# holstegelab/otter

Hardware: AMD Instinct MI355X
Metric: regions/sec (otter assemble) on synthetic TR BED+BAM, 1/2/4/8 MI355X (higher is better)
Workload: dtype i16

## Files before the change

otter_amd/csrc/otg_common.hpp:

```cpp
#pragma once
#include <hip/hip_runtime.h>
#include <cstdint>
#include <cstdio>
#include <cstring>
#include <mutex>
#include <string>
#include <vector>
#include "../../include/otter_gpu.h"

#define OTG_NULL_OFF (-(1 << 30))

struct DevBuf {
  void* p = nullptr;
  size_t cap = 0;
};

struct otg_ctx {
  int device = 0;
  hipStream_t stream = nullptr;
  hipDeviceProp_t prop;
  std::string err;
  int exp_variant = 1;
  long long exp_probe_mismatches = 0;
  int n_cu = 256;
  uint32_t max_seq_len = 65536;
  std::vector<DevBuf> pool;
  struct Pipeline* pipe = nullptr;
  hipEvent_t ev0 = nullptr, ev1 = nullptr;
  hipStream_t tier_stream[5] = {nullptr, nullptr, nullptr, nullptr, nullptr};
  hipEvent_t ev_fork = nullptr, ev_join[5] = {nullptr, nullptr, nullptr, nullptr, nullptr};
  int edit_pass_kind = 0;
  uint32_t* edit_hist = nullptr;
  hipEvent_t edit_hist_ev[2] = {nullptr, nullptr};
  uint32_t edit_hist_mask[2] = {0u, 0u};
  double last_score_ms = 0.0, last_prov_ms = 0.0;
  uint32_t last_align_tiers[2] = {0u, 0u};
  double last_kmer_count_ms = 0.0, last_kmer_epi_ms = 0.0;
  hipEvent_t ev2 = nullptr;
  double last_motif_count_ms = 0.0, last_motif_reduce_ms = 0.0;
  uint32_t last_motif_n = 0, last_motif_stride = 0;
  double last_repeat_runs_ms = 0.0, last_repeat_select_ms = 0.0;
  uint32_t last_repeat_n = 0;
  uint64_t last_repeat_total = 0;
  bool last_repeat_valid = false;
  const uint8_t* last_motif_arena = nullptr;
  const uint64_t* last_motif_off = nullptr;
  const uint32_t* last_motif_len = nullptr;
  double last_unitalign_ms = 0.0;
  uint32_t last_unitalign_n = 0;
  double last_unitparse_forward_ms = 0.0, last_unitparse_trace_ms = 0.0;
  uint32_t last_unitparse_n = 0;
  uint64_t last_unitparse_total = 0;
  bool last_unitparse_valid = false;
  double last_kernel_ms = 0.0;
  double last_gt_align_ms = 0.0, last_gt_cluster_ms = 0.0;
  bool gt_edit_ran = false;
  size_t gt_edit_cnt_off = 0;
  int heur_strategy = OTG_HEURISTIC_NONE, heur_min_wf_len = 10, heur_max_dist = 50, heur_steps = 1;
  int last_chain = -1;
  struct AffineLast {
    uint32_t n_tasks = 0;
    bool hbm_tiers = false;
    bool bounded = false;
    bool sublist = false;
    int reg_mask = 0;
    const void* scores_at = nullptr;
  } affine_last;
  struct Cohort* cohort = nullptr;
};

extern thread_local std::string g_otg_err;

int otg_fail(otg_ctx* ctx, int code, const char* fmt, ...);

#define HIP_TRY(ctx, call)                                                                      \
  do {                                                                                          \
    hipError_t e__ = (call);                                                                    \
    if (e__ != hipSuccess)                                                                      \
      return otg_fail(ctx, OTG_ERR_HIP, "%s failed: %s (%s:%d)", #call, hipGetErrorString(e__), \
                      __FILE__, __LINE__);                                                      \
  } while (0)

void* otg_slot(otg_ctx* ctx, int slot, size_t bytes);

constexpr uint32_t OTG_CLUSTER_NMAX = 256;
enum {
  SLOT_ARENA = 0, SLOT_TASKS, SLOT_SCORES, SLOT_CELLS, SLOT_COUNTERS , SLOT_WF_WS, SLOT_CIG_OFF, SLOT_CIG_LEN,
  SLOT_CIG_ARENA, SLOT_BT_POOL, SLOT_ROWTAB, SLOT_REVOPS, SLOT_TASKSTATE, SLOT_TODO, SLOT_AUX0, SLOT_AUX1,
  SLOT_AUX2, SLOT_AUX3, SLOT_AUX4, SLOT_AUX5, SLOT_AUX6, SLOT_AUX7, SLOT_AUX8, SLOT_AUX9,
  SLOT_P0, SLOT_P1, SLOT_P2, SLOT_P3, SLOT_P4, SLOT_P5, SLOT_P6, SLOT_P7, SLOT_P8, SLOT_P9,
  SLOT_P10, SLOT_P11, SLOT_P12, SLOT_P13, SLOT_P14, SLOT_P15, SLOT_P16, SLOT_P17, SLOT_P18, SLOT_P19,
  SLOT_P20, SLOT_P21, SLOT_P22, SLOT_P23, SLOT_P24, SLOT_P25, SLOT_P26, SLOT_P27, SLOT_P28, SLOT_P29,
  SLOT_KMER_SEQ, SLOT_KMER_META, SLOT_KMER_HIST, SLOT_KMER_OUT,
  SLOT_KMER_BLK,
  SLOT_GTE_CLS, SLOT_GTE_TASKS, SLOT_GTE_SCORES, SLOT_GTE_DEN, SLOT_GTE_TODO,
  SLOT_MOTIF_SEQ, SLOT_MOTIF_META, SLOT_MOTIF_OFF, SLOT_MOTIF_M, SLOT_MOTIF_PLANES, SLOT_MOTIF_OUT,
  SLOT_REPEAT_SEQ, SLOT_REPEAT_META, SLOT_REPEAT_OFF, SLOT_REPEAT_CNT, SLOT_REPEAT_PLANES, SLOT_REPEAT_RUNS, SLOT_REPEAT_STACK, SLOT_REPEAT_SCRATCH,
  SLOT_REPEAT_RES, SLOT_REPEAT_SEGS,
  SLOT_UNITALIGN_SEQ, SLOT_UNITALIGN_META, SLOT_UNITALIGN_UNITS, SLOT_UNITALIGN_BINS, SLOT_UNITALIGN_ORDER,
  SLOT_UNITALIGN_OUT,
  SLOT_UNITPARSE_SEQ, SLOT_UNITPARSE_META, SLOT_UNITPARSE_UNITS, SLOT_UNITPARSE_PLAN, SLOT_UNITPARSE_TRACE,
  SLOT_UNITPARSE_RES, SLOT_UNITPARSE_SEGS,
  SLOT_COUNT
};

inline void otg_region_name(std::string& o, const char* chr, uint32_t chr_len, int32_t start, int32_t end)
{
  o.append(chr, chr_len);
  o += ':'; o += std::to_string((uint32_t)start); o += '-'; o += std::to_string((uint32_t)end);
}

void otg_pipeline_free(otg_ctx* ctx);
int64_t otg_pipeline_run_regions(otg_ctx* ctx);
void otg_cohort_free(otg_ctx* ctx);
void otg_bam_set_samples(otg_bam* b, const char* const* names, uint32_t n, int32_t offset_l, int32_t offset_r);

std::mutex& otg_device_mutex(int device);

#if defined(__HIPCC__)
__device__ __forceinline__ uint32_t otg_wave_atomic_add(uint32_t* ctr, uint32_t val)
{
  uint32_t r;
  uint64_t saved;
  asm volatile(
      "s_mov_b64 %1, exec\n\t"
      "s_mov_b64 exec, 1\n\t"
      "global_atomic_add %0, %2, %3, off sc0\n\t"
      "s_waitcnt vmcnt(0)\n\t"
      "s_mov_b64 exec, %1"
      : "=&v"(r), "=&s"(saved)
      : "v"(ctr), "v"(val)
      : "memory");
  return (uint32_t)__builtin_amdgcn_readfirstlane((int)r);
}

__device__ __forceinline__ int otg_imax(int a, int b) { return a > b ? a : b; }
__device__ __forceinline__ int otg_wave_max_i32(int v)
{
  constexpr int NEG = -2147483647 - 1;
  v = otg_imax(v, __builtin_amdgcn_update_dpp(NEG, v, 0x111, 0xf, 0xf, false));
  v = otg_imax(v, __builtin_amdgcn_update_dpp(NEG, v, 0x112, 0xf, 0xf, false));
  v = otg_imax(v, __builtin_amdgcn_update_dpp(NEG, v, 0x114, 0xf, 0xf, false));
  v = otg_imax(v, __builtin_amdgcn_update_dpp(NEG, v, 0x118, 0xf, 0xf, false));
  v = otg_imax(v, __builtin_amdgcn_update_dpp(NEG, v, 0x142, 0xa, 0xf, false));
  v = otg_imax(v, __builtin_amdgcn_update_dpp(NEG, v, 0x143, 0xc, 0xf, false));
  return __builtin_amdgcn_readlane(v, 63);
}

__device__ __forceinline__ void otg_myers_band(int K, int d, int pbf, int pef, int* KL, int* KU)
{
  const int u1 = (K + d + pbf + 1) / 2, u2 = K + pbf;
  *KU = u1 < u2 ? u1 : u2;
  int l = (K - d + pef + 1) / 2;
  if (l > K) l = K;
  if (K - d + pef < 0) l = K - d + pef;
  *KL = l;
}
__device__ __forceinline__ unsigned long long otg_edit_wfa_cells(int s, int m, int n, int pbf, int tbf)
{
  if (s < 0) return 0ull;
  if (pbf > m) pbf = m;
  if (tbf > n) tbf = n;
  const long long kh = s < n - tbf ? s : n - tbf, kl = s < m - pbf ? s : m - pbf;
  const long long sum_hi = (kh + 1) * tbf + kh * (kh + 1) / 2 + ((long long)s - kh) * n;
  const long long sum_lo = (kl + 1) * pbf + kl * (kl + 1) / 2 + ((long long)s - kl) * m;
  return (unsigned long long)(sum_hi + sum_lo + (long long)s + 1);
}

__device__ __forceinline__ int otg_myers_threshold(int R, int d, int pbf, int pef)
{
  int lo = 0, hi = R;
  while (lo < hi) {
    const int mid = (lo + hi + 1) >> 1;
    int kl, ku;
    otg_myers_band(mid, d, pbf, pef, &kl, &ku);
    if (kl + ku <= R) lo = mid; else hi = mid - 1;
  }
  return lo;
}

__device__ __forceinline__ uint64_t otg_load8(const uint8_t* p) { uint64_t v; __builtin_memcpy(&v, p, 8); return v; }

__device__ __forceinline__ int otg_dpp_shr1(int x) { return __builtin_amdgcn_update_dpp(x, x, 0x138, 0xf, 0xf, false); }
__device__ __forceinline__ int otg_dpp_shl1(int x) { return __builtin_amdgcn_update_dpp(x, x, 0x130, 0xf, 0xf, false); }

__device__ __forceinline__ bool otg_ends_free_done(int h, int v, int pl, int tl, int pef, int tef)
{
  return (h >= tl && pl - v <= pef) || (v >= pl && tl - h <= tef);
}

__device__ __forceinline__ int otg_match16(const uint8_t* P, const uint8_t* T, int v, int h, int rem)
{
  const uint64_t xl = otg_load8(P + v) ^ otg_load8(T + h), xh = otg_load8(P + v + 8) ^ otg_load8(T + h + 8);
  const int m = xl ? (__builtin_ctzll(xl) >> 3) : (xh ? 8 + (__builtin_ctzll(xh) >> 3) : 16);
  return m < rem ? m : rem;
}

__device__ __forceinline__ int otg_match64(const uint8_t* P, const uint8_t* T, int v, int h, int rem)
{
  uint64_t x[8];
#pragma unroll
  for (int i = 0; i < 8; ++i) x[i] = (8 * i < rem) ? (otg_load8(P + v + 8 * i) ^ otg_load8(T + h + 8 * i)) : ~0ull;
  int m = 64;
#pragma unroll
  for (int i = 7; i >= 0; --i) if (x[i]) m = 8 * i + (__builtin_ctzll(x[i]) >> 3);
  return m < rem ? m : rem;
}

__device__ __forceinline__ int otg_wave_match(const uint8_t* P, const uint8_t* T, int v, int h, int rem, int lane)
{
  int total = 0;
  while (total < rem) {
    const int off = total + lane * 8;
    const bool in = off < rem;
    uint64_t x = ~0ull;
    if (in) x = otg_load8(P + v + off) ^ otg_load8(T + h + off);
    const int m = x ? (int)(__builtin_ctzll(x) >> 3) : 8;
    const unsigned long long stop = __ballot(m < 8);
    if (stop) {
      const int first = (int)__builtin_ctzll(stop);
      total += first * 8 + __builtin_amdgcn_readlane(m, first);
      break;
    }
    total += 512;
  }
  return total < rem ? total : rem;
}
#endif


int otg_launch_edit(otg_ctx* ctx, const uint8_t* d_arena, const otg_align_task* d_tasks, uint32_t n_tasks,
                    int32_t* d_scores, uint64_t* d_cells, float* kernel_ms, uint64_t* launches);

int otg_launch_edit_align(otg_ctx* ctx, const uint8_t* d_arena, const otg_align_task* d_tasks, const otg_align_task* h_tasks, uint32_t n_tasks,
                          int32_t* scores_out, uint32_t* len_out, uint8_t* d_cig_base, const uint64_t* cig_slot, double* score_ms, double* prov_ms,
                          uint32_t* finished = nullptr);
int otg_launch_edit_align_adaptive(otg_ctx* ctx, const uint8_t* d_arena, const otg_align_task* d_tasks, const otg_align_task* h_tasks, uint32_t n_tasks,
                                   int32_t* scores_out, uint64_t* cells_out, uint32_t* len_out, uint8_t* d_cig_base, const uint64_t* cig_slot,
                                   double* score_ms, double* prov_ms, uint32_t finished[2]);

constexpr int OTG_MYERS_TIERS = 8;
constexpr int OTG_REG_TIERS = 5;
namespace otg_myers { struct PlaneBlock; }
int otg_launch_myers(otg_ctx* ctx, int tier, const uint8_t* d_arena, const otg_align_task* d_tasks, const uint32_t* d_todo,
                     const uint32_t* d_n_todo, uint32_t n_tasks, int32_t* d_scores, uint64_t* d_cells,
                     uint32_t* ticket, uint32_t* n_overflow, uint32_t* overflow_list,
                     const uint32_t* d_pblk = nullptr, const otg_myers::PlaneBlock* d_masks = nullptr);
int otg_launch_edit_todo(otg_ctx* ctx, const uint8_t* d_arena, const otg_align_task* d_tasks, const uint32_t* d_todo,
                         const uint32_t* d_n_todo, uint32_t n_task_slots, int32_t* d_scores, uint64_t* d_cells,
                         float* kernel_ms, uint64_t* launches,
                         const uint32_t* d_pblk = nullptr, const otg_myers::PlaneBlock* d_masks = nullptr);
int otg_launch_read_masks(otg_ctx* ctx, const uint8_t* d_arena, const otg_read* d_reads, const uint32_t* d_read_region, uint32_t n_reads,
                          const uint32_t* d_first_blk, otg_myers::PlaneBlock* d_masks, uint32_t* d_read_blk);
int otg_launch_affine_todo(otg_ctx* ctx, const uint8_t* d_arena, const otg_align_task* d_tasks, const uint32_t* d_todo,
                           const uint32_t* d_n_todo, uint32_t n_task_slots, int x, int o, int e, int32_t* d_scores,
                           const uint64_t* d_cig_off, uint32_t* d_cig_len, uint8_t* d_cig_arena, uint64_t* d_cells,
                           float* kernel_ms = nullptr, uint64_t* launches = nullptr);

int otg_launch_affine(otg_ctx* ctx, const uint8_t* d_arena, const otg_align_task* d_tasks, uint32_t n_tasks,
                      int x, int o, int e, int32_t* d_scores, const uint64_t* d_cig_off, uint32_t* d_cig_len,
                      uint8_t* d_cig_arena, uint64_t* d_cells);

int otg_launch_edit_adaptive_todo(otg_ctx* ctx, const uint8_t* d_arena, const otg_align_task* d_tasks, const uint32_t* d_todo,
                                  const uint32_t* d_n_todo, uint32_t n_task_slots, int32_t* d_scores, uint64_t* d_cells,
                                  float* kernel_ms, uint64_t* launches);
int otg_launch_affine_adaptive_todo(otg_ctx* ctx, const uint8_t* d_arena, const otg_align_task* d_tasks, const uint32_t* d_todo,
                                    const uint32_t* d_n_todo, uint32_t n_task_slots, int x, int o, int e, int32_t* d_scores,
                                    const uint64_t* d_cig_off, uint32_t* d_cig_len, uint8_t* d_cig_arena, uint64_t* d_cells,
                                    float* kernel_ms, uint64_t* launches);

int otg_launch_cluster(otg_ctx* ctx, const otg_params* P, const double* d_dist, const uint64_t* d_dist_off,
                       const uint32_t* d_read_len, const uint64_t* d_len_off, const uint32_t* d_n_valid,
                       uint32_t n_regions, uint32_t n_max, const uint32_t* h_wide, uint32_t n_wide, int32_t* d_labels, int32_t* d_ic,
                       int32_t* d_fc, double* d_bounds, int32_t* d_err, const otg_cluster_trace* d_trace = nullptr, int exp_variant = -1);
int otg_launch_exp(otg_ctx* ctx, double* d_x, uint64_t n, int variant);

int otg_launch_poa(otg_ctx* ctx, const uint8_t* d_seq_arena, const uint8_t* d_cig_arena,
                   const otg_poa_member* d_members, uint32_t n_members, const otg_poa_graph* d_graphs,
                   const otg_poa_graph* h_graphs, uint32_t n_graphs, uint32_t* d_out_len,
                   std::vector<uint64_t>& node_off);

int otg_genotype_resident(otg_ctx* ctx, const otg_params* params, const uint8_t* d_arena, const uint64_t* d_off, const uint32_t* d_len,
                          const uint32_t* d_first, const uint32_t* d_n, const uint32_t* h_n_alleles, uint32_t n_regions, const uint64_t* d_poff,
                          uint64_t n_pairs, uint64_t na, int32_t* d_gt, double* d_hsd, int32_t* d_ngt, double* d_height = nullptr,
                          int metric = OTG_GT_METRIC_LENGTH, uint32_t max_len = 0);

int otg_genotype_metric_fits(otg_ctx* ctx, const char* who, int metric, uint64_t n_pairs);
int otg_device_max_u32(otg_ctx* ctx, const uint32_t* d_v, uint64_t n, uint32_t* out);
int otg_launch_genotype_edit_matrix(otg_ctx* ctx, const uint8_t* d_arena, const uint64_t* d_off, const uint32_t* d_len, const uint32_t* d_first,
                                    const uint32_t* d_n, uint32_t n_regions, const uint64_t* d_poff, uint64_t n_pairs, uint64_t na, uint32_t max_len);
int otg_genotype_metric_finish(otg_ctx* ctx, int metric, uint64_t* n_aligned);

int otg_kmer_usage_fits(otg_ctx* ctx, const char* who, uint32_t n, int32_t k);
int otg_kmer_usage_resident(otg_ctx* ctx, const char* who, const uint8_t* d_arena, const uint64_t* d_off, const uint32_t* d_len, const uint32_t* h_blk,
                            uint32_t n, int32_t k, double* usage_out, double* gc_out, double* hsd_out);

int otg_motif_args(otg_ctx* ctx, const char* who, uint32_t max_period, uint32_t slack);
int otg_motif_stride_fits(otg_ctx* ctx, const char* who, uint32_t max_len, uint32_t max_period, uint32_t unit_stride);
int otg_motif_resident(otg_ctx* ctx, const char* who, const uint8_t* d_arena, const uint64_t* d_off, const uint32_t* d_len, uint32_t n,
                       uint32_t max_period, uint32_t slack, otg_motif* out, uint8_t* unit_out, uint32_t unit_stride);
uint32_t otg_motif_lds_len();
void otg_motif_plane_scan(otg_ctx* ctx, const uint32_t* d_len, uint32_t n, uint32_t max_period, uint32_t lds_len, uint64_t* d_ploff, uint64_t* d_total);
void otg_motif_pack_planes(otg_ctx* ctx, const uint8_t* d_arena, const uint64_t* d_off, const uint32_t* d_len, uint32_t n, const uint64_t* d_ploff,
                           uint32_t* d_planes);
struct OtgUnitSource {
  const uint8_t* d_units; const uint64_t* d_unit_off; const uint32_t* d_unit_len; const otg_motif* d_motifs; uint32_t unit_stride;
};
int otg_unitalign_resident(otg_ctx* ctx, const char* who, const uint8_t* d_arena, const uint64_t* d_off, const uint32_t* d_len, const OtgUnitSource& units,
                           const uint32_t* d_task_seq, const uint32_t* d_task_unit, uint32_t n_tasks, otg_unitalign* out);
int otg_unitalign_check(otg_ctx* ctx, const char* who, uint32_t n_seqs, const uint8_t* unit_arena, uint64_t unit_bytes, const uint64_t* unit_off,
                        const uint32_t* unit_len, uint32_t n_units, const uint32_t* task_seq, const uint32_t* task_unit, uint32_t n_tasks);
int otg_unitalign_upload(otg_ctx* ctx, const uint8_t* unit_arena, uint64_t unit_bytes, const uint64_t* unit_off, const uint32_t* unit_len, uint32_t n_units,
                         const uint32_t* task_seq, const uint32_t* task_unit, uint32_t n_tasks, OtgUnitSource* units, const uint32_t** d_task_seq,
                         const uint32_t** d_task_unit);
int otg_unitparse_check(otg_ctx* ctx, const char* who, uint32_t n_seqs, const uint8_t* unit_arena, uint64_t unit_bytes, const uint64_t* unit_off,
                        const uint32_t* unit_len, uint32_t n_units, const uint64_t* set_first, uint32_t n_sets, const uint32_t* task_seq,
                        const uint32_t* task_set, uint32_t n_tasks);
int otg_unitparse_resident(otg_ctx* ctx, const char* who, const uint8_t* d_arena, const uint64_t* d_off, const uint32_t* d_len, const uint32_t* h_len,
                           uint32_t n_seqs, const uint8_t* unit_arena, uint64_t unit_bytes, const uint64_t* unit_off, const uint32_t* unit_len,
                           uint32_t n_units, const uint64_t* set_first, uint32_t n_sets, const uint32_t* task_seq, const uint32_t* task_set, uint32_t n_tasks,
                           otg_unitparse_sum* sums, uint64_t* seg_off, uint64_t* n_segments);
int otg_repeat_args(otg_ctx* ctx, const char* who, uint32_t max_period, uint32_t min_copies, uint32_t min_span);
int otg_repeat_resident(otg_ctx* ctx, const char* who, const uint8_t* d_arena, const uint64_t* d_off, const uint32_t* d_len, uint32_t n,
                        uint32_t max_period, uint32_t min_copies, uint32_t min_span, otg_repeat_sum* sums, uint64_t* seg_off, uint64_t* n_segments);

int otg_launch_genotype(otg_ctx* ctx, const otg_params* P, const uint8_t* d_arena, const uint64_t* d_seq_off,
                        const uint32_t* d_seq_len, const uint32_t* d_first, const uint32_t* d_n, uint32_t n_regions,
                        const uint64_t* d_pair_off, uint64_t n_pairs_total, uint64_t n_alleles_total, uint32_t a_max,
                        const uint32_t* h_wide, uint32_t n_wide,
                        int32_t* d_gt, int32_t* d_gtl, int32_t* d_gtk, double* d_hsd, int32_t* d_ngt, int32_t* d_reps,
                        int32_t* d_err, double* d_height_l = nullptr, double* d_height_k = nullptr, bool dl_given = false);
```

otter_amd/csrc/otg_scan.hpp:

```cpp
#pragma once
#include <cstdint>

#if defined(__HIPCC__)
template <class T>
struct OtgScanPtr {
  const T* p;
  __device__ __forceinline__ T operator()(uint32_t i) const { return p[i]; }
};

template <class Tacc, class Tout, class In>
__global__ void __launch_bounds__(1024) otg_scan_kernel(In in, uint32_t n, Tout* __restrict__ out, Tacc* __restrict__ total)
{
  constexpr uint32_t ITEMS = 8, T = 1024;
  __shared__ Tacc part[T];
  __shared__ Tacc carry_s;
  const uint32_t t = threadIdx.x;
  if (t == 0) carry_s = 0;
  __syncthreads();
  for (uint32_t base = 0; base < n; base += ITEMS * T) {
    Tacc v[ITEMS];
    Tacc sum = 0;
#pragma unroll
    for (uint32_t k = 0; k < ITEMS; ++k) {
      const uint32_t i = base + t * ITEMS + k;
      v[k] = i < n ? (Tacc)in(i) : (Tacc)0;
      sum += v[k];
    }
    part[t] = sum;
    __syncthreads();
    for (uint32_t d = 1; d < T; d <<= 1) {
      const Tacc add = t >= d ? part[t - d] : (Tacc)0;
      __syncthreads();
      part[t] += add;
      __syncthreads();
    }
    Tacc run = carry_s + part[t] - sum;
#pragma unroll
    for (uint32_t k = 0; k < ITEMS; ++k) {
      const uint32_t i = base + t * ITEMS + k;
      if (i < n) out[i] = (Tout)run;
      run += v[k];
    }
    __syncthreads();
    if (t == T - 1) carry_s += part[t];
    __syncthreads();
  }
  if (t == 0) {
    out[n] = (Tout)carry_s;
    if (total) *total = carry_s;
  }
}
#endif
```

otter_amd/csrc/pipeline.hip:

```cpp
#include "otg_chain.hpp"
#include "myers_masks.hpp"
#include <algorithm>
#include <chrono>
#include <cmath>
#include <vector>
#include <cstdlib>

enum { AL_NONE = 0, AL_COPY = 1, AL_POA = 2 };

struct AlleleSlot {
  uint64_t src_off;
  uint32_t src_len;
  int32_t kind;
  int32_t scov, acov, tcov;
  float se;
  int32_t ps, hp;
};

struct Pipeline {
  otg_params P;
  uint32_t n_reads = 0, n_regions = 0;
  uint64_t arena_bytes = 0;
  uint64_t rev_base = 0;
  std::vector<otg_read> h_reads;
  std::vector<otg_region> h_regions;
  std::vector<uint64_t> h_dist_off, h_re_off, h_cig_off;
  uint64_t n_pair_slots = 0, n_re_slots = 0, cig_bytes = 0;
  uint64_t n_mask_blocks = 0;
  uint32_t cl_nmax = 0;
  std::vector<uint32_t> cl_wide;
  std::vector<DevBuf> buf;
  otg_run_stats stats;
  uint32_t out_alleles = 0;
  uint64_t out_seq_bytes = 0;
  bool ran = false;
};

enum {
  B_ARENA = 0, B_READS, B_REGIONS, B_READ_REGION, B_DIST_OFF, B_RE_OFF, B_CIG_OFF, B_FIRST_READ64,
  B_STATUS, B_NVALID, B_IGNHAPS, B_VALID, B_VPOS, B_VLEN,
  B_TASKS, B_TODO, B_SCORES, B_DEN, B_DIST, B_CELLS, B_CNT,
  B_CLLAB, B_IC, B_FC, B_BOUNDS, B_CLERR, B_LABELS,
  B_REDIST, B_RTASKS, B_RKIND, B_CIGLEN, B_CIG,
  B_ALLELES, B_GRAPHS, B_MEMBERS, B_POALEN,
  B_ALLEN, B_ALOFF, B_ALIDX, B_OUTSEQ, B_OUTAL, B_REGRES, B_STATS, B_SCAN_TMP, B_TOTALS,
  B_MASKS, B_MASK_FIRST, B_MASK_READ, B_MASK_TASK,
  B_COUNT
};

static void* pbuf(otg_ctx* ctx, Pipeline* pl, int i, size_t bytes)
{
  if (bytes == 0) bytes = 16;
  DevBuf& b = pl->buf[i];
  if (b.cap >= bytes) return b.p;
  if (b.p) { (void)hipStreamSynchronize(ctx->stream); (void)hipFree(b.p); b.p = nullptr; b.cap = 0; }
  size_t want = bytes + (bytes >> 4) + 256;
  hipError_t e = hipMalloc(&b.p, want);
  if (e != hipSuccess) { otg_fail(ctx, OTG_ERR_HIP, "hipMalloc(%zu) for pipeline buffer %d failed: %s", want, i, hipGetErrorString(e)); b.p = nullptr; return nullptr; }
  b.cap = want;
  return b.p;
}

void otg_pipeline_free(otg_ctx* ctx)
{
  if (!ctx || !ctx->pipe) return;
  for (auto& b : ctx->pipe->buf) if (b.p) (void)hipFree(b.p);
  delete ctx->pipe;
  ctx->pipe = nullptr;
}

int64_t otg_pipeline_run_regions(otg_ctx* ctx) { return (ctx && ctx->pipe && ctx->pipe->ran) ? (int64_t)ctx->pipe->n_regions : -1; }

namespace {

__device__ __forceinline__ size_t didx(int N, int r, int c) { return (size_t)((((long long)(2 * N - 3 - r)) * r) >> 1) + c - 1; }

__device__ bool seq_equal(const uint8_t* a, const uint8_t* b, uint32_t n)
{
  for (uint32_t i = 0; i < n; ++i) if (a[i] != b[i]) return false;
  return true;
}

__device__ __forceinline__ void make_task(otg_align_task& t, uint64_t po, uint32_t pl, uint64_t to, uint32_t tl,
                                          int ef, int pbf, int pef, int tbf, int tef)
{
  t.pattern_off = po; t.text_off = to; t.pattern_len = pl; t.text_len = tl;
  t.pattern_begin_free = pbf; t.pattern_end_free = pef; t.text_begin_free = tbf; t.text_end_free = tef;
  t.endsfree = ef; t._pad = 0;
}

__device__ int anreads_task(const uint8_t* arena, const otg_read& x, const otg_read& y, otg_align_task& t, uint32_t* den, double* known, uint64_t rev_base = 0)
{
  const bool xs = x.spanning_l && x.spanning_r, ys = y.spanning_l && y.spanning_r;
  if (x.seq_len == y.seq_len && seq_equal(arena + x.seq_off, arena + y.seq_off, x.seq_len)) { *known = 0.0; return 0; }
  if ((xs && ys) || (ys && x.seq_len >= y.seq_len)) {
    const bool x_is_smallest = x.seq_len < y.seq_len;
    if (x_is_smallest) { make_task(t, y.seq_off, y.seq_len, x.seq_off, x.seq_len, 0, 0, 0, 0, 0); *den = y.seq_len; }
    else { make_task(t, x.seq_off, x.seq_len, y.seq_off, y.seq_len, 0, 0, 0, 0, 0); *den = x.seq_len; }
    return 1;
  }
  if (ys) {
    const int length_diff = (int)y.seq_len - (int)x.seq_len;
    int pbf, pef;
    if (x.spanning_l) { pbf = 0; pef = length_diff; }
    else if (x.spanning_r) { pbf = length_diff; pef = 0; }
    else { pbf = length_diff / 2; pef = length_diff / 2; }
    if (x.spanning_r && !x.spanning_l && rev_base) {
      make_task(t, rev_base + y.seq_off, y.seq_len, rev_base + x.seq_off, x.seq_len, 1, 0, length_diff, 0, 0);
      t._pad = 1;
    } else
    make_task(t, y.seq_off, y.seq_len, x.seq_off, x.seq_len, 1, pbf, pef, 0, 0);
    *den = x.seq_len;
    return 1;
  }
  *known = -1.0;
  return 0;
}

__device__ uint32_t task_mask_block(const uint32_t* __restrict__ read_blk, const otg_align_task& t, const otg_read& x, uint32_t xi, const otg_read& y, uint32_t yi)
{
  if (t._pad & 1) return otg_myers::NO_MASKS;
  if (t.pattern_off == y.seq_off && t.pattern_len == y.seq_len) return read_blk[yi];
  if (t.pattern_off == x.seq_off && t.pattern_len == x.seq_len) return read_blk[xi];
  return otg_myers::NO_MASKS;
}

__global__ void K_realign_prepare(const otg_read* __restrict__ reads, const otg_region* __restrict__ regions,
                                  const uint32_t* __restrict__ read_region, uint32_t n_reads, int flank,
                                  otg_align_task* __restrict__ tasks, uint8_t* __restrict__ kind,
                                  uint32_t* __restrict__ todo, uint32_t* __restrict__ n_todo)
{
  const uint32_t i = blockIdx.x * blockDim.x + threadIdx.x;
  if (i >= n_reads) return;
  if (read_region[i] == 0xffffffffu) { kind[i] = 0; return; }
  const otg_read rd = reads[i];
  const otg_region rg = regions[read_region[i]];
  uint8_t k = 0;
  const bool spanning = rd.spanning_l && rd.spanning_r;
  if (!spanning && (rd.spanning_l || rd.spanning_r) && rg.flank_l_len && rg.flank_r_len) {
    const bool left = rd.spanning_r && rd.ccoord_first >= flank;
    const bool right = rd.spanning_l && (int)rd.seq_len - rd.ccoord_second >= flank;
    if (left && rd.ccoord_first > 0) {
      make_task(tasks[i], rd.seq_off, (uint32_t)rd.ccoord_first, rg.flank_l_off, rg.flank_l_len, 0, 0, 0, 0, 0);
      k = 1;
    } else if (!left && right && (int)rd.seq_len - rd.ccoord_second > 0) {
      make_task(tasks[i], rd.seq_off + (uint32_t)rd.ccoord_second, rd.seq_len - (uint32_t)rd.ccoord_second, rg.flank_r_off, rg.flank_r_len, 0, 0, 0, 0, 0);
      k = 2;
    }
  }
  kind[i] = k;
  if (k) todo[atomicAdd(n_todo, 1u)] = i;
}

__global__ void K_realign_apply(otg_read* __restrict__ reads, uint32_t n_reads, const uint8_t* __restrict__ kind,
                                const uint8_t* __restrict__ cig, const uint64_t* __restrict__ cig_off,
                                const uint32_t* __restrict__ cig_len, int flank, double min_sim)
{
  const uint32_t i = blockIdx.x * blockDim.x + threadIdx.x;
  if (i >= n_reads || !kind[i]) return;
  const uint8_t* c = cig + cig_off[i];
  const uint32_t n = cig_len[i];
  int prev = 0, j = 0, best = 0, best_i = 0, last_nonpos = 0, start_i = 0;
  bool have0 = false;
  for (uint32_t q = 0; q < n; ++q) {
    const uint8_t op = c[q];
    if (op == 'I') continue;
    int sc = 0;
    if (op == 'M') sc = (j == 0) ? 1 : prev + 1;
    else if (j > 0 && prev > 0) sc = prev - 1;
    if (!have0) { best = sc; best_i = 0; have0 = true; last_nonpos = 0; start_i = 0; }
    if (sc <= 0) last_nonpos = j;
    if (sc > best) { best = sc; best_i = j; start_i = last_nonpos; }
    prev = sc; ++j;
  }
  if (!have0) return;
  if (((double)best / (double)flank) >= min_sim) {
    otg_read rd = reads[i];
    if (kind[i] == 1) { rd.seq_off += (uint32_t)best_i; rd.seq_len -= (uint32_t)best_i; }
    else { rd.seq_len = (uint32_t)(rd.ccoord_second + start_i); }
    rd.spanning_l = 1; rd.spanning_r = 1;
    reads[i] = rd;
  }
}

__global__ void K_region_prepare(const otg_read* __restrict__ reads, const otg_region* __restrict__ regions, uint32_t n_regions,
                                 int max_cov, int ignore_haps, int32_t* __restrict__ status, uint32_t* __restrict__ n_valid,
                                 int32_t* __restrict__ ign, uint32_t* __restrict__ valid, int32_t* __restrict__ vpos,
                                 uint32_t* __restrict__ vlen)
{
  const uint32_t r = blockIdx.x * blockDim.x + threadIdx.x;
  if (r >= n_regions) return;
  const otg_region rg = regions[r];
  const uint32_t f = rg.first_read, n = rg.n_reads;
  int st = OTG_REGION_OK;
  uint32_t nv = 0;
  int lig = ignore_haps;
  for (uint32_t i = 0; i < n; ++i) vpos[f + i] = -1;
  if (n == 0) st = OTG_REGION_EMPTY;
  else if ((int)n > max_cov) st = OTG_REGION_SKIP_MAXCOV;
  else {
    uint32_t span = 0;
    for (uint32_t i = 0; i < n; ++i) span += (reads[f + i].spanning_l && reads[f + i].spanning_r);
    if (span == 0) st = OTG_REGION_NO_SPANNING;
    else {
      for (int pass = 0; pass < 2; ++pass) {
        nv = 0;
        for (uint32_t i = 0; i < n; ++i) {
          const otg_read& rd = reads[f + i];
          const bool sp = rd.spanning_l && rd.spanning_r;
          const bool ok = sp && (lig || (rd.ps >= 0 && rd.hp >= 0));
          if (ok) valid[f + nv++] = f + i;
        }
        if (nv < 2 && !lig) lig = 1; else break;
      }
      if (nv == 0) st = OTG_REGION_NO_SPANNING;
      else for (uint32_t v = 0; v < nv; ++v) { vpos[valid[f + v]] = (int32_t)v; vlen[f + v] = reads[valid[f + v]].seq_len; }
    }
  }
  status[r] = st; n_valid[r] = (st == OTG_REGION_OK) ? nv : 0; ign[r] = lig;
}

__global__ void K_pair_tasks(const uint8_t* __restrict__ arena, const otg_read* __restrict__ reads,
                             const otg_region* __restrict__ regions, uint32_t n_regions, const uint32_t* __restrict__ n_valid,
                             const int32_t* __restrict__ ign, const uint32_t* __restrict__ valid,
                             const uint64_t* __restrict__ dist_off, int max_alleles,
                             otg_align_task* __restrict__ tasks, uint32_t* __restrict__ den, double* __restrict__ dist,
                             uint32_t* __restrict__ todo, uint32_t* __restrict__ n_todo,
                             const uint32_t* __restrict__ read_blk, uint32_t* __restrict__ task_blk)
{
  for (uint32_t r = blockIdx.x; r < n_regions; r += gridDim.x) {
    const int n = (int)n_valid[r];
    if (n < 2) continue;
    const uint32_t f = regions[r].first_read;
    const uint64_t base = dist_off[r];
    const size_t np = (size_t)n * (n - 1) / 2;
    if (max_alleles == 1) { for (size_t q = threadIdx.x; q < np; q += blockDim.x) dist[base + q] = 1.0; continue; }
    for (int i = 0; i < n - 1; ++i) {
      const uint32_t xi = valid[f + i];
      const otg_read x = reads[xi];
      for (int j = i + 1 + (int)threadIdx.x; j < n; j += (int)blockDim.x) {
        const uint32_t yi = valid[f + j];
        const otg_read y = reads[yi];
        const uint64_t slot = base + didx(n, i, j);
        if (!ign[r]) {
          const bool bx = x.ps >= 0 && x.hp >= 0, by = y.ps >= 0 && y.hp >= 0;
          dist[slot] = (bx && by && x.ps == y.ps && x.hp == y.hp) ? 0.0 : 1.0;
        } else {
          double known = 0;
          uint32_t d = 1;
          if (anreads_task(arena, x, y, tasks[slot], &d, &known)) {
            den[slot] = d; todo[atomicAdd(n_todo, 1u)] = (uint32_t)slot;
            if (task_blk) task_blk[slot] = task_mask_block(read_blk, tasks[slot], x, xi, y, yi);
          }
          else dist[slot] = known;
        }
      }
    }
  }
}

__global__ void K_dist_epilogue(const uint32_t* __restrict__ todo, const uint32_t* __restrict__ n_todo,
                                const int32_t* __restrict__ scores, const uint32_t* __restrict__ den, double* __restrict__ dist,
                                uint32_t* __restrict__ fail_flag)
{
  const uint32_t n = *n_todo;
  for (uint32_t t = blockIdx.x * blockDim.x + threadIdx.x; t < n; t += gridDim.x * blockDim.x) {
    const uint32_t slot = todo[t];
    if (scores[slot] < 0) *fail_flag = 1u;
    dist[slot] = scores[slot] / (double)den[slot];
  }
}

__global__ void K_stats(const uint32_t* __restrict__ todo, const uint32_t* __restrict__ n_todo,
                        const otg_align_task* __restrict__ tasks, const uint64_t* __restrict__ cells, unsigned long long* acc,
                        const int32_t* __restrict__ scores, uint32_t* __restrict__ fail_flag)
{
  __shared__ unsigned long long sc[256], sb[256];
  const uint32_t n = *n_todo;
  unsigned long long c = 0, b = 0;
  for (uint32_t t = blockIdx.x * blockDim.x + threadIdx.x; t < n; t += gridDim.x * blockDim.x) {
    const uint32_t slot = todo[t];
    if (scores[slot] < 0) { *fail_flag = 1u; continue; }
    c += cells[slot];
    b += (unsigned long long)tasks[slot].pattern_len + tasks[slot].text_len;
  }
  sc[threadIdx.x] = c; sb[threadIdx.x] = b;
  __syncthreads();
  for (int s = 128; s > 0; s >>= 1) { if ((int)threadIdx.x < s) { sc[threadIdx.x] += sc[threadIdx.x + s]; sb[threadIdx.x] += sb[threadIdx.x + s]; } __syncthreads(); }
  if (threadIdx.x == 0) { atomicAdd(&acc[0], sc[0]); atomicAdd(&acc[1], sb[0]); if (blockIdx.x == 0) atomicAdd(&acc[2], (unsigned long long)n); }
}

__global__ void K_mark_failed_affine(const uint32_t* __restrict__ todo, const uint32_t* __restrict__ n_todo, const int32_t* __restrict__ scores,
                                     const uint32_t* __restrict__ read_region, int32_t* __restrict__ status)
{
  const uint32_t n = *n_todo;
  for (uint32_t t = blockIdx.x * blockDim.x + threadIdx.x; t < n; t += gridDim.x * blockDim.x) {
    const uint32_t slot = todo[t];
    if (scores[slot] < 0) { const uint32_t r = read_region[slot]; if (r != 0xffffffffu) status[r] = OTG_REGION_ALIGN_CAPACITY; }
  }
}

__global__ void K_scatter_labels(const uint32_t* __restrict__ read_region, const otg_region* __restrict__ regions,
                                 const int32_t* __restrict__ vpos, const int32_t* __restrict__ cl_labels, uint32_t n_reads,
                                 int32_t* __restrict__ labels)
{
  const uint32_t i = blockIdx.x * blockDim.x + threadIdx.x;
  if (i >= n_reads) return;
  if (read_region[i] == 0xffffffffu) { labels[i] = -1; return; }
  const int v = vpos[i];
  labels[i] = v >= 0 ? cl_labels[regions[read_region[i]].first_read + v] : -1;
}

__global__ void K_reverse_reads(uint8_t* __restrict__ arena, const otg_read* __restrict__ reads, const otg_region* __restrict__ regions,
                                const uint32_t* __restrict__ read_region, uint32_t n_reads, const int32_t* __restrict__ status,
                                const uint32_t* __restrict__ n_valid, uint64_t rev_base)
{
  const uint32_t lane = threadIdx.x & 63u;
  const uint32_t nw = gridDim.x * (blockDim.x >> 6);
  for (uint32_t i = blockIdx.x * (blockDim.x >> 6) + (threadIdx.x >> 6); i < n_reads; i += nw) {
    const uint32_t r = read_region[i];
    if (r == 0xffffffffu || status[r] != OTG_REGION_OK || n_valid[r] >= regions[r].n_reads) continue;
    const otg_read rd = reads[i];
    const uint8_t* src = arena + rd.seq_off;
    uint8_t* dst = arena + rev_base + rd.seq_off;
    for (uint32_t j = lane; j < rd.seq_len; j += 64) dst[j] = src[rd.seq_len - 1 - j];
  }
}

__global__ void K_reassign_tasks(const uint8_t* __restrict__ arena, const otg_read* __restrict__ reads,
                                 const otg_region* __restrict__ regions, uint32_t n_regions, const int32_t* __restrict__ status,
                                 const uint32_t* __restrict__ n_valid, const int32_t* __restrict__ fc, const int32_t* __restrict__ labels,
                                 const uint64_t* __restrict__ re_off, otg_align_task* __restrict__ tasks,
                                 uint32_t* __restrict__ den, double* __restrict__ dist,
                                 uint32_t* __restrict__ todo, uint32_t* __restrict__ n_todo, uint64_t rev_base,
                                 const uint32_t* __restrict__ read_blk, uint32_t* __restrict__ task_blk)
{
  for (uint32_t r = blockIdx.x; r < n_regions; r += gridDim.x) {
    if (status[r] != OTG_REGION_OK || fc[r] <= 0) continue;
    const otg_region rg = regions[r];
    const int n = (int)rg.n_reads;
    if ((int)n_valid[r] >= n) continue;
    const uint32_t f = rg.first_read;
    for (int i = 0; i < n; ++i) {
      if (labels[f + i] >= 0) continue;
      const otg_read x = reads[f + i];
      for (int j = (int)threadIdx.x; j < n; j += (int)blockDim.x) {
        if (j == i) continue;
        const otg_read y = reads[f + j];
        if (!(y.spanning_l && y.spanning_r)) continue;
        if (labels[f + j] < 0 && j > i) continue;
        const uint64_t slot = re_off[r] + (uint64_t)i * n + j;
        double known = 0;
        uint32_t d = 1;
        if (anreads_task(arena, x, y, tasks[slot], &d, &known, rev_base)) {
          den[slot] = d; todo[atomicAdd(n_todo, 1u)] = (uint32_t)slot;
          if (task_blk) task_blk[slot] = task_mask_block(read_blk, tasks[slot], x, f + (uint32_t)i, y, f + (uint32_t)j);
        }
        else dist[slot] = known;
      }
    }
  }
}

__global__ void K_reassign_apply(const otg_read* __restrict__ reads, const otg_region* __restrict__ regions, uint32_t n_regions,
                                 const int32_t* __restrict__ status, const uint32_t* __restrict__ n_valid,
                                 const int32_t* __restrict__ fc, const uint64_t* __restrict__ re_off,
                                 const double* __restrict__ dist, double min_sim, double max_error,
                                 int32_t* __restrict__ labels, int32_t* __restrict__ status_out)
{
  const uint32_t r = blockIdx.x * blockDim.x + threadIdx.x;
  if (r >= n_regions || status[r] != OTG_REGION_OK) return;
  const otg_region rg = regions[r];
  const int n = (int)rg.n_reads;
  if ((int)n_valid[r] >= n) return;
  const uint32_t f = rg.first_read;
  const int total = fc[r];
  if (total <= 0) return;
  for (int i = 0; i < n; ++i) {
    if (labels[f + i] >= 0) continue;
    int max_label = 0; double max_val = 0.0; int same = 0;
    for (int l = 0; l < total; ++l) {
      double ms = 0.0;
      for (int j = 0; j < n; ++j) {
        if (j == i || labels[f + j] != l) continue;
        const otg_read& y = reads[f + j];
        if (!(y.spanning_l && y.spanning_r)) continue;
        const double d = dist[re_off[r] + (uint64_t)i * n + j];
        if (d < 0) { status_out[r] = OTG_ERR_FATAL; return; }
        const double sim = 1 - d;
        if (sim > ms) ms = sim;
      }
      if (l == 0 || ms > max_val) { max_val = ms; max_label = l; }
    }
    double min_diff = 1.0;
    for (int l = 0; l < total; ++l) {
      double ms = 0.0;
      for (int j = 0; j < n; ++j) {
        if (j == i || labels[f + j] != l) continue;
        const otg_read& y = reads[f + j];
        if (!(y.spanning_l && y.spanning_r)) continue;
        const double sim = 1 - dist[re_off[r] + (uint64_t)i * n + j];
        if (sim > ms) ms = sim;
      }
      if (ms == max_val) ++same;
      if (l != max_label) { const double diff = max_val - ms; if (diff < min_diff) min_diff = diff; }
    }
    if (same == 1 && max_val >= min_sim && min_diff >= max_error) labels[f + i] = max_label;
  }
}

__global__ void K_consensus_prepare(const otg_read* __restrict__ reads, const otg_region* __restrict__ regions, uint32_t n_regions,
                                    int32_t* __restrict__ status, const uint32_t* __restrict__ n_valid, const int32_t* __restrict__ ign,
                                    const uint32_t* __restrict__ valid, const int32_t* __restrict__ labels, const int32_t* __restrict__ fc,
                                    const uint64_t* __restrict__ dist_off, const double* __restrict__ dist,
                                    const uint64_t* __restrict__ cig_off,
                                    AlleleSlot* __restrict__ alleles, otg_poa_graph* __restrict__ graphs,
                                    otg_poa_member* __restrict__ members, otg_align_task* __restrict__ tasks,
                                    uint32_t* __restrict__ todo, uint32_t* __restrict__ n_todo, uint32_t* __restrict__ scratch)
{
  const uint32_t r = blockIdx.x * blockDim.x + threadIdx.x;
  if (r >= n_regions) return;
  const otg_region rg = regions[r];
  const uint32_t f = rg.first_read;
  const int n = (int)rg.n_reads;
  for (int i = 0; i < n; ++i) { alleles[f + i].kind = AL_NONE; graphs[f + i].backbone_len = 0; graphs[f + i].n_members = 0; graphs[f + i].first_member = f; graphs[f + i].backbone_off = 0; graphs[f + i].c = 1.0f; graphs[f + i].t = 0.3f; }
  if (status[r] != OTG_REGION_OK) return;
  const int nv = (int)n_valid[r];
  const int total = fc[r];
  const double* D = dist + dist_off[r];
  uint32_t* liv = scratch + f;
  uint32_t mpos = f;
  for (int label = 0; label < total; ++label) {
    int nl = 0;
    for (int vi = 0; vi < nv; ++vi) if (labels[valid[f + vi]] == label) liv[nl++] = (uint32_t)vi;
    if (nl == 0) { status[r] = OTG_ERR_FATAL; return; }
    uint32_t rep_vi = liv[0];
    double min_sum = 100000000.0;
    for (int a = 0; a < nl; ++a) {
      double s = 0.0;
      for (int b = 0; b < nl; ++b) if (liv[a] != liv[b]) { const int i = (int)liv[a], j = (int)liv[b]; s += i < j ? D[didx(nv, i, j)] : D[didx(nv, j, i)]; }
      if (s < min_sum) { rep_vi = liv[a]; min_sum = s; }
    }
    const uint32_t rep = valid[f + rep_vi];
    int n_all = 0;
    for (int i = 0; i < n; ++i) if (f + i != rep && labels[f + i] == label) ++n_all;
    AlleleSlot A;
    A.tcov = n; A.acov = n_all + 1; A.scov = nl;
    if (nl == 1) A.se = 0;
    else if (nl == 2) { const int i = (int)liv[0], j = (int)liv[1]; A.se = (float)(i < j ? D[didx(nv, i, j)] : D[didx(nv, j, i)]); }
    else {
      double u = 0.0, q = 0.0; int cnt = 0;
      for (int a = 0; a < nl; ++a) if (liv[a] != rep_vi) { const int i = (int)liv[a], j = (int)rep_vi; u += i < j ? D[didx(nv, i, j)] : D[didx(nv, j, i)]; ++cnt; }
      u /= cnt;
      for (int a = 0; a < nl; ++a) if (liv[a] != rep_vi) { const int i = (int)liv[a], j = (int)rep_vi; const double v = (i < j ? D[didx(nv, i, j)] : D[didx(nv, j, i)]); q += (v - u) * (v - u); }
      A.se = (float)(sqrt(q / (cnt - 1)) / sqrt((double)cnt));
    }
    int ps = -1, hp = -1; bool conflicting = false;
    if (!ign[r]) {
      for (int a = 0; a < nl; ++a) {
        const otg_read& rd = reads[valid[f + liv[a]]];
        if (ps < 0) ps = rd.ps; else if (ps != rd.ps) conflicting = true;
        if (hp < 0) hp = rd.hp; else if (hp != rd.hp) conflicting = true;
      }
    }
    if (conflicting) { status[r] = OTG_REGION_HAP_CONFLICT; return; }
    const otg_read rep_read = reads[rep];
    A.ps = ign[r] ? -1 : rep_read.ps; A.hp = ign[r] ? -1 : rep_read.hp;
    A.src_off = 0; A.src_len = 0;
    if (n_all + 1 <= 2) {
      const otg_read& fr = reads[valid[f + liv[0]]];
      A.kind = AL_COPY; A.src_off = fr.seq_off; A.src_len = fr.seq_len;
    } else {
      A.kind = AL_POA;
      otg_poa_graph G;
      G.backbone_off = rep_read.seq_off; G.backbone_len = rep_read.seq_len; G.first_member = mpos; G.n_members = (uint32_t)n_all;
      float c = (float)((n_all + 1) * 0.4);
      if (n_all + 1 < 4) c = 1.0f;
      G.c = c; G.t = 0.3f; G._pad = 0;
      graphs[f + label] = G;
      uint64_t prev_cig_read = (uint64_t)-1;
      for (int i = 0; i < n; ++i) {
        if (f + i == rep || labels[f + i] != label) continue;
        const otg_read rd = reads[f + i];
        const int length_diff = (int)rep_read.seq_len - (int)rd.seq_len;
        const bool sp = rd.spanning_l && rd.spanning_r;
        int ef = 0, pbf = 0, pef = 0, tbf = 0, tef = 0; bool do_align = true;
        if (sp || length_diff < 0) {
          if (length_diff >= 0) { }
          else if (rd.spanning_l) { ef = 1; tef = -length_diff; }
          else if (rd.spanning_r) { ef = 1; tbf = -length_diff; }
          else do_align = false;
        } else {
          ef = 1;
          if (rd.spanning_l) pef = length_diff;
          else if (rd.spanning_r) pbf = length_diff;
          else { pbf = length_diff / 2; pef = length_diff / 2; }
        }
        otg_poa_member M;
        M.seq_off = rd.seq_off; M.seq_len = rd.seq_len; M.spanning_l = rd.spanning_l; M.spanning_r = rd.spanning_r;
        for (int q = 0; q < 6; ++q) M._pad[q] = 0;
        if (do_align) {
          make_task(tasks[f + i], rep_read.seq_off, rep_read.seq_len, rd.seq_off, rd.seq_len, ef, pbf, pef, tbf, tef);
          todo[atomicAdd(n_todo, 1u)] = f + i;
          prev_cig_read = f + i;
        }
        M.cigar_off = prev_cig_read == (uint64_t)-1 ? (uint64_t)-1 : cig_off[prev_cig_read];
        M.cigar_len = prev_cig_read == (uint64_t)-1 ? 0u : (uint32_t)prev_cig_read;
        members[mpos++] = M;
      }
    }
    alleles[f + label] = A;
  }
}

__global__ void K_member_cigars(otg_poa_member* __restrict__ members, const otg_poa_graph* __restrict__ graphs, uint32_t n_slots,
                                const uint32_t* __restrict__ cig_len)
{
  const uint32_t g = blockIdx.x * blockDim.x + threadIdx.x;
  if (g >= n_slots) return;
  const otg_poa_graph G = graphs[g];
  for (uint32_t m = 0; m < G.n_members; ++m) {
    otg_poa_member& M = members[G.first_member + m];
    if (M.cigar_off == (uint64_t)-1) { M.cigar_off = 0; M.cigar_len = 0; }
    else M.cigar_len = cig_len[M.cigar_len];
  }
}

__global__ void K_allele_len(const AlleleSlot* __restrict__ alleles, const int32_t* __restrict__ status,
                             const uint32_t* __restrict__ read_region, const uint32_t* __restrict__ poa_len, const int32_t* __restrict__ poa_status,
                             uint32_t n_slots, uint32_t* __restrict__ al_len, uint32_t* __restrict__ al_flag, int32_t* __restrict__ status_out)
{
  const uint32_t i = blockIdx.x * blockDim.x + threadIdx.x;
  if (i >= n_slots) return;
  uint32_t len = 0, flag = 0;
  const uint32_t r = read_region[i];
  if (r != 0xffffffffu && status[r] == OTG_REGION_OK && alleles[i].kind != AL_NONE) {
    flag = 1;
    if (alleles[i].kind == AL_COPY) len = alleles[i].src_len;
    else {
      if (poa_status[i]) status_out[r] = OTG_ERR_FATAL;
      len = poa_len[i] ? poa_len[i] : 1;
    }
  }
  al_len[i] = len; al_flag[i] = flag;
}

__global__ __launch_bounds__(1024) void K_scan(const uint32_t* __restrict__ in, uint64_t* __restrict__ out, uint32_t n, uint64_t* __restrict__ total)
{
  __shared__ uint64_t part[1024];
  const uint32_t t = threadIdx.x;
  const uint32_t chunk = (n + 1023) / 1024;
  const uint32_t a = t * chunk, b = a + chunk < n ? a + chunk : n;
  uint64_t s = 0;
  for (uint32_t i = a; i < b; ++i) s += in[i];
  part[t] = s;
  __syncthreads();
  if (t == 0) { uint64_t acc = 0; for (int i = 0; i < 1024; ++i) { const uint64_t v = part[i]; part[i] = acc; acc += v; } *total = acc; }
  __syncthreads();
  uint64_t acc = part[t];
  for (uint32_t i = a; i < b; ++i) { out[i] = acc; acc += in[i]; }
}

__global__ void K_gather(const uint8_t* __restrict__ arena, const AlleleSlot* __restrict__ alleles, const uint32_t* __restrict__ al_len,
                         const uint32_t* __restrict__ al_flag, const uint64_t* __restrict__ al_off, const uint64_t* __restrict__ al_idx,
                         const uint32_t* __restrict__ read_region, const otg_region* __restrict__ regions, const int32_t* __restrict__ ic,
                         const uint8_t* __restrict__ poa_out, const uint64_t* __restrict__ poa_node_off, const uint32_t* __restrict__ poa_start,
                         const uint32_t* __restrict__ poa_len, uint32_t n_slots, uint8_t* __restrict__ out_seq, otg_allele* __restrict__ out_al)
{
  for (uint32_t i = blockIdx.x; i < n_slots; i += gridDim.x) {
    if (!al_flag[i]) continue;
    const AlleleSlot A = alleles[i];
    const uint32_t len = al_len[i];
    uint8_t* dst = out_seq + al_off[i];
    if (A.kind == AL_COPY) { const uint8_t* src = arena + A.src_off; for (uint32_t q = threadIdx.x; q < len; q += blockDim.x) dst[q] = src[q]; }
    else if (poa_len[i] == 0) { if (threadIdx.x == 0) dst[0] = 'N'; }
    else { const uint8_t* src = poa_out + poa_node_off[i] + poa_start[i]; for (uint32_t q = threadIdx.x; q < len; q += blockDim.x) dst[q] = src[q]; }
    if (threadIdx.x == 0) {
      const uint32_t r = read_region[i];
      otg_allele o;
      o.seq_off = al_off[i]; o.seq_len = len; o.scov = A.scov; o.acov = A.acov; o.tcov = A.tcov; o.se = A.se; o.ic = ic[r];
      o.ps = A.ps; o.hp = A.hp; o.region = r; o.label = (int32_t)(i - regions[r].first_read);
      out_al[al_idx[i]] = o;
    }
  }
}

__global__ void K_region_results(const otg_region* __restrict__ regions, uint32_t n_regions, const int32_t* __restrict__ status,
                                 const int32_t* __restrict__ ic, const int32_t* __restrict__ fc, const uint32_t* __restrict__ n_valid,
                                 const uint64_t* __restrict__ al_idx, const uint32_t* __restrict__ al_flag,
                                 const int32_t* __restrict__ clerr, otg_region_result* __restrict__ out)
{
  const uint32_t r = blockIdx.x * blockDim.x + threadIdx.x;
  if (r >= n_regions) return;
  otg_region_result o;
  o.status = status[r]; o.ic = 0; o.fc = 0; o.n_valid = (int32_t)n_valid[r]; o.first_allele = 0; o.n_alleles = 0;
  if (o.status == OTG_REGION_OK && clerr[r]) o.status = OTG_ERR_FATAL;
  if (regions[r].n_reads) o.first_allele = (uint32_t)al_idx[regions[r].first_read];
  if (o.status == OTG_REGION_OK) {
    o.ic = ic[r]; o.fc = fc[r];
    uint32_t na = 0;
    for (uint32_t i = 0; i < regions[r].n_reads; ++i) na += al_flag[regions[r].first_read + i];
    o.n_alleles = na;
  }
  out[r] = o;
}

__global__ void K_fill_f64(double* p, size_t n, double v)
{
  for (size_t i = blockIdx.x * (size_t)blockDim.x + threadIdx.x; i < n; i += (size_t)gridDim.x * blockDim.x) p[i] = v;
}

static void dbg(otg_ctx* ctx, const char* what)
{
  if (!otg_env_set("OTG_DEBUG")) return;
  hipError_t e = hipStreamSynchronize(ctx->stream);
  hipError_t e2 = hipGetLastError();
  fprintf(stderr, "[otg] %s: %s / %s\n", what, hipGetErrorString(e), hipGetErrorString(e2));
}

struct Timer {
  otg_ctx* ctx; std::chrono::steady_clock::time_point t0;
  explicit Timer(otg_ctx* c) : ctx(c) { (void)hipStreamSynchronize(c->stream); t0 = std::chrono::steady_clock::now(); }
  double ms() { (void)hipStreamSynchronize(ctx->stream); return std::chrono::duration<double, std::milli>(std::chrono::steady_clock::now() - t0).count(); }
};

}

extern "C" {

int otg_assemble_submit(otg_ctx* ctx, const otg_params* params, const uint8_t* seq_arena, uint64_t arena_bytes,
                        const otg_read* reads, uint32_t n_reads, const otg_region* regions, uint32_t n_regions)
{
  if (!ctx) return otg_fail(nullptr, OTG_ERR_NO_DEVICE, "otg_assemble_submit: no context (no HIP device?)");
  if (!params || (n_reads && (!reads || !seq_arena)) || (n_regions && !regions)) return otg_fail(ctx, OTG_ERR_ARG, "otg_assemble_submit: NULL argument");
  HIP_TRY(ctx, hipSetDevice(ctx->device));
  if (!ctx->pipe) { ctx->pipe = new Pipeline(); ctx->pipe->buf.resize(B_COUNT); }
  Pipeline* pl = ctx->pipe;
  pl->P = *params; pl->n_reads = n_reads; pl->n_regions = n_regions; pl->arena_bytes = arena_bytes; pl->ran = false;
  pl->cl_nmax = 0; pl->cl_wide.clear();
  pl->h_reads.assign(reads, reads + n_reads);
  pl->h_regions.assign(regions, regions + n_regions);
  std::vector<uint32_t> read_region(n_reads, 0xffffffffu);
  std::vector<uint8_t> covered(n_reads, 0);
  pl->h_dist_off.assign(n_regions + 1, 0); pl->h_re_off.assign(n_regions + 1, 0); pl->h_cig_off.assign((size_t)n_reads + 1, 0);
  uint32_t maxlen = 1;
  std::vector<uint32_t> region_maxlen(n_regions, 1);
  for (uint32_t r = 0; r < n_regions; ++r) {
    const otg_region& g = regions[r];
    if ((uint64_t)g.first_read + g.n_reads > n_reads) return otg_fail(ctx, OTG_ERR_ARG, "region %u: read range out of bounds", r);
    if (g.flank_l_off + g.flank_l_len > arena_bytes || g.flank_r_off + g.flank_r_len > arena_bytes) return otg_fail(ctx, OTG_ERR_ARG, "region %u: flank outside the arena", r);
    uint64_t n = g.n_reads;
    uint32_t ml = std::max(g.flank_l_len, g.flank_r_len);
    for (uint32_t i = 0; i < g.n_reads; ++i) {
      const otg_read& q = reads[g.first_read + i];
      if (covered[g.first_read + i]) return otg_fail(ctx, OTG_ERR_ARG, "read %u belongs to two regions", g.first_read + i);
      covered[g.first_read + i] = 1; read_region[g.first_read + i] = r;
      if (q.seq_off + q.seq_len > arena_bytes) return otg_fail(ctx, OTG_ERR_ARG, "read %u: sequence outside the arena", g.first_read + i);
      ml = std::max(ml, q.seq_len);
    }
    region_maxlen[r] = ml; maxlen = std::max(maxlen, ml);
    const bool big = (int)g.n_reads > params->max_cov;
    if (!big) {
      if (n >= 65536) return otg_fail(ctx, OTG_ERR_CAPACITY, "region %u: %llu reads, more than the 65 535 one region can hold (V^2 slots below 2^32)", r, (unsigned long long)n);
      pl->cl_nmax = std::max<uint32_t>(pl->cl_nmax, g.n_reads);
      if (g.n_reads > OTG_CLUSTER_NMAX) pl->cl_wide.push_back(r);
    }
    pl->h_dist_off[r + 1] = pl->h_dist_off[r] + (big ? 0 : n * (n ? n - 1 : 0) / 2);
    pl->h_re_off[r + 1] = pl->h_re_off[r] + (big ? 0 : n * n);
  }
  for (uint32_t i = 0; i < n_reads; ++i)
    pl->h_cig_off[i + 1] = pl->h_cig_off[i] + (covered[i] ? (((uint64_t)region_maxlen[read_region[i]] + reads[i].seq_len + 15) & ~15ull) : 0);
  pl->n_pair_slots = pl->h_dist_off[n_regions]; pl->n_re_slots = pl->h_re_off[n_regions]; pl->cig_bytes = pl->h_cig_off[n_reads];
  static const bool edit_masks = otg_env_int("OTG_EDIT_MASKS", 1) != 0;
  std::vector<uint32_t> mask_first(n_reads, 0u);
  pl->n_mask_blocks = 0;
  if (edit_masks) {
    uint64_t nb = 0;
    for (uint32_t i = 0; i < n_reads; ++i) { mask_first[i] = (uint32_t)nb; if (covered[i]) nb += ((uint64_t)reads[i].seq_len + 63) >> 6; if (nb >= 0xffffffffull) break; }
    pl->n_mask_blocks = nb < 0xffffffffull ? nb : 0;
  }
  if (pl->n_pair_slots >= 0xffffffffull || pl->n_re_slots >= 0xffffffffull)
    return otg_fail(ctx, OTG_ERR_CAPACITY, "batch too large: split it (pair slots %llu, reassignment slots %llu)", (unsigned long long)pl->n_pair_slots, (unsigned long long)pl->n_re_slots);
  ctx->max_seq_len = maxlen;
  std::vector<uint64_t> first64(n_regions);
  for (uint32_t r = 0; r < n_regions; ++r) first64[r] = regions[r].first_read;
  pl->rev_base = (arena_bytes + 64 + 255) & ~(uint64_t)255;
  uint8_t* d_arena = (uint8_t*)pbuf(ctx, pl, B_ARENA, pl->rev_base + arena_bytes + 64);
  void* d_reads = pbuf(ctx, pl, B_READS, (size_t)n_reads * sizeof(otg_read));
  void* d_regions = pbuf(ctx, pl, B_REGIONS, (size_t)n_regions * sizeof(otg_region));
  void* d_rr = pbuf(ctx, pl, B_READ_REGION, (size_t)n_reads * 4);
  void* d_do = pbuf(ctx, pl, B_DIST_OFF, (size_t)(n_regions + 1) * 8);
  void* d_ro = pbuf(ctx, pl, B_RE_OFF, (size_t)(n_regions + 1) * 8);
  void* d_co = pbuf(ctx, pl, B_CIG_OFF, (size_t)(n_reads + 1) * 8);
  void* d_f64 = pbuf(ctx, pl, B_FIRST_READ64, (size_t)n_regions * 8);
  if (!d_arena || !d_reads || !d_regions || !d_rr || !d_do || !d_ro || !d_co || !d_f64) return OTG_ERR_HIP;
  if (pl->n_mask_blocks) {
    void* d_mf = pbuf(ctx, pl, B_MASK_FIRST, (size_t)n_reads * 4);
    if (!d_mf) return OTG_ERR_HIP;
    HIP_TRY(ctx, hipMemcpyAsync(d_mf, mask_first.data(), (size_t)n_reads * 4, hipMemcpyHostToDevice, ctx->stream));
  }
  HIP_TRY(ctx, hipMemsetAsync(d_arena + arena_bytes, 0, 64, ctx->stream));
  HIP_TRY(ctx, hipMemsetAsync(d_arena + pl->rev_base + arena_bytes, 0, 64, ctx->stream));
  if (arena_bytes) HIP_TRY(ctx, hipMemcpyAsync(d_arena, seq_arena, arena_bytes, hipMemcpyHostToDevice, ctx->stream));
  if (n_reads) HIP_TRY(ctx, hipMemcpyAsync(d_rr, read_region.data(), (size_t)n_reads * 4, hipMemcpyHostToDevice, ctx->stream));
  if (n_regions) HIP_TRY(ctx, hipMemcpyAsync(d_regions, regions, (size_t)n_regions * sizeof(otg_region), hipMemcpyHostToDevice, ctx->stream));
  HIP_TRY(ctx, hipMemcpyAsync(d_do, pl->h_dist_off.data(), (size_t)(n_regions + 1) * 8, hipMemcpyHostToDevice, ctx->stream));
  HIP_TRY(ctx, hipMemcpyAsync(d_ro, pl->h_re_off.data(), (size_t)(n_regions + 1) * 8, hipMemcpyHostToDevice, ctx->stream));
  HIP_TRY(ctx, hipMemcpyAsync(d_co, pl->h_cig_off.data(), (size_t)(n_reads + 1) * 8, hipMemcpyHostToDevice, ctx->stream));
  if (n_regions) HIP_TRY(ctx, hipMemcpyAsync(d_f64, first64.data(), (size_t)n_regions * 8, hipMemcpyHostToDevice, ctx->stream));
  HIP_TRY(ctx, hipStreamSynchronize(ctx->stream));
  const size_t ntask = std::max<size_t>(std::max<size_t>(pl->n_pair_slots, pl->n_re_slots), n_reads) + 1;
  if (!pbuf(ctx, pl, B_TASKS, ntask * sizeof(otg_align_task)) || !pbuf(ctx, pl, B_TODO, ntask * 4) || !pbuf(ctx, pl, B_SCORES, ntask * 4) ||
      !pbuf(ctx, pl, B_DEN, ntask * 4) || !pbuf(ctx, pl, B_CELLS, ntask * 8) || !pbuf(ctx, pl, B_DIST, (pl->n_pair_slots + 1) * 8) ||
      !pbuf(ctx, pl, B_REDIST, (pl->n_re_slots + 1) * 8) || !pbuf(ctx, pl, B_CNT, 64 * 8) || !pbuf(ctx, pl, B_STATS, 64 * 8) ||
      !pbuf(ctx, pl, B_STATUS, (size_t)n_regions * 4 + 4) || !pbuf(ctx, pl, B_NVALID, (size_t)n_regions * 4 + 4) ||
      !pbuf(ctx, pl, B_IGNHAPS, (size_t)n_regions * 4 + 4) || !pbuf(ctx, pl, B_VALID, (size_t)n_reads * 4 + 4) ||
      !pbuf(ctx, pl, B_VPOS, (size_t)n_reads * 4 + 4) || !pbuf(ctx, pl, B_VLEN, (size_t)n_reads * 4 + 4) ||
      !pbuf(ctx, pl, B_CLLAB, (size_t)n_reads * 4 + 4) || !pbuf(ctx, pl, B_IC, (size_t)n_regions * 4 + 4) || !pbuf(ctx, pl, B_FC, (size_t)n_regions * 4 + 4) ||
      !pbuf(ctx, pl, B_BOUNDS, (size_t)n_regions * 24 + 8) || !pbuf(ctx, pl, B_CLERR, (size_t)n_regions * 4 + 4) || !pbuf(ctx, pl, B_LABELS, (size_t)n_reads * 4 + 4) ||
      !pbuf(ctx, pl, B_RKIND, (size_t)n_reads + 4) || !pbuf(ctx, pl, B_CIGLEN, (size_t)n_reads * 4 + 4) || !pbuf(ctx, pl, B_CIG, pl->cig_bytes + 64) ||
      !pbuf(ctx, pl, B_ALLELES, (size_t)(n_reads + 1) * sizeof(AlleleSlot)) || !pbuf(ctx, pl, B_GRAPHS, (size_t)(n_reads + 1) * sizeof(otg_poa_graph)) ||
      !pbuf(ctx, pl, B_MEMBERS, (size_t)(n_reads + 1) * sizeof(otg_poa_member)) || !pbuf(ctx, pl, B_POALEN, (size_t)n_reads * 4 + 4) ||
      !pbuf(ctx, pl, B_ALLEN, (size_t)n_reads * 4 + 4) || !pbuf(ctx, pl, B_ALOFF, (size_t)n_reads * 8 + 8) || !pbuf(ctx, pl, B_ALIDX, (size_t)n_reads * 8 + 8) ||
      !pbuf(ctx, pl, B_SCAN_TMP, (size_t)n_reads * 4 + 4) || !pbuf(ctx, pl, B_TOTALS, 64) || !pbuf(ctx, pl, B_REGRES, (size_t)(n_regions + 1) * sizeof(otg_region_result)) ||
      !otg_slot(ctx, SLOT_AUX9, (pl->n_pair_slots + 1) * 8))
    return OTG_ERR_HIP;
  if (pl->n_mask_blocks && (!pbuf(ctx, pl, B_MASKS, (size_t)pl->n_mask_blocks * sizeof(otg_myers::PlaneBlock)) || !pbuf(ctx, pl, B_MASK_READ, (size_t)n_reads * 4) ||
                            !pbuf(ctx, pl, B_MASK_TASK, ntask * 4)))
    return OTG_ERR_HIP;
  return OTG_OK;
}

static int assemble_run_impl(otg_ctx* ctx, bool realign_only);

int otg_assemble_run(otg_ctx* ctx) { return assemble_run_impl(ctx, false); }

int otg_assemble_realign(otg_ctx* ctx) { return assemble_run_impl(ctx, true); }

int otg_assemble_collect_reads(otg_ctx* ctx, otg_read* reads_out, uint32_t n_reads)
{
  if (!ctx) return otg_fail(nullptr, OTG_ERR_NO_DEVICE, "otg_assemble_collect_reads: no context");
  Pipeline* pl = ctx->pipe;
  if (!pl) return otg_fail(ctx, OTG_ERR_ARG, "otg_assemble_collect_reads: nothing submitted");
  if (n_reads != pl->n_reads || (n_reads && !reads_out)) return otg_fail(ctx, OTG_ERR_ARG, "otg_assemble_collect_reads: expected room for %u reads", pl->n_reads);
  HIP_TRY(ctx, hipSetDevice(ctx->device));
  if (n_reads) HIP_TRY(ctx, hipMemcpyAsync(reads_out, pl->buf[B_READS].p, (size_t)n_reads * sizeof(otg_read), hipMemcpyDeviceToHost, ctx->stream));
  HIP_TRY(ctx, hipStreamSynchronize(ctx->stream));
  return OTG_OK;
}

int otg_assemble_collect_dist(otg_ctx* ctx, double* dist_out, uint64_t n_slots)
{
  if (!ctx) return otg_fail(nullptr, OTG_ERR_NO_DEVICE, "otg_assemble_collect_dist: no context");
  Pipeline* pl = ctx->pipe;
  if (!pl || !pl->ran) return otg_fail(ctx, OTG_ERR_ARG, "otg_assemble_collect_dist: no completed run");
  if (n_slots != pl->n_pair_slots || (n_slots && !dist_out)) return otg_fail(ctx, OTG_ERR_ARG, "otg_assemble_collect_dist: expected room for %llu distances", (unsigned long long)pl->n_pair_slots);
  HIP_TRY(ctx, hipSetDevice(ctx->device));
  if (n_slots) HIP_TRY(ctx, hipMemcpyAsync(dist_out, pl->buf[B_DIST].p, (size_t)n_slots * sizeof(double), hipMemcpyDeviceToHost, ctx->stream));
  HIP_TRY(ctx, hipStreamSynchronize(ctx->stream));
  return OTG_OK;
}

static int assemble_run_body(otg_ctx* ctx, bool realign_only);

static int assemble_run_impl(otg_ctx* ctx, bool realign_only)
{
  if (!ctx) return otg_fail(nullptr, OTG_ERR_NO_DEVICE, "otg_assemble_run: no context");
  Pipeline* pl = ctx->pipe;
  if (!pl) return otg_fail(ctx, OTG_ERR_ARG, "otg_assemble_run: nothing submitted");
  const int sv[4] = {ctx->heur_strategy, ctx->heur_min_wf_len, ctx->heur_max_dist, ctx->heur_steps};
  const otg_params& P = pl->P;
  if (P.heuristic != OTG_HEURISTIC_NONE && P.heuristic != OTG_HEURISTIC_WFADAPTIVE) return otg_fail(ctx, OTG_ERR_ARG, "otg_assemble_run: unknown heuristic %d in otg_params", P.heuristic);
  ctx->heur_strategy = P.heuristic;
  if (P.heuristic == OTG_HEURISTIC_WFADAPTIVE) {
    if (P.heur_min_wavefront_length < 0 || P.heur_max_distance_threshold < 0) return otg_fail(ctx, OTG_ERR_ARG, "otg_assemble_run: negative heuristic parameter in otg_params");
    ctx->heur_min_wf_len = P.heur_min_wavefront_length; ctx->heur_max_dist = P.heur_max_distance_threshold;
    ctx->heur_steps = P.heur_steps_between_cutoffs < 1 ? 1 : P.heur_steps_between_cutoffs;
  }
  const int rc = assemble_run_body(ctx, realign_only);
  ctx->heur_strategy = sv[0]; ctx->heur_min_wf_len = sv[1]; ctx->heur_max_dist = sv[2]; ctx->heur_steps = sv[3];
  return rc;
}

static int assemble_run_body(otg_ctx* ctx, bool realign_only)
{
  Pipeline* pl = ctx->pipe;
  HIP_TRY(ctx, hipSetDevice(ctx->device));
  const otg_params& P = pl->P;
  const uint32_t NR = pl->n_reads, NG = pl->n_regions;
  hipStream_t st = ctx->stream;
  auto B = [&](int i) { return pl->buf[i].p; };
  uint8_t* d_arena = (uint8_t*)B(B_ARENA);
  otg_read* d_reads = (otg_read*)B(B_READS);
  const otg_region* d_regions = (const otg_region*)B(B_REGIONS);
  const uint32_t* d_rr = (const uint32_t*)B(B_READ_REGION);
  otg_align_task* d_tasks = (otg_align_task*)B(B_TASKS);
  uint32_t* d_todo = (uint32_t*)B(B_TODO);
  int32_t* d_scores = (int32_t*)B(B_SCORES);
  uint32_t* d_den = (uint32_t*)B(B_DEN);
  uint64_t* d_cells = (uint64_t*)B(B_CELLS);
  double* d_dist = (double*)B(B_DIST);
  double* d_redist = (double*)B(B_REDIST);
  uint32_t* d_cnt = (uint32_t*)B(B_CNT);
  unsigned long long* d_stats = (unsigned long long*)B(B_STATS);
  int32_t* d_status = (int32_t*)B(B_STATUS);
  uint32_t* d_nvalid = (uint32_t*)B(B_NVALID);
  int32_t* d_ign = (int32_t*)B(B_IGNHAPS);
  uint32_t* d_valid = (uint32_t*)B(B_VALID);
  int32_t* d_vpos = (int32_t*)B(B_VPOS);
  uint32_t* d_vlen = (uint32_t*)B(B_VLEN);
  int32_t* d_labels = (int32_t*)B(B_LABELS);
  uint64_t* d_cig_off = (uint64_t*)B(B_CIG_OFF);
  uint32_t* d_cig_len = (uint32_t*)B(B_CIGLEN);
  uint8_t* d_cig = (uint8_t*)B(B_CIG);
  const bool masks = pl->n_mask_blocks != 0 && ctx->heur_strategy == OTG_HEURISTIC_NONE;
  otg_myers::PlaneBlock* d_masks = masks ? (otg_myers::PlaneBlock*)B(B_MASKS) : nullptr;
  uint32_t* d_read_blk = masks ? (uint32_t*)B(B_MASK_READ) : nullptr;
  uint32_t* d_task_blk = masks ? (uint32_t*)B(B_MASK_TASK) : nullptr;
  memset(&pl->stats, 0, sizeof(pl->stats));
  pl->ran = false;
  pl->out_alleles = 0; pl->out_seq_bytes = 0;
  if (NG == 0 || NR == 0) { pl->ran = true; return OTG_OK; }
  Timer total(ctx);
  HIP_TRY(ctx, hipMemcpyAsync(d_reads, pl->h_reads.data(), (size_t)NR * sizeof(otg_read), hipMemcpyHostToDevice, st));
  HIP_TRY(ctx, hipMemsetAsync(d_cnt, 0, 64 * 8, st));
  HIP_TRY(ctx, hipMemsetAsync(d_stats, 0, 64 * 8, st));
  if (unsigned long long* visited = otg_affine_visited(ctx)) HIP_TRY(ctx, hipMemsetAsync(visited, 0, 8, st));
  const int TB = 256;
  const uint32_t gr_reads = (NR + TB - 1) / TB, gr_regions = (NG + TB - 1) / TB;
  const uint32_t gr_blocks = std::min<uint32_t>(NG, (uint32_t)ctx->n_cu * 16);
  int rc;
  if (P.realign) {
    Timer t(ctx);
    hipLaunchKernelGGL(K_realign_prepare, dim3(gr_reads), dim3(TB), 0, st, d_reads, d_regions, d_rr, NR, P.flank, d_tasks, (uint8_t*)B(B_RKIND), d_todo, d_cnt + 16);
    HIP_TRY(ctx, hipMemsetAsync(d_cig_len, 0, (size_t)NR * 4, st));
    { float kms = 0; uint64_t kl = 0;
      rc = otg_launch_affine_todo(ctx, d_arena, d_tasks, d_todo, d_cnt + 16, NR, P.mismatch, P.gap_open, P.gap_ext, d_scores, d_cig_off, d_cig_len, d_cig, d_cells, &kms, &kl);
      if (rc) return rc;
      pl->stats.ms_affine_kernel += kms; pl->stats.affine_kernel_launches += kl; }
    hipLaunchKernelGGL(K_stats, dim3(64), dim3(256), 0, st, d_todo, d_cnt + 16, d_tasks, d_cells, d_stats + 4, d_scores, d_cnt + 42);
    hipLaunchKernelGGL(K_realign_apply, dim3(gr_reads), dim3(TB), 0, st, d_reads, NR, (const uint8_t*)B(B_RKIND), d_cig, d_cig_off, d_cig_len, P.flank, P.min_sim);
    pl->stats.ms_realign = t.ms();
  }
  dbg(ctx, "realign done");
  if (realign_only) {
    HIP_TRY(ctx, hipStreamSynchronize(st));
    pl->stats.ms_total = total.ms();
    uint32_t hf = 0;
    HIP_TRY(ctx, hipMemcpy(&hf, d_cnt + 42, sizeof(hf), hipMemcpyDeviceToHost));
    if (hf) return otg_fail(ctx, OTG_ERR_CAPACITY, "a gap-affine alignment exhausted its backtrace storage on the device");
    return OTG_OK;
  }
  {
    Timer t(ctx);
    hipLaunchKernelGGL(K_region_prepare, dim3(gr_regions), dim3(TB), 0, st, d_reads, d_regions, NG, P.max_cov, P.ignore_haps, d_status, d_nvalid, d_ign, d_valid, d_vpos, d_vlen);
    if (d_masks) {
      rc = otg_launch_read_masks(ctx, d_arena, d_reads, d_rr, NR, (const uint32_t*)B(B_MASK_FIRST), d_masks, d_read_blk);
      if (rc) return rc;
    }
    hipLaunchKernelGGL(K_pair_tasks, dim3(gr_blocks), dim3(64), 0, st, d_arena, d_reads, d_regions, NG, d_nvalid, d_ign, d_valid, (const uint64_t*)B(B_DIST_OFF), P.max_alleles, d_tasks, d_den, d_dist, d_todo, d_cnt + 20,
                       (const uint32_t*)d_read_blk, d_task_blk);
    float kms = 0; uint64_t kl = 0;
    dbg(ctx, "pair tasks done");
    rc = otg_launch_edit_todo(ctx, d_arena, d_tasks, d_todo, d_cnt + 20, (uint32_t)pl->n_pair_slots, d_scores, d_cells, &kms, &kl, d_task_blk, d_masks);
    if (rc) return rc;
    pl->stats.ms_edit_kernel += kms; pl->stats.edit_kernel_launches += kl;
    hipLaunchKernelGGL(K_dist_epilogue, dim3(1024), dim3(256), 0, st, d_todo, d_cnt + 20, d_scores, d_den, d_dist, d_cnt + 40);
    hipLaunchKernelGGL(K_stats, dim3(64), dim3(256), 0, st, d_todo, d_cnt + 20, d_tasks, d_cells, d_stats + 0, d_scores, d_cnt + 40);
    pl->stats.ms_edit = t.ms();
  }
  dbg(ctx, "edit done");
  {
    Timer t(ctx);
    rc = otg_launch_cluster(ctx, &P, d_dist, (const uint64_t*)B(B_DIST_OFF), d_vlen, (const uint64_t*)B(B_FIRST_READ64), d_nvalid, NG,
                            pl->cl_nmax, pl->cl_wide.data(), (uint32_t)pl->cl_wide.size(), (int32_t*)B(B_CLLAB), (int32_t*)B(B_IC), (int32_t*)B(B_FC), (double*)B(B_BOUNDS), (int32_t*)B(B_CLERR));
    if (rc) return rc;
    hipLaunchKernelGGL(K_scatter_labels, dim3(gr_reads), dim3(TB), 0, st, d_rr, d_regions, d_vpos, (const int32_t*)B(B_CLLAB), NR, d_labels);
    pl->stats.ms_cluster = t.ms();
  }
  dbg(ctx, "cluster done");
  {
    Timer t(ctx);
    static const bool no_rev = otg_env_set("OTG_NO_REASSIGN_REV");
    const uint64_t rev_base = (no_rev || ctx->heur_strategy != OTG_HEURISTIC_NONE) ? 0 : pl->rev_base;
    if (rev_base) hipLaunchKernelGGL(K_reverse_reads, dim3(std::min<uint32_t>((NR + 3) / 4, (uint32_t)ctx->n_cu * 32)), dim3(256), 0, st, d_arena, d_reads, d_regions, d_rr, NR,
                                     d_status, d_nvalid, rev_base);
    hipLaunchKernelGGL(K_reassign_tasks, dim3(gr_blocks), dim3(64), 0, st, d_arena, d_reads, d_regions, NG, d_status, d_nvalid, (const int32_t*)B(B_FC), d_labels,
                       (const uint64_t*)B(B_RE_OFF), d_tasks, d_den, d_redist, d_todo, d_cnt + 24, rev_base, (const uint32_t*)d_read_blk, d_task_blk);
    float kms = 0; uint64_t kl = 0;
    ctx->edit_pass_kind = 1;
    rc = otg_launch_edit_todo(ctx, d_arena, d_tasks, d_todo, d_cnt + 24, (uint32_t)pl->n_re_slots, d_scores, d_cells, &kms, &kl, d_task_blk, d_masks);
    ctx->edit_pass_kind = 0;
    if (rc) return rc;
    pl->stats.ms_edit_kernel += kms; pl->stats.edit_kernel_launches += kl;
    hipLaunchKernelGGL(K_dist_epilogue, dim3(1024), dim3(256), 0, st, d_todo, d_cnt + 24, d_scores, d_den, d_redist, d_cnt + 40);
    hipLaunchKernelGGL(K_stats, dim3(64), dim3(256), 0, st, d_todo, d_cnt + 24, d_tasks, d_cells, d_stats + 0, d_scores, d_cnt + 40);
    hipLaunchKernelGGL(K_reassign_apply, dim3((NG + 63) / 64), dim3(64), 0, st, d_reads, d_regions, NG, d_status, d_nvalid, (const int32_t*)B(B_FC),
                       (const uint64_t*)B(B_RE_OFF), d_redist, P.min_sim, P.max_error, d_labels, d_status);
    pl->stats.ms_reassign = t.ms();
  }
  dbg(ctx, "reassign done");
  std::vector<uint64_t> node_off;
  {
    Timer t(ctx);
    HIP_TRY(ctx, hipMemsetAsync(d_cig_len, 0, (size_t)NR * 4, st));
    HIP_TRY(ctx, hipMemsetAsync(B(B_ALLELES), 0, (size_t)NR * sizeof(AlleleSlot), st));
    HIP_TRY(ctx, hipMemsetAsync(B(B_GRAPHS), 0, (size_t)NR * sizeof(otg_poa_graph), st));
    HIP_TRY(ctx, hipMemsetAsync(B(B_MEMBERS), 0, (size_t)(NR + 1) * sizeof(otg_poa_member), st));
    hipLaunchKernelGGL(K_consensus_prepare, dim3((NG + 63) / 64), dim3(64), 0, st, d_reads, d_regions, NG, d_status, d_nvalid, d_ign, d_valid, d_labels,
                       (const int32_t*)B(B_FC), (const uint64_t*)B(B_DIST_OFF), d_dist, d_cig_off, (AlleleSlot*)B(B_ALLELES),
                       (otg_poa_graph*)B(B_GRAPHS), (otg_poa_member*)B(B_MEMBERS), d_tasks, d_todo, d_cnt + 28, (uint32_t*)B(B_SCAN_TMP));
    { float kms = 0; uint64_t kl = 0;
      rc = otg_launch_affine_todo(ctx, d_arena, d_tasks, d_todo, d_cnt + 28, NR, P.mismatch, P.gap_open, P.gap_ext, d_scores, d_cig_off, d_cig_len, d_cig, d_cells, &kms, &kl);
      if (rc) return rc;
      pl->stats.ms_affine_kernel += kms; pl->stats.affine_kernel_launches += kl; }
    hipLaunchKernelGGL(K_stats, dim3(64), dim3(256), 0, st, d_todo, d_cnt + 28, d_tasks, d_cells, d_stats + 4, d_scores, d_cnt + 41);
    hipLaunchKernelGGL(K_mark_failed_affine, dim3(64), dim3(256), 0, st, d_todo, d_cnt + 28, d_scores, d_rr, d_status);
    hipLaunchKernelGGL(K_member_cigars, dim3(gr_reads), dim3(TB), 0, st, (otg_poa_member*)B(B_MEMBERS), (const otg_poa_graph*)B(B_GRAPHS), NR, d_cig_len);
    pl->stats.ms_affine = t.ms();
    dbg(ctx, "affine done");
    Timer t2(ctx);
    std::vector<otg_poa_graph> h_graphs(NR);
    HIP_TRY(ctx, hipMemcpyAsync(h_graphs.data(), B(B_GRAPHS), (size_t)NR * sizeof(otg_poa_graph), hipMemcpyDeviceToHost, st));
    HIP_TRY(ctx, hipStreamSynchronize(st));
    rc = otg_launch_poa(ctx, d_arena, d_cig, (const otg_poa_member*)B(B_MEMBERS), NR, (const otg_poa_graph*)B(B_GRAPHS), h_graphs.data(), NR,
                        (uint32_t*)B(B_POALEN), node_off);
    if (rc) return rc;
    pl->stats.ms_poa = t2.ms();
  }
  dbg(ctx, "consensus done");
  {
    uint32_t* d_allen = (uint32_t*)B(B_ALLEN);
    uint32_t* d_alflag = (uint32_t*)B(B_SCAN_TMP);
    uint64_t* d_aloff = (uint64_t*)B(B_ALOFF);
    uint64_t* d_alidx = (uint64_t*)B(B_ALIDX);
    uint64_t* d_tot = (uint64_t*)B(B_TOTALS);
    hipLaunchKernelGGL(K_allele_len, dim3(gr_reads), dim3(TB), 0, st, (const AlleleSlot*)B(B_ALLELES), d_status, d_rr, (const uint32_t*)B(B_POALEN),
                       (const int32_t*)ctx->pool[SLOT_P28].p, NR, d_allen, d_alflag, d_status);
    hipLaunchKernelGGL(K_scan, dim3(1), dim3(1024), 0, st, d_allen, d_aloff, NR, d_tot + 0);
    hipLaunchKernelGGL(K_scan, dim3(1), dim3(1024), 0, st, d_alflag, d_alidx, NR, d_tot + 1);
    uint64_t h_tot[2];
    HIP_TRY(ctx, hipMemcpyAsync(h_tot, d_tot, 16, hipMemcpyDeviceToHost, st));
    HIP_TRY(ctx, hipStreamSynchronize(st));
    pl->out_seq_bytes = h_tot[0]; pl->out_alleles = (uint32_t)h_tot[1];
    uint8_t* d_outseq = (uint8_t*)pbuf(ctx, pl, B_OUTSEQ, pl->out_seq_bytes + 16);
    otg_allele* d_outal = (otg_allele*)pbuf(ctx, pl, B_OUTAL, (size_t)(pl->out_alleles + 1) * sizeof(otg_allele));
    if (!d_outseq || !d_outal) return OTG_ERR_HIP;
    uint64_t* d_nodeoff = (uint64_t*)ctx->pool[SLOT_P0].p;
    hipLaunchKernelGGL(K_gather, dim3(std::min<uint32_t>(NR, (uint32_t)ctx->n_cu * 16)), dim3(128), 0, st, d_arena, (const AlleleSlot*)B(B_ALLELES), d_allen, d_alflag,
                       d_aloff, d_alidx, d_rr, d_regions, (const int32_t*)B(B_IC), (const uint8_t*)ctx->pool[SLOT_P17].p, d_nodeoff,
                       (const uint32_t*)ctx->pool[SLOT_P29].p, (const uint32_t*)B(B_POALEN), NR, d_outseq, d_outal);
    hipLaunchKernelGGL(K_region_results, dim3(gr_regions), dim3(TB), 0, st, d_regions, NG, d_status, (const int32_t*)B(B_IC), (const int32_t*)B(B_FC), d_nvalid,
                       d_alidx, d_alflag, (const int32_t*)B(B_CLERR), (otg_region_result*)B(B_REGRES));
  }
  dbg(ctx, "gather done");
  HIP_TRY(ctx, hipGetLastError());
  pl->stats.ms_total = total.ms();
  {
    uint32_t hf[3];
    HIP_TRY(ctx, hipMemcpy(hf, d_cnt + 40, sizeof(hf), hipMemcpyDeviceToHost));
    if (hf[0]) return otg_fail(ctx, OTG_ERR_FATAL, "an edit-distance alignment did not complete on the device");
    if (hf[2]) return otg_fail(ctx, OTG_ERR_CAPACITY, "a flank re-alignment exhausted its backtrace storage on the device");
  }
  unsigned long long hs[8];
  HIP_TRY(ctx, hipMemcpy(hs, d_stats, sizeof(hs), hipMemcpyDeviceToHost));
  pl->stats.edit_cells = hs[0]; pl->stats.edit_seq_bytes = hs[1]; pl->stats.edit_tasks = hs[2];
  pl->stats.affine_cells = hs[4]; pl->stats.affine_seq_bytes = hs[5]; pl->stats.affine_tasks = hs[6];
  pl->stats.n_regions = NG;
  if (const unsigned long long* visited = otg_affine_visited(ctx)) { unsigned long long v = 0; HIP_TRY(ctx, hipMemcpy(&v, visited, 8, hipMemcpyDeviceToHost)); pl->stats.affine_visited_cells = v; }
  pl->stats.allele_bytes = pl->out_seq_bytes + 40ull * pl->out_alleles;
  pl->stats.algorithmic_bytes = pl->stats.edit_seq_bytes + 4 * pl->stats.edit_cells + pl->stats.affine_seq_bytes + 4 * pl->stats.affine_cells +
                                (pl->stats.affine_cells + 1) / 2 + pl->stats.allele_bytes;
  {
    std::vector<otg_region_result> rr(NG);
    HIP_TRY(ctx, hipMemcpy(rr.data(), B(B_REGRES), (size_t)NG * sizeof(otg_region_result), hipMemcpyDeviceToHost));
    uint64_t ok = 0;
    for (auto& r : rr) { if (r.status < 0) return otg_fail(ctx, OTG_ERR_FATAL, "a region hit a condition on which the reference exit(1)s (status %d)", r.status); ok += (r.n_alleles > 0); }
    pl->stats.n_regions_ok = ok;
  }
  pl->ran = true;
  return OTG_OK;
}

int otg_assemble_result_sizes(otg_ctx* ctx, uint32_t* n_alleles, uint64_t* seq_bytes)
{
  if (!ctx || !ctx->pipe || !ctx->pipe->ran) return otg_fail(ctx, OTG_ERR_ARG, "otg_assemble_result_sizes: no completed run");
  if (n_alleles) *n_alleles = ctx->pipe->out_alleles;
  if (seq_bytes) *seq_bytes = ctx->pipe->out_seq_bytes;
  return OTG_OK;
}

int otg_assemble_collect(otg_ctx* ctx, otg_region_result* region_out, otg_allele* alleles_out, uint32_t allele_capacity,
                         uint8_t* seq_out, uint64_t seq_capacity, int32_t* labels_out)
{
  if (!ctx || !ctx->pipe || !ctx->pipe->ran) return otg_fail(ctx, OTG_ERR_ARG, "otg_assemble_collect: no completed run");
  Pipeline* pl = ctx->pipe;
  HIP_TRY(ctx, hipSetDevice(ctx->device));
  if (allele_capacity < pl->out_alleles || seq_capacity < pl->out_seq_bytes) return otg_fail(ctx, OTG_ERR_CAPACITY, "otg_assemble_collect: output buffers too small");
  if (pl->n_regions == 0 || pl->n_reads == 0) {
    for (uint32_t r = 0; r < pl->n_regions; ++r) { if (region_out) { memset(&region_out[r], 0, sizeof(otg_region_result)); region_out[r].status = OTG_REGION_EMPTY; } }
    return OTG_OK;
  }
  if (region_out) HIP_TRY(ctx, hipMemcpyAsync(region_out, pl->buf[B_REGRES].p, (size_t)pl->n_regions * sizeof(otg_region_result), hipMemcpyDeviceToHost, ctx->stream));
  if (alleles_out && pl->out_alleles) HIP_TRY(ctx, hipMemcpyAsync(alleles_out, pl->buf[B_OUTAL].p, (size_t)pl->out_alleles * sizeof(otg_allele), hipMemcpyDeviceToHost, ctx->stream));
  if (seq_out && pl->out_seq_bytes) HIP_TRY(ctx, hipMemcpyAsync(seq_out, pl->buf[B_OUTSEQ].p, pl->out_seq_bytes, hipMemcpyDeviceToHost, ctx->stream));
  if (labels_out) HIP_TRY(ctx, hipMemcpyAsync(labels_out, pl->buf[B_LABELS].p, (size_t)pl->n_reads * 4, hipMemcpyDeviceToHost, ctx->stream));
  HIP_TRY(ctx, hipStreamSynchronize(ctx->stream));
  return OTG_OK;
}

int otg_assemble_device_results(otg_ctx* ctx, const otg_region_result** d_regions, const otg_allele** d_alleles, const uint8_t** d_seqs)
{
  if (!ctx || !ctx->pipe || !ctx->pipe->ran) return otg_fail(ctx, OTG_ERR_ARG, "otg_assemble_device_results: no completed run");
  Pipeline* pl = ctx->pipe;
  HIP_TRY(ctx, hipSetDevice(ctx->device));
  HIP_TRY(ctx, hipStreamSynchronize(ctx->stream));
  const bool empty = pl->n_regions == 0 || pl->n_reads == 0;
  if (d_regions) *d_regions = empty ? nullptr : (const otg_region_result*)pl->buf[B_REGRES].p;
  if (d_alleles) *d_alleles = (empty || !pl->out_alleles) ? nullptr : (const otg_allele*)pl->buf[B_OUTAL].p;
  if (d_seqs) *d_seqs = (empty || !pl->out_seq_bytes) ? nullptr : (const uint8_t*)pl->buf[B_OUTSEQ].p;
  return OTG_OK;
}

int otg_assemble_stats(otg_ctx* ctx, otg_run_stats* out)
{
  if (!ctx || !ctx->pipe || !out) return otg_fail(ctx, OTG_ERR_ARG, "otg_assemble_stats: no run");
  *out = ctx->pipe->stats;
  return OTG_OK;
}

}
```

otter_amd/csrc/poa.hip:

```cpp
#include "otg_common.hpp"
#include <vector>
#include <cstdlib>
#include <algorithm>

namespace {

struct NodeG { float hw; int32_t pred; uint32_t indeg; int32_t head; };
struct EdgeG { uint32_t sink; float w; int32_t next; uint32_t base; };
struct NodeL { float hw; int16_t pred; uint16_t indeg; int16_t head; uint16_t pad; };
struct EdgeL { uint16_t sink; uint16_t w; int16_t next; uint16_t base; };

struct PoaDev {
  const uint8_t* seq_arena;
  const uint8_t* cig_arena;
  const otg_poa_member* members;
  const otg_poa_graph* graphs;
  uint32_t n_graphs;
  const uint64_t* node_off;
  const uint64_t* edge_off;
  const uint64_t* wnode_off; const uint64_t* wedge_off; const uint64_t* wstart_off; const uint64_t* wanch_off;
  NodeG* nodes; uint8_t* node_base; uint8_t* is_end; uint32_t* bb_cnt; uint32_t* queue;
  EdgeG* edges;
  uint32_t* start_list;
  const uint64_t* out_off; uint32_t* out_len; uint8_t* out_arena; uint32_t* out_start; int32_t* status;
  const uint32_t* order;
  unsigned long long* prof;
  unsigned long long* prof_graph;
  uint32_t* fb_list;
  uint32_t* fb_count;
  int v2;
  int32_t* anext; int32_t* ahead; int32_t* atail; uint32_t* acnt;
};
struct PoaAux { int32_t* anext; int32_t* ahead; int32_t* atail; uint32_t* acnt; };

__global__ void poa_count_kernel(const uint8_t* __restrict__ cig_arena, const otg_poa_member* __restrict__ members,
                                 uint32_t n_members, uint32_t* __restrict__ n_alt, uint32_t* __restrict__ n_mrun)
{
  const uint32_t m = blockIdx.x * blockDim.x + threadIdx.x;
  if (m >= n_members) return;
  const uint8_t* c = cig_arena + members[m].cigar_off;
  const uint32_t n = members[m].cigar_len;
  uint32_t alt = 0, mrun = 0;
  uint8_t prev = 0;
  for (uint32_t i = 0; i < n; ++i) {
    const uint8_t op = c[i];
    alt += (op == 'X' || op == 'I');
    mrun += (op == 'M' && prev != 'M');
    prev = op;
  }
  n_alt[m] = alt; n_mrun[m] = mrun;
}

#define OTG_LDS __attribute__((address_space(3)))
template <bool LDS> struct PoaStore;
template <> struct PoaStore<false> {
  NodeG* nodes; EdgeG* edges;
  uint8_t *nbase, *isend; uint32_t *bbc, *queue, *starts;
  uint32_t node_cap, edge_cap; bool reduced;
  __device__ __forceinline__ NodeG ldN(uint32_t i) const { return nodes[i]; }
  __device__ __forceinline__ void stN(uint32_t i, const NodeG& n) const { nodes[i] = n; }
  __device__ __forceinline__ void stList(uint32_t i, int head, int tail) const { nodes[i].head = head; nodes[i].pred = tail; }
  __device__ __forceinline__ void stTail(uint32_t i, int tail) const { nodes[i].pred = tail; }
  __device__ __forceinline__ void stPred(uint32_t i, int pr) const { nodes[i].pred = pr; }
  __device__ __forceinline__ void incIndeg(uint32_t i) const { nodes[i].indeg = nodes[i].indeg + 1u; }
  __device__ __forceinline__ void incIndegAtomic(uint32_t i) const { atomicAdd(&nodes[i].indeg, 1u); }
  __device__ __forceinline__ float ldHw(uint32_t i) const { return nodes[i].hw; }
  __device__ __forceinline__ void stHw(uint32_t i, float w) const { nodes[i].hw = w; }
  __device__ __forceinline__ void stHwPred(uint32_t i, float w, int pr) const { nodes[i].hw = w; nodes[i].pred = pr; }
  __device__ __forceinline__ int ldPred(uint32_t i) const { return nodes[i].pred; }
  __device__ __forceinline__ EdgeG ldE(int e) const { return edges[e]; }
  __device__ __forceinline__ void stE(int e, const EdgeG& x) const { edges[e] = x; }
  __device__ __forceinline__ void stEw(int e, float w) const { edges[e].w = w; }
  __device__ __forceinline__ void stEnext(int e, int nx) const { edges[e].next = nx; }
  __device__ __forceinline__ uint32_t ldEbase(int e) const { return edges[e].base; }
  __device__ __forceinline__ void stIndeg(uint32_t i, uint32_t v) const { nodes[i].indeg = v; }
};
template <> struct PoaStore<true> {
  OTG_LDS NodeL* nodes; OTG_LDS EdgeL* edges;
  OTG_LDS uint8_t *nbase, *isend; OTG_LDS uint16_t *bbc, *queue, *starts;
  uint32_t node_cap, edge_cap; bool reduced;
  __device__ __forceinline__ NodeG ldN(uint32_t i) const { NodeG n; n.hw = nodes[i].hw; n.pred = nodes[i].pred; n.indeg = nodes[i].indeg; n.head = nodes[i].head; return n; }
  __device__ __forceinline__ void stN(uint32_t i, const NodeG& n) const { nodes[i].hw = n.hw; nodes[i].pred = (int16_t)n.pred; nodes[i].indeg = (uint16_t)n.indeg; nodes[i].head = (int16_t)n.head; }
  __device__ __forceinline__ void stList(uint32_t i, int head, int tail) const { nodes[i].head = (int16_t)head; nodes[i].pred = (int16_t)tail; }
  __device__ __forceinline__ void stTail(uint32_t i, int tail) const { nodes[i].pred = (int16_t)tail; }
  __device__ __forceinline__ void stPred(uint32_t i, int pr) const { nodes[i].pred = (int16_t)pr; }
  __device__ __forceinline__ void incIndeg(uint32_t i) const { nodes[i].indeg = (uint16_t)(nodes[i].indeg + 1u); }
  __device__ __forceinline__ void incIndegAtomic(uint32_t i) const { incIndeg(i); }
  __device__ __forceinline__ float ldHw(uint32_t i) const { return nodes[i].hw; }
  __device__ __forceinline__ void stHw(uint32_t i, float w) const { nodes[i].hw = w; }
  __device__ __forceinline__ void stHwPred(uint32_t i, float w, int pr) const { nodes[i].hw = w; nodes[i].pred = (int16_t)pr; }
  __device__ __forceinline__ int ldPred(uint32_t i) const { return nodes[i].pred; }
  __device__ __forceinline__ EdgeG ldE(int e) const { EdgeG x; x.sink = edges[e].sink; x.w = (float)edges[e].w; x.next = edges[e].next; x.base = edges[e].base; return x; }
  __device__ __forceinline__ void stE(int e, const EdgeG& x) const { edges[e].sink = (uint16_t)x.sink; edges[e].w = (uint16_t)x.w; edges[e].next = (int16_t)x.next; edges[e].base = (uint16_t)x.base; }
  __device__ __forceinline__ void stEw(int e, float w) const { edges[e].w = (uint16_t)w; }
  __device__ __forceinline__ void stEnext(int e, int nx) const { edges[e].next = (int16_t)nx; }
  __device__ __forceinline__ uint32_t ldEbase(int e) const { return edges[e].base; }
  __device__ __forceinline__ void stIndeg(uint32_t i, uint32_t v) const { nodes[i].indeg = (uint16_t)v; }
};

template <bool LDS> __device__ __forceinline__ void poa_phase_fence()
{
  if (LDS) { __builtin_amdgcn_fence(__ATOMIC_ACQ_REL, "wavefront"); __builtin_amdgcn_wave_barrier(); }
  else __threadfence();
}

using lds_u32 = __attribute__((address_space(3))) uint32_t;
using lds_i32 = __attribute__((address_space(3))) int32_t;
using lds_f32 = __attribute__((address_space(3))) float;
constexpr int POA_WK = 8;
struct PoaScratch {
  volatile lds_u32* ops;
  volatile lds_u32* stage;
  volatile lds_f32* hw;
  volatile lds_i32* pred;
};

__device__ __forceinline__ uint32_t poa_wave_excl_sum(uint32_t v, int lane, uint32_t* total)
{
  (void)lane;
  int x = (int)v;
  x += __builtin_amdgcn_update_dpp(0, x, 0x111, 0xf, 0xf, false);
  x += __builtin_amdgcn_update_dpp(0, x, 0x112, 0xf, 0xf, false);
  x += __builtin_amdgcn_update_dpp(0, x, 0x114, 0xf, 0xf, false);
  x += __builtin_amdgcn_update_dpp(0, x, 0x118, 0xf, 0xf, false);
  x += __builtin_amdgcn_update_dpp(0, x, 0x142, 0xa, 0xf, false);
  x += __builtin_amdgcn_update_dpp(0, x, 0x143, 0xc, 0xf, false);
  *total = (uint32_t)__builtin_amdgcn_readlane(x, 63);
  return (uint32_t)x - v;
}
__device__ __forceinline__ void poa_lds_order() { asm volatile("s_waitcnt lgkmcnt(0)" ::: "memory"); __builtin_amdgcn_wave_barrier(); }
__device__ __forceinline__ float poa_readlane_f(float v, int l) { return __int_as_float(__builtin_amdgcn_readlane(__float_as_int(v), l)); }

template <bool LDS>
__device__ __forceinline__ bool poa_graph_body(const PoaDev& P, const uint32_t g, const PoaStore<LDS>& S, const uint32_t out_cap,
                                               const PoaAux& X, const PoaScratch& L, const bool v2_in)
{
  const int lane = threadIdx.x & 63;
  const otg_poa_graph G = P.graphs[g];
  const uint32_t node_cap = S.node_cap, edge_cap = S.edge_cap;
  auto nbase = S.nbase; auto isend = S.isend; auto bbc = S.bbc; auto queue = S.queue; auto starts = S.starts;
  const int B = (int)G.backbone_len;
  const bool V2 = !LDS && v2_in && B >= 2;
  constexpr int WK = POA_WK;
  int* bdiff = (int*)(void*)&queue[0];
  uint32_t n_nodes = (uint32_t)B, n_edges = 0, n_start = B >= 2 ? 1u : 0u;
  int status = 0;
  bool tree_ok = true;
  const unsigned long long lt = (1ull << lane) - 1ull;
  const unsigned long long t0 = P.prof ? wall_clock64() : 0ull;
  unsigned long long pf_wide = 0, pf_wide_ops = 0, pf_narrow = 0, pf_serial = 0, pf_follow = 0, pf_sM = 0, pf_sX = 0, pf_sI = 0, pf_sD = 0, pf_snom = 0, pf_sirr = 0, pf_shead = 0;
  unsigned long long tq_serial = 0, tq_layout = 0, tq_mid = 0, tq_a = 0, tq_turn = 0, tq_c = 0, tq_mark = 0;
  auto tick = [&](unsigned long long& acc) { if (P.prof) { const unsigned long long now = wall_clock64(); acc += now - tq_mark; tq_mark = now; } };

  {
    const uint8_t* bb = P.seq_arena + G.backbone_off;
    for (uint32_t i = (uint32_t)lane; i < node_cap; i += 64) {
      const bool isb = (int)i < B && B >= 2;
      nbase[i] = isb ? bb[i] : (uint8_t)0;
      isend[i] = (isb && i >= 1 && B - (int)i <= 10) ? 1 : 0;
      NodeG n; n.hw = 0.0f; n.pred = -1; n.indeg = (isb && i >= 1) ? 1u : 0u; n.head = -1;
      S.stN(i, n);
      bbc[i] = 0;
      if (V2) queue[i] = 0;
    }
    if (V2) for (int i = lane; i <= B; i += 64) { X.ahead[i] = -1; X.atail[i] = -1; X.acnt[i] = 0u; }
    if (B >= 2) starts[0] = 0;
    poa_phase_fence<LDS>();
  }

  uint32_t cn_id = 0xffffffffu; int cn_head = -1, cn_tail = -1;
  int cur_anc = 0;
  auto node_lists = [&](uint32_t x, int& head, int& tail) {
    if (x == cn_id) { head = cn_head; tail = cn_tail; }
    else { const NodeG n = S.ldN(x); head = n.head; tail = n.pred; }
  };
  auto new_node = [&](uint8_t base) -> uint32_t {
    if (n_nodes >= node_cap) { status = 1; return n_nodes - 1; }
    nbase[n_nodes] = base;
    cn_id = n_nodes; cn_head = -1; cn_tail = -1;
    return n_nodes++;
  };
  auto append_edge = [&](uint32_t src, int src_head, int src_tail, uint32_t sink, uint32_t sink_base) {
    if (n_edges >= edge_cap) { status = 2; return; }
    const int e = (int)n_edges++;
    EdgeG x; x.sink = sink; x.w = 1.0f; x.next = -1; x.base = V2 ? (sink_base | (src << 8)) : sink_base;
    S.stE(e, x);
    if (src_tail >= 0) { S.stEnext(src_tail, e); S.stTail(src, e); } else { src_head = e; S.stList(src, e, e); }
    if (src == cn_id) { cn_head = src_head; cn_tail = e; }
    if (V2) {
      X.anext[e] = -1;
      if ((int)sink >= B) S.stIndeg(sink, (uint32_t)(e + 1));
      if (cur_anc < -1 || cur_anc >= B || ((int)src < B && (int)src != cur_anc)) tree_ok = false;
      else {
        const int t = X.atail[cur_anc + 1];
        if (t >= 0) X.anext[t] = e; else X.ahead[cur_anc + 1] = e;
        X.atail[cur_anc + 1] = e;
        X.acnt[cur_anc + 1] = X.acnt[cur_anc + 1] + 1u;
      }
    }
  };
  auto insert_edge = [&](uint32_t src, int src_head, int src_tail, uint32_t sink) {
    if ((int)src < B - 1 && sink == src + 1) { bbc[src] = bbc[src] + 1; return; }
    for (int e = src_head; e >= 0;) {
      const EdgeG x = S.ldE(e);
      if (x.sink == sink) { S.stEw(e, x.w + 1.0f); return; }
      e = x.next;
    }
    if ((int)sink >= B) tree_ok = false;
    append_edge(src, src_head, src_tail, sink, (int)sink >= B ? (uint32_t)nbase[sink] : 0u);
  };
  int as_edge = -1;
  auto alt_step = [&](uint32_t prev, int prev_head, int prev_tail, uint8_t tc) -> uint32_t {
    for (int e = prev_head; e >= 0;) {
      const EdgeG x = S.ldE(e);
      if ((int)x.sink >= B && (x.base & 0xffu) == (uint32_t)tc) { S.stEw(e, x.w + 1.0f); as_edge = e; return x.sink; }
      e = x.next;
    }
    as_edge = -1;
    const uint32_t nn = new_node(tc);
    if (!status) append_edge(prev, prev_head, prev_tail, nn, tc);
    return nn;
  };

  const uint8_t* seq = nullptr; const uint8_t* cig = nullptr;
  int clen = 0, slen = 0;
  bool spl = false, spr = false;
  auto set_member = [&](const uint32_t mi) {
    const otg_poa_member M = P.members[G.first_member + mi];
    seq = P.seq_arena + M.seq_off; cig = P.cig_arena + M.cigar_off;
    clen = (int)M.cigar_len; slen = (int)M.seq_len;
    spl = M.spanning_l != 0; spr = M.spanning_r != 0;
  };
  auto par_runs = [&](const bool lead, const int p0, const int ref0, const int nv) {
      uint32_t n_newn = 0, n_newe = 0, pv = 0, last_ex = 0;
      int ph = -1, pt = -1, ltl = -1, r = 0, r_miss = 0, jmiss = -1, r_close = -1, anc = 0;
      bool missed = false, close_new = false, closed = false;
      if (lead) {
        anc = ref0 - 1; pv = (uint32_t)anc; r = ref0;
        { const NodeG na = S.ldN(pv); ph = na.head; pt = na.pred; }
        for (int j = p0; j < nv; ++j) {
          const uint32_t o = L.ops[j];
          const int op = (int)(o & 0xffu);
          const uint32_t tc = (o >> 8) & 0xffu;
          if (op == 'M') { closed = true; r_close = r; break; }
          if (op == 'D') { r += 1; if (!missed && B - r <= 10 && spr) isend[pv] = 1; continue; }
          if (!missed) {
            bool found = false;
            for (int e = ph; e >= 0;) {
              const EdgeG x = S.ldE(e);
              if ((int)x.sink >= B && (x.base & 0xffu) == tc) { S.stEw(e, x.w + 1.0f); pv = x.sink; found = true; break; }
              e = x.next;
            }
            if (found) { const NodeG nn = S.ldN(pv); ph = nn.head; pt = nn.pred; }
            else { missed = true; jmiss = j; r_miss = r; last_ex = pv; ltl = pt; }
          }
          if (missed) ++n_newn;
          if (op == 'X') r += 1;
          if (!missed && B - r <= 10 && spr) isend[pv] = 1;
        }
        if (closed) {
          if (!missed) {
            if ((int)pv < B - 1 && r_close == (int)pv + 1) bbc[pv] = bbc[pv] + 1;
            else {
              bool found = false;
              for (int e = ph; e >= 0;) {
                const EdgeG x = S.ldE(e);
                if ((int)x.sink == r_close) { S.stEw(e, x.w + 1.0f); found = true; break; }
                e = x.next;
              }
              if (!found) { close_new = true; last_ex = pv; ltl = pt; }
            }
          }
          if (B - (r_close + 1) <= 10 && spr) isend[r_close] = 1;
        }
        n_newe = n_newn + ((closed && (missed || close_new)) ? 1u : 0u);
      }
      tick(tq_a);
      tick(tq_turn);
      uint32_t tot_n = 0, tot_e = 0;
      const uint32_t nb = n_nodes + poa_wave_excl_sum(n_newn, lane, &tot_n);
      const uint32_t eb = n_edges + poa_wave_excl_sum(n_newe, lane, &tot_e);
      if (n_nodes + tot_n > node_cap) status = 1;
      else if (n_edges + tot_e > edge_cap) status = 2;
      if (!status) {
        if (lead && n_newe) {
          uint32_t src = last_ex, k = 0;
          if (missed) {
            int r2 = r_miss;
            for (int j = jmiss; j < nv; ++j) {
              const uint32_t o = L.ops[j];
              const int op = (int)(o & 0xffu);
              const uint32_t tc = (o >> 8) & 0xffu;
              if (op == 'M') break;
              if (op == 'D') { r2 += 1; if (B - r2 <= 10 && spr) isend[src] = 1; continue; }
              const uint32_t id = nb + k;
              const int ein = (int)(eb + k);
              const bool has_out = k + 1u < n_newe;
              nbase[id] = (uint8_t)tc;
              EdgeG x; x.sink = id; x.w = 1.0f; x.next = -1; x.base = tc | (src << 8);
              S.stE(ein, x);
              X.anext[ein] = has_out ? ein + 1 : -1;
              NodeG nn; nn.hw = 0.0f; nn.pred = has_out ? ein + 1 : -1; nn.indeg = (uint32_t)(ein + 1); nn.head = has_out ? ein + 1 : -1;
              S.stN(id, nn);
              src = id; ++k;
              if (op == 'X') r2 += 1;
              if (B - r2 <= 10 && spr) isend[id] = 1;
            }
          }
          if (closed && (missed || close_new)) {
            const int ec = (int)(eb + k);
            EdgeG x; x.sink = (uint32_t)r_close; x.w = 1.0f; x.next = -1; x.base = src << 8;
            S.stE(ec, x);
            X.anext[ec] = -1;
          }
          if (ltl >= 0) { S.stEnext(ltl, (int)eb); S.stTail(last_ex, (int)eb); } else S.stList(last_ex, (int)eb, (int)eb);
          const int t = X.atail[anc + 1];
          if (t >= 0) X.anext[t] = (int)eb; else X.ahead[anc + 1] = (int)eb;
          X.atail[anc + 1] = (int)(eb + n_newe - 1u);
          X.acnt[anc + 1] = X.acnt[anc + 1] + n_newe;
        }
        n_nodes += tot_n; n_edges += tot_e;
      }
      cn_id = 0xffffffffu;
  };
  int pre_ci = -1; int pre_cc[WK];
#pragma unroll
  for (int k = 0; k < WK; ++k) pre_cc[k] = 0;
  auto wide_chunk = [&](const int ci0, const int ref0, const int tgt0, int& nv_out, int& totr_out, int& tott_out, int& lastop_out) -> bool {
    const int rem = clen - ci0;
    const int rem4 = rem < 64 * WK ? rem : 64 * WK;
    const int o0 = WK * lane;
    int cc[WK];
    if (P.prof) tq_mark = wall_clock64();
    if (pre_ci == ci0) {
#pragma unroll
      for (int k = 0; k < WK; ++k) cc[k] = o0 + k < rem4 ? pre_cc[k] : 0;
    } else {
#pragma unroll
      for (int k = 0; k < WK; ++k) cc[k] = o0 + k < rem4 ? (int)cig[ci0 + o0 + k] : 0;
    }
    int nv = rem4;
    if (rem > 64 * WK) {
      int lm = -1;
#pragma unroll
      for (int k = 0; k < WK; ++k) if (cc[k] == 'M') lm = o0 + k;
      lm = otg_wave_max_i32(lm);
      if (lm < 0) return false;
      nv = lm + 1;
    }
    uint32_t totr = 0, tott = 0, totl = 0;
    int refk[WK], tgtk[WK]; bool simk[WK], leadk[WK];
    uint32_t li = 0;
    for (int attempt = 0; attempt < 2; ++attempt) {
// ... 192 lines not shown
          if (k == 0) S.stList((uint32_t)prev, ein, ein);
          if (V2) X.anext[ein] = (has_out && anc_ok) ? ein + 1 : -1;
          if (B - (ref_at + (isX ? 1 : 0)) <= 10 && spr) isend[id] = 1;
        }
        if (V2) {
          if (!anc_ok) tree_ok = false;
          else {
            const int e0 = (int)n_edges, t = X.atail[cur_anc + 1];
            if (t >= 0) X.anext[t] = e0; else X.ahead[cur_anc + 1] = e0;
            X.atail[cur_anc + 1] = e0 + run - 1;
            X.acnt[cur_anc + 1] = X.acnt[cur_anc + 1] + (uint32_t)run;
          }
        }
        n_nodes += (uint32_t)run; n_edges += (uint32_t)run;
        prev = (int)n_nodes - 1;
        cn_id = (uint32_t)prev; cn_head = -1; cn_tail = -1;
        if (run > 1) todo &= ~(((1ull << (run - 1)) - 1ull) << (l + 1));
        pf_follow += (unsigned long long)run;
        return true;
      };
      while (todo && !status) {
        const int l = (int)__builtin_ctzll(todo);
        todo &= todo - 1ull;
        bool stepped = false;
        if (P.prof) { const int o_ = __builtin_amdgcn_readlane(c, l); pf_sM += o_ == 'M'; pf_sX += o_ == 'X'; pf_sI += o_ == 'I'; pf_sD += o_ == 'D'; }
        const int op = __builtin_amdgcn_readlane(c, l), pop = __builtin_amdgcn_readlane(pc, l);
        const int r = __builtin_amdgcn_readlane(ref_at, l);
        const uint8_t tc = (uint8_t)__builtin_amdgcn_readlane(tb, l);
        bool have_lists = false;
        int ph = -1, pt = -1;
        if (pop == 'M') {
          prev = r - 1; first = false; cur_anc = prev;
          if (r >= 1 && r <= B) { ph = __builtin_amdgcn_readlane(pf_head, l); pt = __builtin_amdgcn_readlane(pf_tail, l); have_lists = true; }
        }
        int ref_after = r;
        if (op == 'M') {
          if (first || prev == r) first = false;
          else if ((uint32_t)prev >= n_nodes || (uint32_t)r >= n_nodes) { status = 3; break; }
          else {
            if (!((int)prev < B - 1 && r == prev + 1) && !have_lists) node_lists((uint32_t)prev, ph, pt);
            insert_edge((uint32_t)prev, ph, pt, (uint32_t)r);
          }
          prev = r; ref_after = r + 1; cur_anc = prev;
        } else if (op == 'X') {
          if (first) {
            bool need_new = true;
            for (uint32_t q = 0; q < n_start; ++q) if (nbase[starts[q]] == tc) { need_new = false; break; }
            if (need_new) { prev = (int)new_node(tc); starts[n_start++] = (uint32_t)prev; cur_anc = -1; }
            first = false;
          } else if ((uint32_t)prev >= n_nodes) { status = 3; break; }
          else if (create_chain(l)) continue;
          else {
            if (!have_lists) node_lists((uint32_t)prev, ph, pt);
            prev = (int)alt_step((uint32_t)prev, ph, pt, tc);
            stepped = true;
          }
          ref_after = r + 1;
        } else if (op == 'D') {
          ref_after = r + 1;
          if (first) { prev = ref_after; cur_anc = prev; }
        } else if (op == 'I') {
          if (first) { prev = (int)new_node(tc); starts[n_start++] = (uint32_t)prev; first = false; cur_anc = -1; }
          else if ((uint32_t)prev >= n_nodes) { status = 3; break; }
          else if (create_chain(l)) continue;
          else {
            if (!have_lists) node_lists((uint32_t)prev, ph, pt);
            prev = (int)alt_step((uint32_t)prev, ph, pt, tc);
            stepped = true;
          }
        }
        if (B - ref_after <= 10 && spr && (uint32_t)prev < node_cap) isend[prev] = 1;
        if (stepped && !status) follow_chain(l);
      }
      }
      lastop = __builtin_amdgcn_readlane(c, nvalid - 1);
      if (P.prof) tq_serial += wall_clock64() - ts0;
      ref_i += __builtin_popcountll(mMXD); tgt += __builtin_popcountll(mMXI);
      if (lastop == 'M') { prev = ref_i - 1; first = false; cur_anc = prev; }
      ci += nvalid;
    }
  }
  poa_phase_fence<LDS>();
  if (V2 && !status) {
    int carry = 0;
    for (int b0 = 0; b0 < B; b0 += 64) {
      const int i = b0 + lane;
      const int d = i < B ? bdiff[i] : 0;
      uint32_t tot = 0;
      const int run = carry + (int)poa_wave_excl_sum((uint32_t)d, lane, &tot) + d;
      if (i < B && run) bbc[i] = bbc[i] + (uint32_t)run;
      carry += (int)tot;
    }
    poa_phase_fence<LDS>();
  }
  if (LDS && S.reduced && (status == 1 || status == 2)) return false;
  const unsigned long long t1 = P.prof ? wall_clock64() : 0ull;

  const float c_ = G.c, t_ = G.t;
  auto damp = [&](float w) -> float {
    const float t_applied = t_ * w;
    const float final_weight = c_ > t_applied ? c_ : t_applied;
    return w - final_weight;
  };
  uint32_t qh = 0, qt = 0;
  if (!status && V2 && tree_ok) {
    for (uint32_t i = (uint32_t)lane; i < n_nodes; i += 64) {
      int pr = -1;
      if ((int)i >= B) { const int ie = (int)S.ldN(i).indeg - 1; if (ie >= 0) pr = (int)(S.ldEbase(ie) >> 8); }
      NodeG n; n.hw = 0.0f; n.pred = pr; n.indeg = 0u; n.head = -1;
      S.stN(i, n);
    }
    L.hw[lane] = 0.0f; L.hw[lane + 64] = 0.0f; L.pred[lane] = -1; L.pred[lane + 64] = -1;
    poa_phase_fence<LDS>();
    __builtin_amdgcn_wave_barrier();
    int wb = 0;
    auto relax = [&](uint32_t v, float cand, int u) {
      if ((int)v < wb + 128) {
        const int ix = (int)(v & 127u);
        const float h = L.hw[ix]; const int pr = L.pred[ix];
        if (pr < 0 || cand > h || (cand == h && u < pr)) { L.hw[ix] = cand; L.pred[ix] = u; }
      } else {
        const NodeG nv = S.ldN(v);
        if (nv.pred < 0 || cand > nv.hw || (cand == nv.hw && u < nv.pred)) S.stHwPred(v, cand, u);
      }
    };
    auto window_to = [&](int u) {
      while (u >= wb + 64) {
        const int i0 = wb + lane;
        if (i0 < B) S.stHwPred((uint32_t)i0, L.hw[i0 & 127], L.pred[i0 & 127]);
        wb += 64;
        const int i1 = wb + 64 + lane;
        float h = 0.0f; int pr = -1;
        if (i1 < B) { const NodeG t = S.ldN((uint32_t)i1); h = t.hw; pr = t.pred; }
        L.hw[i1 & 127] = h; L.pred[i1 & 127] = pr;
        poa_lds_order();
      }
    };
    auto sweep_block = [&](int ai0, int nA, int T, uint32_t off, uint32_t cnt, bool bb_step) {
      uint32_t sink = 0, src = 0; float w = 0.0f, hsg = 0.0f, val = 0.0f; int sp = -1;
      if (lane < T) { const int e = (int)L.stage[lane]; const EdgeG x = S.ldE(e); sink = x.sink; w = x.w; src = x.base >> 8; if ((int)src >= B) sp = -2; }
      for (int k = 0; k < T; ++k) {
        const uint32_t sk = (uint32_t)__builtin_amdgcn_readlane((int)sink, k);
        if (sp == -2 && src == sk && k < lane) sp = k;
      }
      if (lane < T && sp == -2) hsg = S.ldHw(src);
      float bbw = 0.0f;
      if (lane < nA) { const int u = ai0 + lane - 1; if (u >= 0 && u < B - 1) bbw = (float)bbc[u]; }
      for (int a = 0; a < nA; ++a) {
        const int u = ai0 + a - 1;
        float hw_u = 0.0f;
        if (u >= 0) {
          window_to(u);
          hw_u = L.hw[u & 127];
          if (bb_step && u < B - 1) relax((uint32_t)(u + 1), hw_u + damp(1.0f + poa_readlane_f(bbw, a)), u);
        }
        const int o = __builtin_amdgcn_readlane((int)off, a), cn = __builtin_amdgcn_readlane((int)cnt, a);
        for (int j = o; j < o + cn; ++j) {
          const uint32_t sk = (uint32_t)__builtin_amdgcn_readlane((int)sink, j), sid = (uint32_t)__builtin_amdgcn_readlane((int)src, j);
          const int spk = __builtin_amdgcn_readlane(sp, j);
          const float wk = poa_readlane_f(w, j);
          const float hs = spk == -1 ? hw_u : (spk >= 0 ? poa_readlane_f(val, spk) : poa_readlane_f(hsg, j));
          const float cand = hs + damp(wk);
          if (lane == j) val = cand;
          if ((int)sk < B) relax(sk, cand, (int)sid);
        }
      }
      if (lane < T && (int)sink >= B) S.stHw(sink, val);
    };
    int ai = 0;
    while (ai <= B) {
      const int aidx = ai + lane;
      const uint32_t cnt = aidx <= B ? X.acnt[aidx] : 0u;
      uint32_t tot = 0;
      const uint32_t off = poa_wave_excl_sum(cnt, lane, &tot);
      const unsigned long long fits = __ballot(aidx <= B && off + cnt <= 64u);
      const int nA = (~fits) ? (int)__builtin_ctzll(~fits) : 64;
      if (nA == 0) {
        const uint32_t c0 = (uint32_t)__builtin_amdgcn_readlane((int)cnt, 0);
        int e = X.ahead[ai];
        bool first_piece = true;
        for (uint32_t done = 0; done < c0;) {
          const uint32_t T = c0 - done < 64u ? c0 - done : 64u;
          if (lane == 0) for (uint32_t k = 0; k < T; ++k) { L.stage[k] = (uint32_t)e; e = X.anext[e]; }
          e = __builtin_amdgcn_readfirstlane(e);
          poa_lds_order();
          sweep_block(ai, 1, (int)T, 0u, lane == 0 ? T : 0u, first_piece);
          __threadfence();
          first_piece = false; done += T;
        }
        ai += 1;
        continue;
      }
      const int T = __builtin_amdgcn_readlane((int)(off + cnt), nA - 1);
      if (lane < nA) { int e = X.ahead[aidx]; for (uint32_t k = 0; k < cnt; ++k) { L.stage[off + k] = (uint32_t)e; e = X.anext[e]; } }
      poa_lds_order();
      sweep_block(ai, nA, T, off, cnt, true);
      ai += nA;
    }
    for (int h2 = 0; h2 < 2; ++h2) { const int i0 = wb + 64 * h2 + lane; if (i0 < B) S.stHwPred((uint32_t)i0, L.hw[i0 & 127], L.pred[i0 & 127]); }
  } else
  if (!status) {
    for (uint32_t i = (uint32_t)lane; i < n_nodes; i += 64) { S.stPred(i, -1); if (V2 && (int)i >= B) S.stIndeg(i, 0u); }
    poa_phase_fence<LDS>();
    if (LDS) { for (uint32_t e = 0; e < n_edges; ++e) S.incIndeg(S.ldE((int)e).sink); }
    else { for (uint32_t e = (uint32_t)lane; e < n_edges; e += 64) S.incIndegAtomic(S.ldE((int)e).sink); }
    poa_phase_fence<LDS>();
    for (uint32_t b0 = 0; b0 < n_nodes; b0 += 64) {
      const uint32_t i = b0 + (uint32_t)lane;
      const bool z = i < n_nodes && S.ldN(i).indeg == 0;
      const unsigned long long zm = __ballot(z);
      if (z) queue[qt + __builtin_popcountll(zm & lt)] = i;
      qt += (uint32_t)__builtin_popcountll(zm);
    }
    poa_phase_fence<LDS>();
    uint32_t pushed_val = 0, pushed_at = 0xffffffffu;
    NodeG rv; rv.hw = 0.0f; rv.pred = -1; rv.indeg = 0; rv.head = -1;
    uint32_t rv_id = 0xffffffffu;
    auto relax_into = [&](uint32_t u, float hw_u, uint32_t v, float w) {
      NodeG nv = v == rv_id ? rv : S.ldN(v);
      const float cand = hw_u + w;
      if (nv.pred < 0) { nv.hw = cand; nv.pred = (int32_t)u; }
      else if (cand > nv.hw || (cand == nv.hw && (int32_t)u < nv.pred)) { nv.hw = cand; nv.pred = (int32_t)u; }
      nv.indeg = nv.indeg - 1u;
      S.stN(v, nv);
      rv = nv; rv_id = v;
      if (nv.indeg == 0) { queue[qt] = v; pushed_val = v; pushed_at = qt; ++qt; }
    };
    while (qh < qt) {
      const uint32_t u = qh == pushed_at ? pushed_val : (uint32_t)queue[qh];
      ++qh;
      const NodeG nu = u == rv_id ? rv : S.ldN(u);
      if ((int)u < B - 1) relax_into(u, nu.hw, u + 1, damp(1.0f + (float)bbc[u]));
      for (int e = nu.head; e >= 0;) {
        const EdgeG x = S.ldE(e);
        relax_into(u, nu.hw, x.sink, damp(x.w));
        e = x.next;
      }
    }
    if (qt != n_nodes) status = 4;
  }
  const unsigned long long t2 = P.prof ? wall_clock64() : 0ull;
  uint32_t len = 0, startpos = 0;
  if (!status && n_nodes > 0) {
    poa_phase_fence<LDS>();
    float bw = 0.0f; uint32_t bi = 0xffffffffu;
    for (uint32_t i = (uint32_t)lane; i < n_nodes; i += 64) {
      if (isend[i]) { const float w = S.ldHw(i); if (bi == 0xffffffffu || w > bw) { bw = w; bi = i; } }
    }
    for (int off = 32; off > 0; off >>= 1) {
      const float ow = __shfl_xor(bw, off); const uint32_t oi = (uint32_t)__shfl_xor((int)bi, off);
      if (oi != 0xffffffffu && (bi == 0xffffffffu || ow > bw || (ow == bw && oi < bi))) { bw = ow; bi = oi; }
    }
    const uint32_t h_node = bi == 0xffffffffu ? 0u : bi;
    uint8_t* out = P.out_arena + P.out_off[g];
    const uint32_t cap = out_cap;
    int32_t cur = (int32_t)h_node;
    if (LDS) {
      uint32_t k = 0;
      while (cur >= 0 && k < cap && k < node_cap) {
        const uint8_t b = nbase[cur];
        if (b) queue[k++] = b;
        cur = S.ldPred((uint32_t)cur);
      }
      poa_phase_fence<LDS>();
      for (uint32_t j = (uint32_t)lane; j < k; j += 64) out[cap - 1 - j] = (uint8_t)queue[j];
      startpos = cap - k; len = k;
    } else {
      uint32_t pos = cap;
      while (cur >= 0 && pos > 0) {
        if (cur < B) {
          const int base0 = cur >= 63 ? cur - 63 : 0;
          const int my = base0 + lane;
          int mypred = -1, myb = 0;
          if (my <= cur) { mypred = S.ldPred((uint32_t)my); myb = (int)nbase[my]; }
          while (cur >= base0 && cur < B && pos > 0) {
            const int l = cur - base0;
            const int b = __builtin_amdgcn_readlane(myb, l);
            if (b) out[--pos] = (uint8_t)b;
            cur = __builtin_amdgcn_readlane(mypred, l);
          }
        } else {
          const uint8_t b = nbase[cur];
          if (b) out[--pos] = b;
          cur = S.ldPred((uint32_t)cur);
        }
      }
      startpos = pos; len = cap - pos;
    }
  }
  if (P.prof && lane == 0) {
    const unsigned long long t3 = wall_clock64();
    atomicAdd(P.prof + 0, t1 - t0); atomicAdd(P.prof + 1, t2 - t1); atomicAdd(P.prof + 2, t3 - t2); atomicAdd(P.prof + 3, 1ull);
    atomicAdd(P.prof + 4, (unsigned long long)n_nodes); atomicAdd(P.prof + 5, (unsigned long long)n_edges); atomicAdd(P.prof + 6, (unsigned long long)B);
    if (LDS) atomicAdd(P.prof + 7, 1ull);
    atomicAdd(P.prof + 8, pf_wide); atomicAdd(P.prof + 9, pf_wide_ops); atomicAdd(P.prof + 10, pf_narrow); atomicAdd(P.prof + 11, pf_serial);
    atomicMax(P.prof + 12, t1 - t0); atomicMax(P.prof + 13, t3 - t0);
    if (P.prof_graph) { unsigned long long* q = P.prof_graph + 9 * (size_t)g; q[0] = t1 - t0; q[1] = pf_wide; q[2] = pf_narrow; q[3] = pf_serial; q[4] = tq_serial | (pf_follow << 40); q[5] = (unsigned long long)G.n_members | ((unsigned long long)B << 32); q[6] = pf_sM | (pf_sX << 32); q[7] = pf_sI | (pf_sD << 32); q[8] = pf_snom | (pf_shead << 20) | (pf_sirr << 40); }
    atomicAdd(P.prof + 27, tq_layout); atomicAdd(P.prof + 28, tq_mid); atomicAdd(P.prof + 29, tq_a); atomicAdd(P.prof + 30, tq_turn); atomicAdd(P.prof + 31, tq_c); atomicAdd(P.prof + 20, tq_serial);
  }
  P.out_len[g] = len; P.out_start[g] = startpos; P.status[g] = status;
  return true;
}

constexpr uint32_t POA_LDS_NODE_B = 18, POA_LDS_EDGE_B = 8;
__global__ __launch_bounds__(64) void poa_graph_lds_kernel(PoaDev P, const uint32_t* __restrict__ list, uint32_t lds_bytes)
{
  extern __shared__ __attribute__((aligned(16))) uint8_t s_graph[];
  const int lane = threadIdx.x & 63;
  const uint32_t g = list[blockIdx.x];
  if (g >= P.n_graphs) return;
  const otg_poa_graph G = P.graphs[g];
  const uint32_t ncap_true = (uint32_t)(P.node_off[g + 1] - P.node_off[g]), ecap_true = (uint32_t)(P.edge_off[g + 1] - P.edge_off[g]);
  const uint32_t B = G.backbone_len, nm = G.n_members;
  const uint32_t start_b = (2u * (nm + 2u) + 7u) & ~7u;
  bool fits = lds_bytes > start_b + 64u && ncap_true < 32768u && ecap_true < 32768u && nm < 32768u;
  uint32_t N = 0, E = 0;
  bool reduced = false;
  if (fits) {
    const uint32_t avail = lds_bytes - start_b - 32u;
    const float estN = (float)B + 0.5f * (float)(ncap_true - B) + 4.0f, estE = 0.5f * (float)ecap_true + 4.0f;
    const float f = (float)avail / ((float)POA_LDS_NODE_B * estN + (float)POA_LDS_EDGE_B * estE);
    N = (uint32_t)(estN * f) & ~3u; E = (uint32_t)(estE * f) & ~1u;
    if (N >= ncap_true) { N = ncap_true; E = ((avail - POA_LDS_NODE_B * N) / POA_LDS_EDGE_B) & ~1u; }
    if (E >= ecap_true) { E = ecap_true; const uint32_t n2 = ((avail - POA_LDS_EDGE_B * E) / POA_LDS_NODE_B) & ~3u; N = n2 < ncap_true ? n2 : ncap_true; }
    reduced = N < ncap_true || E < ecap_true;
    fits = N >= B + 2u && f >= 1.0f;
  }
  if (!fits) {
    if (lane == 0) { const uint32_t k = atomicAdd(P.fb_count, 1u); P.fb_list[k] = g; }
    return;
  }
  PoaStore<true> S;
  uint32_t o = 0;
  S.nodes = (OTG_LDS NodeL*)(s_graph + o); o += 12u * N;
  S.edges = (OTG_LDS EdgeL*)(s_graph + o); o += 8u * E;
  S.bbc = (OTG_LDS uint16_t*)(s_graph + o); o += 2u * N;
  S.queue = (OTG_LDS uint16_t*)(s_graph + o); o += 2u * N;
  S.nbase = (OTG_LDS uint8_t*)(s_graph + o); o += N;
  S.isend = (OTG_LDS uint8_t*)(s_graph + o); o += N;
  o = (o + 3u) & ~3u;
  S.starts = (OTG_LDS uint16_t*)(s_graph + o);
  S.node_cap = N; S.edge_cap = E; S.reduced = reduced;
  if (!poa_graph_body<true>(P, g, S, ncap_true, PoaAux{}, PoaScratch{}, false)) {
    if (lane == 0) { const uint32_t k = atomicAdd(P.fb_count, 1u); P.fb_list[k] = g; }
  }
}

#ifndef OTG_POA_WPEU
#define OTG_POA_WPEU 4
#endif
__global__ __launch_bounds__(64, OTG_POA_WPEU) void poa_graph_wave_kernel(PoaDev P, const uint32_t* __restrict__ list, const uint32_t* __restrict__ count_ptr,
                                                               uint32_t count_imm)
{
  __shared__ uint32_t s_ops[64 * POA_WK], s_stage[64];
  __shared__ float s_hw[128];
  __shared__ int32_t s_pred[128];
  const uint32_t n = count_ptr ? *count_ptr : count_imm;
  for (uint32_t k = blockIdx.x; k < n; k += gridDim.x) {
    const uint32_t g = list[k];
    if (g >= P.n_graphs) continue;
    const uint64_t no = P.wnode_off[g], eo = P.wedge_off[g];
    PoaStore<false> S;
    S.nodes = P.nodes + no; S.edges = P.edges + eo;
    S.nbase = P.node_base + no; S.isend = P.is_end + no; S.bbc = P.bb_cnt + no; S.queue = P.queue + no;
    S.starts = P.start_list + P.wstart_off[g];
    S.node_cap = (uint32_t)(P.node_off[g + 1] - P.node_off[g]); S.edge_cap = (uint32_t)(P.edge_off[g + 1] - P.edge_off[g]); S.reduced = false;
    PoaAux X;
    X.anext = P.anext + eo;
    { const uint64_t ao = P.v2 ? P.wanch_off[g] : 0ull; X.ahead = P.ahead + ao; X.atail = P.atail + ao; X.acnt = P.acnt + ao; }
    PoaScratch L;
    L.ops = (volatile lds_u32*)&s_ops[0]; L.stage = (volatile lds_u32*)&s_stage[0]; L.hw = (volatile lds_f32*)&s_hw[0]; L.pred = (volatile lds_i32*)&s_pred[0];
    poa_graph_body<false>(P, g, S, S.node_cap, X, L, P.v2 != 0);
  }
}

}

int otg_launch_poa(otg_ctx* ctx, const uint8_t* d_seq_arena, const uint8_t* d_cig_arena,
                   const otg_poa_member* d_members, uint32_t n_members, const otg_poa_graph* d_graphs,
                   const otg_poa_graph* h_graphs, uint32_t n_graphs, uint32_t* d_out_len,
                   std::vector<uint64_t>& node_off)
{
  if (n_graphs == 0) return OTG_OK;
  uint32_t* d_alt = (uint32_t*)otg_slot(ctx, SLOT_P20, (size_t)(n_members + 1) * sizeof(uint32_t));
  uint32_t* d_nonm = (uint32_t*)otg_slot(ctx, SLOT_P21, (size_t)(n_members + 1) * sizeof(uint32_t));
  if (!d_alt || !d_nonm) return OTG_ERR_HIP;
  std::vector<uint32_t> h_alt(n_members), h_nonm(n_members);
  if (n_members) {
    hipLaunchKernelGGL(poa_count_kernel, dim3((n_members + 255) / 256), dim3(256), 0, ctx->stream, d_cig_arena, d_members, n_members, d_alt, d_nonm);
    HIP_TRY(ctx, hipMemcpyAsync(h_alt.data(), d_alt, (size_t)n_members * sizeof(uint32_t), hipMemcpyDeviceToHost, ctx->stream));
    HIP_TRY(ctx, hipMemcpyAsync(h_nonm.data(), d_nonm, (size_t)n_members * sizeof(uint32_t), hipMemcpyDeviceToHost, ctx->stream));
    HIP_TRY(ctx, hipStreamSynchronize(ctx->stream));
  }
  std::vector<uint64_t> edge_off(n_graphs + 1), start_off(n_graphs + 1);
  node_off.assign(n_graphs + 1, 0);
  node_off[0] = edge_off[0] = start_off[0] = 0;
  for (uint32_t g = 0; g < n_graphs; ++g) {
    uint64_t alt = 0, mrun = 0;
    for (uint32_t m = 0; m < h_graphs[g].n_members; ++m) { alt += h_alt[h_graphs[g].first_member + m]; mrun += h_nonm[h_graphs[g].first_member + m]; }
    node_off[g + 1] = node_off[g] + (((uint64_t)h_graphs[g].backbone_len + alt + 2 + 3) & ~3ull);
    edge_off[g + 1] = edge_off[g] + ((alt + mrun + 2 + 1) & ~1ull);
    start_off[g + 1] = start_off[g] + h_graphs[g].n_members + 2;
  }
  const uint64_t NN = node_off[n_graphs];
  PoaDev P;
  P.seq_arena = d_seq_arena; P.cig_arena = d_cig_arena; P.members = d_members; P.graphs = d_graphs; P.n_graphs = n_graphs;
  static const bool poa_v1 = getenv("OTG_POA_V1") != nullptr;
  P.v2 = poa_v1 ? 0 : 1;
  for (uint32_t g = 0; g < n_graphs && P.v2; ++g)
    if (node_off[g + 1] - node_off[g] >= (1ull << 24) - 2) P.v2 = 0;
  static const bool no_lds = getenv("OTG_POA_NO_LDS") != nullptr;
  uint32_t lds_bytes = 0, n_lds = 0, n_glob = 0;
  std::vector<uint32_t> order;
  {
    std::vector<uint32_t> est(n_graphs, 0u), live;
    live.reserve(n_graphs);
    for (uint32_t g = 0; g < n_graphs; ++g) {
      if (h_graphs[g].backbone_len == 0 && h_graphs[g].n_members == 0) continue;
      const double B = (double)h_graphs[g].backbone_len, ncap = (double)(node_off[g + 1] - node_off[g]), ecap = (double)(edge_off[g + 1] - edge_off[g]);
      const double need = (double)POA_LDS_NODE_B * (B + 0.5 * (ncap - B) + 4.0) + (double)POA_LDS_EDGE_B * (0.5 * ecap + 4.0) + (double)((2u * (h_graphs[g].n_members + 2u) + 7u) & ~7u) + 32.0 + 64.0;
      est[g] = need > 4.0e9 ? 0xffffffffu : (uint32_t)need;
      live.push_back(g);
    }
    if (!live.empty() && !no_lds) {
      std::vector<uint32_t> e2(live.size());
      for (size_t i = 0; i < live.size(); ++i) e2[i] = est[live[i]];
      const size_t k = (size_t)((double)(live.size() - 1) * 0.97);
      std::nth_element(e2.begin(), e2.begin() + k, e2.end());
      if (e2[k] <= 16u * 1024u) lds_bytes = std::max<uint32_t>((e2[k] + 511u) & ~511u, 4096u);
    }
    auto heavier = [&](uint32_t a, uint32_t b) {
      const uint64_t wa = (edge_off[a + 1] - edge_off[a]) + (node_off[a + 1] - node_off[a]), wb = (edge_off[b + 1] - edge_off[b]) + (node_off[b + 1] - node_off[b]);
      return wa != wb ? wa > wb : a < b;
    };
    order.reserve(live.size());
    for (uint32_t g : live) if (lds_bytes && est[g] <= lds_bytes) order.push_back(g);
    n_lds = (uint32_t)order.size();
    for (uint32_t g : live) if (!(lds_bytes && est[g] <= lds_bytes)) order.push_back(g);
    n_glob = (uint32_t)order.size() - n_lds;
    std::sort(order.begin(), order.begin() + n_lds, heavier);
    std::sort(order.begin() + n_lds, order.end(), heavier);
  }
  static const size_t piece_budget_cfg = getenv("OTG_POA_PIECE_MB") ? (size_t)atoll(getenv("OTG_POA_PIECE_MB")) << 20 : (size_t)24 << 30;
  size_t piece_budget = piece_budget_cfg;
  {
    size_t free_b = 0, total_b = 0, held = 0;
    HIP_TRY(ctx, hipMemGetInfo(&free_b, &total_b));
    for (int sl : {SLOT_P3, SLOT_P4, SLOT_P6, SLOT_P7, SLOT_P8, SLOT_P9, SLOT_P10, SLOT_P11, SLOT_P12, SLOT_P13, SLOT_P16}) held += ctx->pool[sl].cap;
    piece_budget = std::min(piece_budget, std::max<size_t>((size_t)1 << 30, (free_b + held) / 2));
  }
  struct Piece { uint32_t k0, k1; bool lds; };
  std::vector<Piece> pieces;
  std::vector<uint64_t> wnode(n_graphs + 1, 0), wedge(n_graphs + 1, 0), wstart(n_graphs + 1, 0), wanch(n_graphs + 1, 0);
  uint64_t maxN = 0, maxE = 0, maxS = 0, maxA = 0;
  {
    auto cut = [&](uint32_t k0, uint32_t k1, bool lds) {
      uint32_t p0 = k0;
      uint64_t cn = 0, ce = 0, cs = 0, ca = 0;
      for (uint32_t k = k0; k < k1; ++k) {
        const uint32_t g = order[k];
        const uint64_t nc = node_off[g + 1] - node_off[g], ec = edge_off[g + 1] - edge_off[g], sc = start_off[g + 1] - start_off[g];
        const uint64_t ac = ((uint64_t)h_graphs[g].backbone_len + 2 + 3) & ~3ull;
        const uint64_t bytes = (cn + nc) * (sizeof(NodeG) + 10) + (ce + ec) * (sizeof(EdgeG) + 4) + (cs + sc) * 4 + (ca + ac) * 12;
        if (k > p0 && bytes > piece_budget) { pieces.push_back({p0, k, lds}); p0 = k; cn = ce = cs = ca = 0; }
        wnode[g] = cn; wedge[g] = ce; wstart[g] = cs; wanch[g] = ca;
        cn += nc; ce += ec; cs += sc; ca += ac;
        maxN = std::max(maxN, cn); maxE = std::max(maxE, ce); maxS = std::max(maxS, cs); maxA = std::max(maxA, ca);
      }
      if (k1 > p0) pieces.push_back({p0, k1, lds});
    };
    cut(n_lds, n_lds + n_glob, false);
    cut(0, n_lds, true);
  }
  uint64_t* d_node_off = (uint64_t*)otg_slot(ctx, SLOT_P0, (size_t)(n_graphs + 1) * sizeof(uint64_t));
  uint64_t* d_edge_off = (uint64_t*)otg_slot(ctx, SLOT_P1, (size_t)(n_graphs + 1) * sizeof(uint64_t));
  uint64_t* d_woff = (uint64_t*)otg_slot(ctx, SLOT_P2, (size_t)4 * (n_graphs + 1) * sizeof(uint64_t));
  P.node_base = (uint8_t*)otg_slot(ctx, SLOT_P3, maxN);
  P.is_end = (uint8_t*)otg_slot(ctx, SLOT_P4, maxN);
  P.nodes = (NodeG*)otg_slot(ctx, SLOT_P6, maxN * sizeof(NodeG));
  P.bb_cnt = (uint32_t*)otg_slot(ctx, SLOT_P9, maxN * 4);
  P.queue = (uint32_t*)otg_slot(ctx, SLOT_P12, maxN * 4);
  P.edges = (EdgeG*)otg_slot(ctx, SLOT_P13, maxE * sizeof(EdgeG));
  P.start_list = (uint32_t*)otg_slot(ctx, SLOT_P16, maxS * 4);
  P.out_arena = (uint8_t*)otg_slot(ctx, SLOT_P17, NN);
  P.out_start = (uint32_t*)otg_slot(ctx, SLOT_P29, (size_t)n_graphs * 4);
  P.status = (int32_t*)otg_slot(ctx, SLOT_P28, (size_t)n_graphs * 4);
  P.anext = nullptr; P.ahead = nullptr; P.atail = nullptr; P.acnt = nullptr;
  if (P.v2) {
    P.anext = (int32_t*)otg_slot(ctx, SLOT_P7, maxE * 4);
    P.ahead = (int32_t*)otg_slot(ctx, SLOT_P8, maxA * 4);
    P.atail = (int32_t*)otg_slot(ctx, SLOT_P10, maxA * 4);
    P.acnt = (uint32_t*)otg_slot(ctx, SLOT_P11, maxA * 4);
    if (!P.anext || !P.ahead || !P.atail || !P.acnt) return OTG_ERR_HIP;
  }
  uint32_t* d_order = (uint32_t*)otg_slot(ctx, SLOT_P18, (size_t)(n_graphs + 1) * sizeof(uint32_t));
  if (!d_node_off || !d_edge_off || !d_woff || !P.node_base || !P.is_end || !P.nodes || !P.bb_cnt || !P.queue ||
      !P.edges || !P.start_list || !P.out_arena || !P.out_start || !P.status || !d_order)
    return OTG_ERR_HIP;
  P.node_off = d_node_off; P.edge_off = d_edge_off;
  P.wnode_off = d_woff; P.wedge_off = d_woff + (n_graphs + 1); P.wstart_off = d_woff + 2 * (size_t)(n_graphs + 1); P.wanch_off = d_woff + 3 * (size_t)(n_graphs + 1);
  P.out_off = d_node_off;
  P.out_len = d_out_len;
  P.order = d_order;
  if (!order.empty()) HIP_TRY(ctx, hipMemcpyAsync(d_order, order.data(), order.size() * sizeof(uint32_t), hipMemcpyHostToDevice, ctx->stream));
  HIP_TRY(ctx, hipMemsetAsync(d_out_len, 0, (size_t)n_graphs * sizeof(uint32_t), ctx->stream));
  HIP_TRY(ctx, hipMemsetAsync(P.out_start, 0, (size_t)n_graphs * sizeof(uint32_t), ctx->stream));
  HIP_TRY(ctx, hipMemsetAsync(P.status, 0, (size_t)n_graphs * sizeof(int32_t), ctx->stream));
  HIP_TRY(ctx, hipMemcpyAsync(d_node_off, node_off.data(), (size_t)(n_graphs + 1) * sizeof(uint64_t), hipMemcpyHostToDevice, ctx->stream));
  HIP_TRY(ctx, hipMemcpyAsync(d_edge_off, edge_off.data(), (size_t)(n_graphs + 1) * sizeof(uint64_t), hipMemcpyHostToDevice, ctx->stream));
  HIP_TRY(ctx, hipMemcpyAsync(d_woff, wnode.data(), (size_t)(n_graphs + 1) * sizeof(uint64_t), hipMemcpyHostToDevice, ctx->stream));
  HIP_TRY(ctx, hipMemcpyAsync(d_woff + (n_graphs + 1), wedge.data(), (size_t)(n_graphs + 1) * sizeof(uint64_t), hipMemcpyHostToDevice, ctx->stream));
  HIP_TRY(ctx, hipMemcpyAsync(d_woff + 2 * (size_t)(n_graphs + 1), wstart.data(), (size_t)(n_graphs + 1) * sizeof(uint64_t), hipMemcpyHostToDevice, ctx->stream));
  HIP_TRY(ctx, hipMemcpyAsync(d_woff + 3 * (size_t)(n_graphs + 1), wanch.data(), (size_t)(n_graphs + 1) * sizeof(uint64_t), hipMemcpyHostToDevice, ctx->stream));
  HIP_TRY(ctx, hipStreamSynchronize(ctx->stream));
  static const bool profile = getenv("OTG_POA_PROFILE") != nullptr;
  P.prof = nullptr; P.prof_graph = nullptr;
  if (profile) {
    P.prof_graph = (unsigned long long*)otg_slot(ctx, SLOT_P23, (size_t)n_graphs * 9 * sizeof(unsigned long long));
    if (!P.prof_graph) return OTG_ERR_HIP;
    HIP_TRY(ctx, hipMemsetAsync(P.prof_graph, 0, (size_t)n_graphs * 9 * sizeof(unsigned long long), ctx->stream));
    P.prof = (unsigned long long*)otg_slot(ctx, SLOT_P19, 32 * sizeof(unsigned long long));
    if (!P.prof) return OTG_ERR_HIP;
    HIP_TRY(ctx, hipMemsetAsync(P.prof, 0, 32 * sizeof(unsigned long long), ctx->stream));
  }
  P.fb_list = (uint32_t*)otg_slot(ctx, SLOT_P22, (size_t)(n_graphs + 1) * sizeof(uint32_t));
  if (!P.fb_list) return OTG_ERR_HIP;
  P.fb_count = P.fb_list + n_graphs;
  for (const Piece& pc : pieces) {
    const uint32_t n = pc.k1 - pc.k0;
    if (!pc.lds) hipLaunchKernelGGL(poa_graph_wave_kernel, dim3(n), dim3(64), 0, ctx->stream, P, P.order + pc.k0, (const uint32_t*)nullptr, n);
    else {
      HIP_TRY(ctx, hipMemsetAsync(P.fb_count, 0, sizeof(uint32_t), ctx->stream));
      hipLaunchKernelGGL(poa_graph_lds_kernel, dim3(n), dim3(64), lds_bytes, ctx->stream, P, P.order + pc.k0, lds_bytes);
      const uint32_t fg = n < (uint32_t)ctx->n_cu * 32 ? n : (uint32_t)ctx->n_cu * 32;
      hipLaunchKernelGGL(poa_graph_wave_kernel, dim3(fg), dim3(64), 0, ctx->stream, P, (const uint32_t*)P.fb_list, (const uint32_t*)P.fb_count, 0u);
    }
  }
  HIP_TRY(ctx, hipGetLastError());
  if (profile) {
    unsigned long long h[32];
    HIP_TRY(ctx, hipStreamSynchronize(ctx->stream));
    HIP_TRY(ctx, hipMemcpy(h, P.prof, sizeof(h), hipMemcpyDeviceToHost));
    const double n = h[3] ? (double)h[3] : 1.0;
    fprintf(stderr, "[otg] poa profile: %u LDS + %u global launches; %llu graphs done (%llu in LDS, %u bytes each), per graph: insert %.1f us, sweep %.1f us, emit %.1f us; nodes %.0f (backbone %.0f), edges %.0f\n",
            n_lds, n_glob, h[3], h[7], lds_bytes, h[0] / n / 100.0, h[1] / n / 100.0, h[2] / n / 100.0, h[4] / n, h[6] / n, h[5] / n);
    fprintf(stderr, "[otg] poa profile: threading chunks per graph: %.1f wide (%.0f ops each), %.1f narrow one-lane-per-run, %.1f serial; slowest graph: insert %.1f us, whole %.1f us\n",
            h[8] / n, h[8] ? (double)h[9] / (double)h[8] : 0.0, h[10] / n, h[11] / n, h[12] / 100.0, h[13] / 100.0);
    { const double nw = h[8] ? (double)h[8] : 1.0;
      fprintf(stderr, "[otg] poa profile: a wide chunk, us: layout %.2f, bases + marks + staging %.2f, subtree walk %.2f, ids %.2f, chains %.2f; narrow + serial code per graph %.1f us\n",
              h[27] / nw / 100.0, h[28] / nw / 100.0, h[29] / nw / 100.0, h[30] / nw / 100.0, h[31] / nw / 100.0, h[20] / n / 100.0); }
    {
      std::vector<unsigned long long> pg((size_t)n_graphs * 9);
      HIP_TRY(ctx, hipMemcpy(pg.data(), P.prof_graph, pg.size() * sizeof(unsigned long long), hipMemcpyDeviceToHost));
      std::vector<uint32_t> idx(n_graphs);
      for (uint32_t g = 0; g < n_graphs; ++g) idx[g] = g;
      const size_t top = std::min<size_t>(5, n_graphs);
      std::partial_sort(idx.begin(), idx.begin() + top, idx.end(), [&](uint32_t a, uint32_t b) { return pg[9 * (size_t)a] > pg[9 * (size_t)b]; });
      for (size_t t = 0; t < top; ++t) {
        const unsigned long long* q = &pg[9 * (size_t)idx[t]];
        fprintf(stderr, "[otg] poa profile: slow graph %u: %llu members on a backbone of %llu, threading %.1f us = %llu wide + %llu narrow + %llu serial chunks; %.1f us in the narrow + serial code (%llu steps taken as a retraced chain)\n",
                idx[t], q[5] & 0xffffffffull, q[5] >> 32, q[0] / 100.0, q[1], q[2], q[3], (q[4] & ((1ull << 40) - 1ull)) / 100.0, q[4] >> 40);
        fprintf(stderr, "[otg] poa profile:   its serial code: %llu windows without an 'M', %llu member heads, %llu others; ops taken one by one: %llu M, %llu X, %llu I, %llu D\n",
                q[8] & 0xfffffull, (q[8] >> 20) & 0xfffffull, q[8] >> 40, q[6] & 0xffffffffull, q[6] >> 32, q[7] & 0xffffffffull, q[7] >> 32);
      }
    }
  }
  return OTG_OK;
}
```

Before: 17530.

## Plan POA layout on device and batch pipeline scans and readbacks

Adds a device-side POA planning path (count kernels, scans, histogram-based LDS sizing, piece cutting). It replaces the host round trips that copied graph descriptors and per-member counts back, computed offsets on the CPU and uploaded them again. The two allele-length scans become one two-block wave-shuffle scan launch instead of serial single-block kernels. Todo-list appends in the pair and reassign kernels use one wave-aggregated atomic instead of one atomic per lane, and the pair loop is flattened over a triangular index. The final flag, stats and region-result readbacks are merged into async copies with a single sync. The cost is extra complexity, plus a host fallback path that stays available behind environment variables.

```diff
diff --git a/otter_amd/csrc/otg_common.hpp b/otter_amd/csrc/otg_common.hpp
--- a/otter_amd/csrc/otg_common.hpp
+++ b/otter_amd/csrc/otg_common.hpp
@@ -279,6 +279,8 @@
                    const otg_poa_member* d_members, uint32_t n_members, const otg_poa_graph* d_graphs,
                    const otg_poa_graph* h_graphs, uint32_t n_graphs, uint32_t* d_out_len,
                    std::vector<uint64_t>& node_off);
+int otg_launch_poa_resident(otg_ctx* ctx, const uint8_t* d_seq_arena, const uint8_t* d_cig_arena,
+                            const otg_poa_member* d_members, uint32_t n_members, const otg_poa_graph* d_graphs, uint32_t n_graphs, uint32_t* d_out_len);
 
 int otg_genotype_resident(otg_ctx* ctx, const otg_params* params, const uint8_t* d_arena, const uint64_t* d_off, const uint32_t* d_len,
                           const uint32_t* d_first, const uint32_t* d_n, const uint32_t* h_n_alleles, uint32_t n_regions, const uint64_t* d_poff,
diff --git a/otter_amd/csrc/otg_scan.hpp b/otter_amd/csrc/otg_scan.hpp
--- a/otter_amd/csrc/otg_scan.hpp
+++ b/otter_amd/csrc/otg_scan.hpp
@@ -50,4 +50,65 @@
     if (total) *total = carry_s;
   }
 }
+
+struct OtgScanJob {
+  const void* in = nullptr;
+  const uint32_t* idx = nullptr;
+  const uint32_t* first_ptr = nullptr;
+  const uint32_t* n_ptr = nullptr;
+  uint64_t* out = nullptr;
+  uint64_t* total = nullptr;
+  uint32_t n = 0;
+  uint32_t in_u64 = 0;
+  uint32_t write_end = 0;
+};
+constexpr uint32_t OTG_SCAN_MAX_JOBS = 8;
+struct OtgScanJobs { OtgScanJob j[OTG_SCAN_MAX_JOBS]; };
+
+template <uint32_t ITEMS>
+__global__ void __launch_bounds__(1024) otg_scan_jobs_kernel(OtgScanJobs J)
+{
+  constexpr uint32_t T = 1024;
+  __shared__ uint64_t wave_sum[T / 64];
+  const OtgScanJob& job = J.j[blockIdx.x];
+  const uint32_t t = threadIdx.x, lane = t & 63u, wv = t >> 6;
+  const uint32_t n = job.n_ptr ? *job.n_ptr : job.n;
+  const uint32_t* idx = job.idx ? job.idx + (job.first_ptr ? *job.first_ptr : 0u) : nullptr;
+  const uint32_t* in32 = (const uint32_t*)job.in;
+  const uint64_t* in64 = (const uint64_t*)job.in;
+  uint64_t carry = 0;
+  for (uint32_t base = 0; base < n; base += ITEMS * T) {
+    uint64_t v[ITEMS];
+    uint32_t at[ITEMS];
+    uint64_t sum = 0;
+#pragma unroll
+    for (uint32_t k = 0; k < ITEMS; ++k) {
+      const uint32_t i = base + t * ITEMS + k;
+      at[k] = i < n ? (idx ? idx[i] : i) : 0u;
+      v[k] = i < n ? (job.in_u64 ? in64[at[k]] : (uint64_t)in32[at[k]]) : 0ull;
+      sum += v[k];
+    }
+    uint64_t x = sum;
+#pragma unroll
+    for (uint32_t d = 1; d < 64; d <<= 1) { const uint64_t y = __shfl_up(x, d); if (lane >= d) x += y; }
+    if (lane == 63) wave_sum[wv] = x;
+    __syncthreads();
+    uint64_t before = 0, all = 0;
+#pragma unroll
+    for (uint32_t w = 0; w < T / 64; ++w) { const uint64_t s = wave_sum[w]; if (w < wv) before += s; all += s; }
+    uint64_t run = carry + before + x - sum;
+#pragma unroll
+    for (uint32_t k = 0; k < ITEMS; ++k) {
+      const uint32_t i = base + t * ITEMS + k;
+      if (i < n) job.out[at[k]] = run;
+      run += v[k];
+    }
+    carry += all;
+    __syncthreads();
+  }
+  if (t == 0) {
+    if (job.write_end) job.out[n] = carry;
+    if (job.total) *job.total = carry;
+  }
+}
 #endif
diff --git a/otter_amd/csrc/pipeline.hip b/otter_amd/csrc/pipeline.hip
--- a/otter_amd/csrc/pipeline.hip
+++ b/otter_amd/csrc/pipeline.hip
@@ -1,5 +1,6 @@
 #include "otg_chain.hpp"
 #include "myers_masks.hpp"
+#include "otg_scan.hpp"
 #include <algorithm>
 #include <chrono>
 #include <cmath>
@@ -43,10 +44,12 @@
   B_CLLAB, B_IC, B_FC, B_BOUNDS, B_CLERR, B_LABELS,
   B_REDIST, B_RTASKS, B_RKIND, B_CIGLEN, B_CIG,
   B_ALLELES, B_GRAPHS, B_MEMBERS, B_POALEN,
-  B_ALLEN, B_ALOFF, B_ALIDX, B_OUTSEQ, B_OUTAL, B_REGRES, B_STATS, B_SCAN_TMP, B_TOTALS,
+  B_ALLEN, B_ALOFF, B_ALIDX, B_OUTSEQ, B_OUTAL, B_REGRES, B_SCAN_TMP, B_TOTALS,
   B_MASKS, B_MASK_FIRST, B_MASK_READ, B_MASK_TASK,
   B_COUNT
 };
+
+constexpr uint32_t RUN_FLAGS_WORD = 40, RUN_STATS_WORD = 44;
 
 static void* pbuf(otg_ctx* ctx, Pipeline* pl, int i, size_t bytes)
 {
@@ -220,6 +223,14 @@
   status[r] = st; n_valid[r] = (st == OTG_REGION_OK) ? nv : 0; ign[r] = lig;
 }
 
+__device__ __forceinline__ void todo_append(uint32_t* __restrict__ todo, uint32_t* __restrict__ n_todo, bool has, uint32_t slot)
+{
+  const unsigned long long m = __ballot(has);
+  if (!m) return;
+  const uint32_t at = otg_wave_atomic_add(n_todo, (uint32_t)__popcll(m));
+  if (has) todo[at + __builtin_amdgcn_mbcnt_hi((uint32_t)(m >> 32), __builtin_amdgcn_mbcnt_lo((uint32_t)m, 0u))] = slot;
+}
+
 __global__ void K_pair_tasks(const uint8_t* __restrict__ arena, const otg_read* __restrict__ reads,
                              const otg_region* __restrict__ regions, uint32_t n_regions, const uint32_t* __restrict__ n_valid,
                              const int32_t* __restrict__ ign, const uint32_t* __restrict__ valid,
@@ -235,26 +246,36 @@
     const uint64_t base = dist_off[r];
     const size_t np = (size_t)n * (n - 1) / 2;
     if (max_alleles == 1) { for (size_t q = threadIdx.x; q < np; q += blockDim.x) dist[base + q] = 1.0; continue; }
-    for (int i = 0; i < n - 1; ++i) {
-      const uint32_t xi = valid[f + i];
-      const otg_read x = reads[xi];
-      for (int j = i + 1 + (int)threadIdx.x; j < n; j += (int)blockDim.x) {
-        const uint32_t yi = valid[f + j];
+    const bool haps = !ign[r];
+    for (size_t q0 = 0; q0 < np; q0 += blockDim.x) {
+      const size_t q = q0 + threadIdx.x;
+      const bool in = q < np;
+      const uint64_t slot = base + q;
+      bool has = false;
+      if (in) {
+        int i = (int)(((double)(2 * n - 1) - sqrt((double)(2 * n - 1) * (double)(2 * n - 1) - 8.0 * (double)q)) * 0.5);
+        if (i < 0) i = 0;
+        if (i > n - 2) i = n - 2;
+        while (i > 0 && didx(n, i, i + 1) > q) --i;
+        while (i < n - 2 && didx(n, i + 1, i + 2) <= q) ++i;
+        const int j = i + 1 + (int)(q - didx(n, i, i + 1));
+        const uint32_t xi = valid[f + i], yi = valid[f + j];
+        const otg_read x = reads[xi];
         const otg_read y = reads[yi];
-        const uint64_t slot = base + didx(n, i, j);
-        if (!ign[r]) {
+        if (haps) {
           const bool bx = x.ps >= 0 && x.hp >= 0, by = y.ps >= 0 && y.hp >= 0;
           dist[slot] = (bx && by && x.ps == y.ps && x.hp == y.hp) ? 0.0 : 1.0;
         } else {
           double known = 0;
           uint32_t d = 1;
           if (anreads_task(arena, x, y, tasks[slot], &d, &known)) {
-            den[slot] = d; todo[atomicAdd(n_todo, 1u)] = (uint32_t)slot;
+            den[slot] = d; has = true;
             if (task_blk) task_blk[slot] = task_mask_block(read_blk, tasks[slot], x, xi, y, yi);
           }
           else dist[slot] = known;
         }
       }
+      todo_append(todo, n_todo, has, (uint32_t)slot);
     }
   }
 }
@@ -344,19 +365,23 @@
     for (int i = 0; i < n; ++i) {
       if (labels[f + i] >= 0) continue;
       const otg_read x = reads[f + i];
-      for (int j = (int)threadIdx.x; j < n; j += (int)blockDim.x) {
-        if (j == i) continue;
-        const otg_read y = reads[f + j];
-        if (!(y.spanning_l && y.spanning_r)) continue;
-        if (labels[f + j] < 0 && j > i) continue;
-        const uint64_t slot = re_off[r] + (uint64_t)i * n + j;
-        double known = 0;
-        uint32_t d = 1;
-        if (anreads_task(arena, x, y, tasks[slot], &d, &known, rev_base)) {
-          den[slot] = d; todo[atomicAdd(n_todo, 1u)] = (uint32_t)slot;
-          if (task_blk) task_blk[slot] = task_mask_block(read_blk, tasks[slot], x, f + (uint32_t)i, y, f + (uint32_t)j);
+      for (int j0 = 0; j0 < n; j0 += (int)blockDim.x) {
+        const int j = j0 + (int)threadIdx.x;
+        const uint64_t slot = re_off[r] + (uint64_t)i * n + (uint64_t)j;
+        bool has = false;
+        if (j < n && j != i) {
+          const otg_read y = reads[f + j];
+          if (y.spanning_l && y.spanning_r && !(labels[f + j] < 0 && j > i)) {
+            double known = 0;
+            uint32_t d = 1;
+            if (anreads_task(arena, x, y, tasks[slot], &d, &known, rev_base)) {
+              den[slot] = d; has = true;
+              if (task_blk) task_blk[slot] = task_mask_block(read_blk, tasks[slot], x, f + (uint32_t)i, y, f + (uint32_t)j);
+            }
+            else dist[slot] = known;
+          }
         }
-        else dist[slot] = known;
+        todo_append(todo, n_todo, has, (uint32_t)slot);
       }
     }
   }
@@ -545,22 +570,6 @@
   al_len[i] = len; al_flag[i] = flag;
 }
 
-__global__ __launch_bounds__(1024) void K_scan(const uint32_t* __restrict__ in, uint64_t* __restrict__ out, uint32_t n, uint64_t* __restrict__ total)
-{
-  __shared__ uint64_t part[1024];
-  const uint32_t t = threadIdx.x;
-  const uint32_t chunk = (n + 1023) / 1024;
-  const uint32_t a = t * chunk, b = a + chunk < n ? a + chunk : n;
-  uint64_t s = 0;
-  for (uint32_t i = a; i < b; ++i) s += in[i];
-  part[t] = s;
-  __syncthreads();
-  if (t == 0) { uint64_t acc = 0; for (int i = 0; i < 1024; ++i) { const uint64_t v = part[i]; part[i] = acc; acc += v; } *total = acc; }
-  __syncthreads();
-  uint64_t acc = part[t];
-  for (uint32_t i = a; i < b; ++i) { out[i] = acc; acc += in[i]; }
-}
-
 __global__ void K_gather(const uint8_t* __restrict__ arena, const AlleleSlot* __restrict__ alleles, const uint32_t* __restrict__ al_len,
                          const uint32_t* __restrict__ al_flag, const uint64_t* __restrict__ al_off, const uint64_t* __restrict__ al_idx,
                          const uint32_t* __restrict__ read_region, const otg_region* __restrict__ regions, const int32_t* __restrict__ ic,
@@ -712,7 +721,7 @@
   const size_t ntask = std::max<size_t>(std::max<size_t>(pl->n_pair_slots, pl->n_re_slots), n_reads) + 1;
   if (!pbuf(ctx, pl, B_TASKS, ntask * sizeof(otg_align_task)) || !pbuf(ctx, pl, B_TODO, ntask * 4) || !pbuf(ctx, pl, B_SCORES, ntask * 4) ||
       !pbuf(ctx, pl, B_DEN, ntask * 4) || !pbuf(ctx, pl, B_CELLS, ntask * 8) || !pbuf(ctx, pl, B_DIST, (pl->n_pair_slots + 1) * 8) ||
-      !pbuf(ctx, pl, B_REDIST, (pl->n_re_slots + 1) * 8) || !pbuf(ctx, pl, B_CNT, 64 * 8) || !pbuf(ctx, pl, B_STATS, 64 * 8) ||
+      !pbuf(ctx, pl, B_REDIST, (pl->n_re_slots + 1) * 8) || !pbuf(ctx, pl, B_CNT, 64 * 8) ||
       !pbuf(ctx, pl, B_STATUS, (size_t)n_regions * 4 + 4) || !pbuf(ctx, pl, B_NVALID, (size_t)n_regions * 4 + 4) ||
       !pbuf(ctx, pl, B_IGNHAPS, (size_t)n_regions * 4 + 4) || !pbuf(ctx, pl, B_VALID, (size_t)n_reads * 4 + 4) ||
       !pbuf(ctx, pl, B_VPOS, (size_t)n_reads * 4 + 4) || !pbuf(ctx, pl, B_VLEN, (size_t)n_reads * 4 + 4) ||
@@ -802,7 +811,7 @@
   double* d_dist = (double*)B(B_DIST);
   double* d_redist = (double*)B(B_REDIST);
   uint32_t* d_cnt = (uint32_t*)B(B_CNT);
-  unsigned long long* d_stats = (unsigned long long*)B(B_STATS);
+  unsigned long long* d_stats = (unsigned long long*)(d_cnt + RUN_STATS_WORD);
   int32_t* d_status = (int32_t*)B(B_STATUS);
   uint32_t* d_nvalid = (uint32_t*)B(B_NVALID);
   int32_t* d_ign = (int32_t*)B(B_IGNHAPS);
@@ -824,7 +833,6 @@
   Timer total(ctx);
   HIP_TRY(ctx, hipMemcpyAsync(d_reads, pl->h_reads.data(), (size_t)NR * sizeof(otg_read), hipMemcpyHostToDevice, st));
   HIP_TRY(ctx, hipMemsetAsync(d_cnt, 0, 64 * 8, st));
-  HIP_TRY(ctx, hipMemsetAsync(d_stats, 0, 64 * 8, st));
   if (unsigned long long* visited = otg_affine_visited(ctx)) HIP_TRY(ctx, hipMemsetAsync(visited, 0, 8, st));
   const int TB = 256;
   const uint32_t gr_reads = (NR + TB - 1) / TB, gr_regions = (NG + TB - 1) / TB;
@@ -900,7 +908,6 @@
     pl->stats.ms_reassign = t.ms();
   }
   dbg(ctx, "reassign done");
-  std::vector<uint64_t> node_off;
   {
     Timer t(ctx);
     HIP_TRY(ctx, hipMemsetAsync(d_cig_len, 0, (size_t)NR * 4, st));
@@ -920,11 +927,7 @@
     pl->stats.ms_affine = t.ms();
     dbg(ctx, "affine done");
     Timer t2(ctx);
-    std::vector<otg_poa_graph> h_graphs(NR);
-    HIP_TRY(ctx, hipMemcpyAsync(h_graphs.data(), B(B_GRAPHS), (size_t)NR * sizeof(otg_poa_graph), hipMemcpyDeviceToHost, st));
-    HIP_TRY(ctx, hipStreamSynchronize(st));
-    rc = otg_launch_poa(ctx, d_arena, d_cig, (const otg_poa_member*)B(B_MEMBERS), NR, (const otg_poa_graph*)B(B_GRAPHS), h_graphs.data(), NR,
-                        (uint32_t*)B(B_POALEN), node_off);
+    rc = otg_launch_poa_resident(ctx, d_arena, d_cig, (const otg_poa_member*)B(B_MEMBERS), NR, (const otg_poa_graph*)B(B_GRAPHS), NR, (uint32_t*)B(B_POALEN));
     if (rc) return rc;
     pl->stats.ms_poa = t2.ms();
   }
@@ -937,8 +940,12 @@
     uint64_t* d_tot = (uint64_t*)B(B_TOTALS);
     hipLaunchKernelGGL(K_allele_len, dim3(gr_reads), dim3(TB), 0, st, (const AlleleSlot*)B(B_ALLELES), d_status, d_rr, (const uint32_t*)B(B_POALEN),
                        (const int32_t*)ctx->pool[SLOT_P28].p, NR, d_allen, d_alflag, d_status);
-    hipLaunchKernelGGL(K_scan, dim3(1), dim3(1024), 0, st, d_allen, d_aloff, NR, d_tot + 0);
-    hipLaunchKernelGGL(K_scan, dim3(1), dim3(1024), 0, st, d_alflag, d_alidx, NR, d_tot + 1);
+    {
+      OtgScanJobs sj;
+      sj.j[0].in = d_allen; sj.j[0].out = d_aloff; sj.j[0].n = NR; sj.j[0].total = d_tot + 0;
+      sj.j[1].in = d_alflag; sj.j[1].out = d_alidx; sj.j[1].n = NR; sj.j[1].total = d_tot + 1;
+      hipLaunchKernelGGL(otg_scan_jobs_kernel<8>, dim3(2), dim3(1024), 0, st, sj);
+    }
     uint64_t h_tot[2];
     HIP_TRY(ctx, hipMemcpyAsync(h_tot, d_tot, 16, hipMemcpyDeviceToHost, st));
     HIP_TRY(ctx, hipStreamSynchronize(st));
@@ -955,25 +962,29 @@
   }
   dbg(ctx, "gather done");
   HIP_TRY(ctx, hipGetLastError());
+  struct { uint32_t flags[RUN_STATS_WORD - RUN_FLAGS_WORD]; unsigned long long stats[8]; } tail;
+  static_assert(sizeof(tail) == (RUN_STATS_WORD - RUN_FLAGS_WORD) * 4 + 64, "the flags and the statistics words are one contiguous range");
+  unsigned long long h_visited = 0;
+  const unsigned long long* d_visited = otg_affine_visited(ctx);
+  std::vector<otg_region_result> rr(NG);
+  HIP_TRY(ctx, hipMemcpyAsync(&tail, d_cnt + RUN_FLAGS_WORD, sizeof(tail), hipMemcpyDeviceToHost, st));
+  if (d_visited) HIP_TRY(ctx, hipMemcpyAsync(&h_visited, d_visited, 8, hipMemcpyDeviceToHost, st));
+  HIP_TRY(ctx, hipMemcpyAsync(rr.data(), B(B_REGRES), (size_t)NG * sizeof(otg_region_result), hipMemcpyDeviceToHost, st));
   pl->stats.ms_total = total.ms();
   {
-    uint32_t hf[3];
-    HIP_TRY(ctx, hipMemcpy(hf, d_cnt + 40, sizeof(hf), hipMemcpyDeviceToHost));
+    const uint32_t* hf = tail.flags;
     if (hf[0]) return otg_fail(ctx, OTG_ERR_FATAL, "an edit-distance alignment did not complete on the device");
     if (hf[2]) return otg_fail(ctx, OTG_ERR_CAPACITY, "a flank re-alignment exhausted its backtrace storage on the device");
   }
-  unsigned long long hs[8];
-  HIP_TRY(ctx, hipMemcpy(hs, d_stats, sizeof(hs), hipMemcpyDeviceToHost));
+  const unsigned long long* hs = tail.stats;
   pl->stats.edit_cells = hs[0]; pl->stats.edit_seq_bytes = hs[1]; pl->stats.edit_tasks = hs[2];
   pl->stats.affine_cells = hs[4]; pl->stats.affine_seq_bytes = hs[5]; pl->stats.affine_tasks = hs[6];
   pl->stats.n_regions = NG;
-  if (const unsigned long long* visited = otg_affine_visited(ctx)) { unsigned long long v = 0; HIP_TRY(ctx, hipMemcpy(&v, visited, 8, hipMemcpyDeviceToHost)); pl->stats.affine_visited_cells = v; }
+  if (d_visited) pl->stats.affine_visited_cells = h_visited;
   pl->stats.allele_bytes = pl->out_seq_bytes + 40ull * pl->out_alleles;
   pl->stats.algorithmic_bytes = pl->stats.edit_seq_bytes + 4 * pl->stats.edit_cells + pl->stats.affine_seq_bytes + 4 * pl->stats.affine_cells +
                                 (pl->stats.affine_cells + 1) / 2 + pl->stats.allele_bytes;
   {
-    std::vector<otg_region_result> rr(NG);
-    HIP_TRY(ctx, hipMemcpy(rr.data(), B(B_REGRES), (size_t)NG * sizeof(otg_region_result), hipMemcpyDeviceToHost));
     uint64_t ok = 0;
     for (auto& r : rr) { if (r.status < 0) return otg_fail(ctx, OTG_ERR_FATAL, "a region hit a condition on which the reference exit(1)s (status %d)", r.status); ok += (r.n_alleles > 0); }
     pl->stats.n_regions_ok = ok;
diff --git a/otter_amd/csrc/poa.hip b/otter_amd/csrc/poa.hip
--- a/otter_amd/csrc/poa.hip
+++ b/otter_amd/csrc/poa.hip
@@ -1,5 +1,7 @@
 #include "otg_common.hpp"
+#include "otg_scan.hpp"
 #include <vector>
+#include <cstddef>
 #include <cstdlib>
 #include <algorithm>
 
@@ -49,6 +51,154 @@
     prev = op;
   }
   n_alt[m] = alt; n_mrun[m] = mrun;
+}
+
+constexpr uint32_t POA_LDS_NODE_B = 18, POA_LDS_EDGE_B = 8;
+constexpr uint32_t POA_EST_STEP = 512, POA_EST_MAX = 16u * 1024u, POA_EST_BUCKETS = POA_EST_MAX / POA_EST_STEP + 2;
+enum { CAP_NODE = 0, CAP_EDGE, CAP_START, CAP_ANCHOR, CAP_KINDS };
+struct PoaPlanRec {
+  uint64_t nn;
+  uint64_t tot[2][CAP_KINDS];
+  uint32_t n_list[2];
+  uint32_t first[2];
+  uint32_t n_live, lds_bytes;
+  uint32_t wide;
+  uint32_t unsortable;
+  uint32_t est_hist[POA_EST_BUCKETS];
+};
+constexpr size_t POA_PLAN_REC_HOST_BYTES = offsetof(PoaPlanRec, est_hist);
+static_assert(POA_PLAN_REC_HOST_BYTES <= 128, "the host reads one record of at most 128 bytes");
+
+constexpr uint32_t POA_PLAN_U = 8;
+__global__ __launch_bounds__(256) void poa_plan_count_kernel(const uint8_t* __restrict__ cig_arena, const otg_poa_member* __restrict__ members,
+                                                             const otg_poa_graph* __restrict__ graphs, uint32_t n_graphs,
+                                                             uint64_t* __restrict__ cap, uint32_t* __restrict__ est, uint32_t* __restrict__ weight,
+                                                             PoaPlanRec* __restrict__ rec)
+{
+  const uint32_t lane = threadIdx.x & 63u;
+  const uint32_t g = blockIdx.x * (blockDim.x >> 6) + (threadIdx.x >> 6);
+  if (g >= n_graphs) return;
+  const otg_poa_graph G = graphs[g];
+  uint64_t alt = 0, mrun = 0;
+  for (uint32_t m = 0; m < G.n_members; ++m) {
+    const otg_poa_member M = members[G.first_member + m];
+    const uint8_t* c = cig_arena + M.cigar_off;
+    const uint32_t n = M.cigar_len;
+    unsigned long long carry = 0;
+    for (uint32_t base = 0; base < n; base += 64u * POA_PLAN_U) {
+      uint8_t op[POA_PLAN_U];
+#pragma unroll
+      for (uint32_t u = 0; u < POA_PLAN_U; ++u) { const uint32_t i = base + u * 64u + lane; op[u] = (i >= base && i < n) ? c[i] : (uint8_t)0; }
+#pragma unroll
+      for (uint32_t u = 0; u < POA_PLAN_U; ++u) {
+        const unsigned long long a = __ballot(op[u] == 'X' || op[u] == 'I'), mm = __ballot(op[u] == 'M');
+        alt += (uint64_t)__popcll(a);
+        mrun += (uint64_t)__popcll(mm & ~((mm << 1) | carry));
+        carry = mm >> 63;
+      }
+    }
+  }
+  if (lane != 0) return;
+  const uint64_t ncap = ((uint64_t)G.backbone_len + alt + 2 + 3) & ~3ull, ecap = (alt + mrun + 2 + 1) & ~1ull;
+  const size_t stride = (size_t)n_graphs + 1;
+  cap[CAP_NODE * stride + g] = ncap;
+  cap[CAP_EDGE * stride + g] = ecap;
+  cap[CAP_START * stride + g] = (uint64_t)G.n_members + 2;
+  cap[CAP_ANCHOR * stride + g] = ((uint64_t)G.backbone_len + 2 + 3) & ~3ull;
+  if (ncap >= (1ull << 24) - 2) rec->wide = 1u;
+  uint32_t e = 0, w = 0;
+  if (!(G.backbone_len == 0 && G.n_members == 0)) {
+    const double B = (double)G.backbone_len;
+    const double need = (double)POA_LDS_NODE_B * (B + 0.5 * ((double)ncap - B) + 4.0) + (double)POA_LDS_EDGE_B * (0.5 * (double)ecap + 4.0) + (double)((2u * (G.n_members + 2u) + 7u) & ~7u) + 32.0 + 64.0;
+    e = need > 4.0e9 ? 0xffffffffu : (uint32_t)need;
+    const uint64_t bucket = ((uint64_t)e + POA_EST_STEP - 1) / POA_EST_STEP;
+    atomicAdd(&rec->est_hist[bucket < POA_EST_BUCKETS - 1 ? bucket : POA_EST_BUCKETS - 1], 1u);
+    atomicAdd(&rec->n_live, 1u);
+    if (ncap + ecap >= (1ull << 31)) rec->unsortable = 1u; else w = (uint32_t)(ncap + ecap);
+  }
+  est[g] = e; weight[g] = w;
+}
+
+__device__ uint32_t poa_plan_lds_bytes(const PoaPlanRec* rec, int no_lds)
+{
+  const uint32_t n_live = rec->n_live;
+  if (n_live == 0 || no_lds) return 0u;
+  const uint64_t k = (uint64_t)((double)(n_live - 1) * 0.97);
+  uint64_t seen = 0;
+  for (uint32_t b = 1; b < POA_EST_BUCKETS - 1; ++b) {
+    seen += rec->est_hist[b];
+    if (seen > k) { const uint32_t v = b * POA_EST_STEP; return v > 4096u ? v : 4096u; }
+  }
+  return 0u;
+}
+
+constexpr uint32_t POA_SORT_BITS = 11, POA_SORT_RADIX = 1u << POA_SORT_BITS, POA_SORT_PASSES = 3, POA_SORT_CHUNK = 4096;
+__global__ __launch_bounds__(256) void poa_plan_keys_kernel(const uint32_t* __restrict__ est, const uint32_t* __restrict__ weight, uint32_t n_graphs, int no_lds,
+                                                            uint64_t* __restrict__ keys, uint32_t* __restrict__ vals, PoaPlanRec* __restrict__ rec)
+{
+  __shared__ uint32_t s_lds;
+  if (threadIdx.x == 0) s_lds = poa_plan_lds_bytes(rec, no_lds);
+  __syncthreads();
+  const uint32_t lds_bytes = s_lds;
+  const uint32_t g = blockIdx.x * blockDim.x + threadIdx.x;
+  uint32_t list = 2;
+  if (g < n_graphs) {
+    const uint32_t e = est[g];
+    if (e) list = (lds_bytes && e <= lds_bytes) ? 0u : 1u;
+    keys[g] = ((uint64_t)list << 31) | (uint64_t)(0x7fffffffu - weight[g]);
+    vals[g] = g;
+  }
+  const unsigned long long m0 = __ballot(list == 0), m1 = __ballot(list == 1);
+  if ((threadIdx.x & 63u) == 0) {
+    if (m0) atomicAdd(&rec->n_list[0], (uint32_t)__popcll(m0));
+    if (m1) atomicAdd(&rec->n_list[1], (uint32_t)__popcll(m1));
+  }
+  if (blockIdx.x == 0 && threadIdx.x == 0) rec->lds_bytes = lds_bytes;
+}
+
+__global__ void poa_plan_first_kernel(PoaPlanRec* rec) { rec->first[0] = 0u; rec->first[1] = rec->n_list[0]; }
+
+__global__ __launch_bounds__(64) void poa_plan_sort_hist_kernel(const uint64_t* __restrict__ keys, uint32_t n, uint32_t shift, uint32_t W, uint32_t* __restrict__ table)
+{
+  __shared__ uint32_t h[POA_SORT_RADIX];
+  const uint32_t lane = threadIdx.x, w = blockIdx.x;
+  for (uint32_t d = lane; d < POA_SORT_RADIX; d += 64) h[d] = 0;
+  __syncthreads();
+  const uint32_t a = w * POA_SORT_CHUNK, b = a + POA_SORT_CHUNK < n ? a + POA_SORT_CHUNK : n;
+  for (uint32_t i = a + lane; i < b; i += 64) atomicAdd(&h[(uint32_t)(keys[i] >> shift) & (POA_SORT_RADIX - 1)], 1u);
+  __syncthreads();
+  for (uint32_t d = lane; d < POA_SORT_RADIX; d += 64) table[(size_t)d * W + w] = h[d];
+}
+
+__global__ __launch_bounds__(64) void poa_plan_sort_scatter_kernel(const uint64_t* __restrict__ keys, const uint32_t* __restrict__ vals, uint32_t n, uint32_t shift,
+                                                                   uint32_t W, const uint64_t* __restrict__ offs, uint64_t* __restrict__ keys_out, uint32_t* __restrict__ vals_out)
+{
+  __shared__ uint32_t pos[POA_SORT_RADIX];
+  const uint32_t lane = threadIdx.x, w = blockIdx.x;
+  for (uint32_t d = lane; d < POA_SORT_RADIX; d += 64) pos[d] = (uint32_t)offs[(size_t)d * W + w];
+  __syncthreads();
+  const uint32_t a = w * POA_SORT_CHUNK, b = a + POA_SORT_CHUNK < n ? a + POA_SORT_CHUNK : n;
+  for (uint32_t base = a; base < b; base += 64) {
+    const uint32_t i = base + lane;
+    const bool in = i < b;
+    const uint64_t key = in ? keys[i] : 0ull;
+    const uint32_t d = (uint32_t)(key >> shift) & (POA_SORT_RADIX - 1);
+    unsigned long long peers = __ballot(in);
+#pragma unroll
+    for (uint32_t bit = 0; bit < POA_SORT_BITS; ++bit) {
+      const bool s = (d >> bit) & 1u;
+      const unsigned long long mb = __ballot(in && s);
+      peers &= s ? mb : ~mb;
+    }
+    uint32_t p = 0;
+    if (in) p = pos[d] + (uint32_t)__popcll(peers & ((1ull << lane) - 1ull));
+    __syncthreads();
+    if (in) {
+      keys_out[p] = key; vals_out[p] = vals[i];
+      if (lane == 63u - (uint32_t)__builtin_clzll(peers)) pos[d] += (uint32_t)__popcll(peers);
+    }
+    __syncthreads();
+  }
 }
 
 #define OTG_LDS __attribute__((address_space(3)))
@@ -847,7 +997,6 @@
   return true;
 }
 
-constexpr uint32_t POA_LDS_NODE_B = 18, POA_LDS_EDGE_B = 8;
 __global__ __launch_bounds__(64) void poa_graph_lds_kernel(PoaDev P, const uint32_t* __restrict__ list, uint32_t lds_bytes)
 {
   extern __shared__ __attribute__((aligned(16))) uint8_t s_graph[];
@@ -919,145 +1068,66 @@
   }
 }
 
-}
-
-int otg_launch_poa(otg_ctx* ctx, const uint8_t* d_seq_arena, const uint8_t* d_cig_arena,
-                   const otg_poa_member* d_members, uint32_t n_members, const otg_poa_graph* d_graphs,
-                   const otg_poa_graph* h_graphs, uint32_t n_graphs, uint32_t* d_out_len,
-                   std::vector<uint64_t>& node_off)
-{
-  if (n_graphs == 0) return OTG_OK;
-  uint32_t* d_alt = (uint32_t*)otg_slot(ctx, SLOT_P20, (size_t)(n_members + 1) * sizeof(uint32_t));
-  uint32_t* d_nonm = (uint32_t*)otg_slot(ctx, SLOT_P21, (size_t)(n_members + 1) * sizeof(uint32_t));
-  if (!d_alt || !d_nonm) return OTG_ERR_HIP;
-  std::vector<uint32_t> h_alt(n_members), h_nonm(n_members);
-  if (n_members) {
-    hipLaunchKernelGGL(poa_count_kernel, dim3((n_members + 255) / 256), dim3(256), 0, ctx->stream, d_cig_arena, d_members, n_members, d_alt, d_nonm);
-    HIP_TRY(ctx, hipMemcpyAsync(h_alt.data(), d_alt, (size_t)n_members * sizeof(uint32_t), hipMemcpyDeviceToHost, ctx->stream));
-    HIP_TRY(ctx, hipMemcpyAsync(h_nonm.data(), d_nonm, (size_t)n_members * sizeof(uint32_t), hipMemcpyDeviceToHost, ctx->stream));
-    HIP_TRY(ctx, hipStreamSynchronize(ctx->stream));
-  }
-  std::vector<uint64_t> edge_off(n_graphs + 1), start_off(n_graphs + 1);
-  node_off.assign(n_graphs + 1, 0);
-  node_off[0] = edge_off[0] = start_off[0] = 0;
-  for (uint32_t g = 0; g < n_graphs; ++g) {
-    uint64_t alt = 0, mrun = 0;
-    for (uint32_t m = 0; m < h_graphs[g].n_members; ++m) { alt += h_alt[h_graphs[g].first_member + m]; mrun += h_nonm[h_graphs[g].first_member + m]; }
-    node_off[g + 1] = node_off[g] + (((uint64_t)h_graphs[g].backbone_len + alt + 2 + 3) & ~3ull);
-    edge_off[g + 1] = edge_off[g] + ((alt + mrun + 2 + 1) & ~1ull);
-    start_off[g + 1] = start_off[g] + h_graphs[g].n_members + 2;
-  }
-  const uint64_t NN = node_off[n_graphs];
-  PoaDev P;
-  P.seq_arena = d_seq_arena; P.cig_arena = d_cig_arena; P.members = d_members; P.graphs = d_graphs; P.n_graphs = n_graphs;
-  static const bool poa_v1 = getenv("OTG_POA_V1") != nullptr;
-  P.v2 = poa_v1 ? 0 : 1;
-  for (uint32_t g = 0; g < n_graphs && P.v2; ++g)
-    if (node_off[g + 1] - node_off[g] >= (1ull << 24) - 2) P.v2 = 0;
-  static const bool no_lds = getenv("OTG_POA_NO_LDS") != nullptr;
+struct PoaPiece { uint32_t k0, k1; bool lds; };
+struct PoaLayout {
+  uint64_t NN = 0, maxN = 0, maxE = 0, maxS = 0, maxA = 0;
   uint32_t lds_bytes = 0, n_lds = 0, n_glob = 0;
-  std::vector<uint32_t> order;
-  {
-    std::vector<uint32_t> est(n_graphs, 0u), live;
-    live.reserve(n_graphs);
-    for (uint32_t g = 0; g < n_graphs; ++g) {
-      if (h_graphs[g].backbone_len == 0 && h_graphs[g].n_members == 0) continue;
-      const double B = (double)h_graphs[g].backbone_len, ncap = (double)(node_off[g + 1] - node_off[g]), ecap = (double)(edge_off[g + 1] - edge_off[g]);
-      const double need = (double)POA_LDS_NODE_B * (B + 0.5 * (ncap - B) + 4.0) + (double)POA_LDS_EDGE_B * (0.5 * ecap + 4.0) + (double)((2u * (h_graphs[g].n_members + 2u) + 7u) & ~7u) + 32.0 + 64.0;
-      est[g] = need > 4.0e9 ? 0xffffffffu : (uint32_t)need;
-      live.push_back(g);
-    }
-    if (!live.empty() && !no_lds) {
-      std::vector<uint32_t> e2(live.size());
-      for (size_t i = 0; i < live.size(); ++i) e2[i] = est[live[i]];
-      const size_t k = (size_t)((double)(live.size() - 1) * 0.97);
-      std::nth_element(e2.begin(), e2.begin() + k, e2.end());
-      if (e2[k] <= 16u * 1024u) lds_bytes = std::max<uint32_t>((e2[k] + 511u) & ~511u, 4096u);
-    }
-    auto heavier = [&](uint32_t a, uint32_t b) {
-      const uint64_t wa = (edge_off[a + 1] - edge_off[a]) + (node_off[a + 1] - node_off[a]), wb = (edge_off[b + 1] - edge_off[b]) + (node_off[b + 1] - node_off[b]);
-      return wa != wb ? wa > wb : a < b;
-    };
-    order.reserve(live.size());
-    for (uint32_t g : live) if (lds_bytes && est[g] <= lds_bytes) order.push_back(g);
-    n_lds = (uint32_t)order.size();
-    for (uint32_t g : live) if (!(lds_bytes && est[g] <= lds_bytes)) order.push_back(g);
-    n_glob = (uint32_t)order.size() - n_lds;
-    std::sort(order.begin(), order.begin() + n_lds, heavier);
-    std::sort(order.begin() + n_lds, order.end(), heavier);
-  }
+  std::vector<PoaPiece> pieces;
+};
+
+inline uint64_t poa_image_bytes(uint64_t cn, uint64_t ce, uint64_t cs, uint64_t ca) { return cn * (sizeof(NodeG) + 10) + ce * (sizeof(EdgeG) + 4) + cs * 4 + ca * 12; }
+
+int poa_piece_budget(otg_ctx* ctx, size_t* out)
+{
   static const size_t piece_budget_cfg = getenv("OTG_POA_PIECE_MB") ? (size_t)atoll(getenv("OTG_POA_PIECE_MB")) << 20 : (size_t)24 << 30;
-  size_t piece_budget = piece_budget_cfg;
-  {
-    size_t free_b = 0, total_b = 0, held = 0;
-    HIP_TRY(ctx, hipMemGetInfo(&free_b, &total_b));
-    for (int sl : {SLOT_P3, SLOT_P4, SLOT_P6, SLOT_P7, SLOT_P8, SLOT_P9, SLOT_P10, SLOT_P11, SLOT_P12, SLOT_P13, SLOT_P16}) held += ctx->pool[sl].cap;
-    piece_budget = std::min(piece_budget, std::max<size_t>((size_t)1 << 30, (free_b + held) / 2));
-  }
-  struct Piece { uint32_t k0, k1; bool lds; };
-  std::vector<Piece> pieces;
-  std::vector<uint64_t> wnode(n_graphs + 1, 0), wedge(n_graphs + 1, 0), wstart(n_graphs + 1, 0), wanch(n_graphs + 1, 0);
-  uint64_t maxN = 0, maxE = 0, maxS = 0, maxA = 0;
-  {
-    auto cut = [&](uint32_t k0, uint32_t k1, bool lds) {
-      uint32_t p0 = k0;
-      uint64_t cn = 0, ce = 0, cs = 0, ca = 0;
-      for (uint32_t k = k0; k < k1; ++k) {
-        const uint32_t g = order[k];
-        const uint64_t nc = node_off[g + 1] - node_off[g], ec = edge_off[g + 1] - edge_off[g], sc = start_off[g + 1] - start_off[g];
-        const uint64_t ac = ((uint64_t)h_graphs[g].backbone_len + 2 + 3) & ~3ull;
-        const uint64_t bytes = (cn + nc) * (sizeof(NodeG) + 10) + (ce + ec) * (sizeof(EdgeG) + 4) + (cs + sc) * 4 + (ca + ac) * 12;
-        if (k > p0 && bytes > piece_budget) { pieces.push_back({p0, k, lds}); p0 = k; cn = ce = cs = ca = 0; }
-        wnode[g] = cn; wedge[g] = ce; wstart[g] = cs; wanch[g] = ca;
-        cn += nc; ce += ec; cs += sc; ca += ac;
-        maxN = std::max(maxN, cn); maxE = std::max(maxE, ce); maxS = std::max(maxS, cs); maxA = std::max(maxA, ca);
-      }
-      if (k1 > p0) pieces.push_back({p0, k1, lds});
-    };
-    cut(n_lds, n_lds + n_glob, false);
-    cut(0, n_lds, true);
-  }
+  size_t free_b = 0, total_b = 0, held = 0;
+  HIP_TRY(ctx, hipMemGetInfo(&free_b, &total_b));
+  for (int sl : {SLOT_P3, SLOT_P4, SLOT_P6, SLOT_P7, SLOT_P8, SLOT_P9, SLOT_P10, SLOT_P11, SLOT_P12, SLOT_P13, SLOT_P16}) held += ctx->pool[sl].cap;
+  *out = std::min(piece_budget_cfg, std::max<size_t>((size_t)1 << 30, (free_b + held) / 2));
+  return OTG_OK;
+}
+
+int poa_offset_slots(otg_ctx* ctx, PoaDev& P, uint32_t n_graphs)
+{
   uint64_t* d_node_off = (uint64_t*)otg_slot(ctx, SLOT_P0, (size_t)(n_graphs + 1) * sizeof(uint64_t));
   uint64_t* d_edge_off = (uint64_t*)otg_slot(ctx, SLOT_P1, (size_t)(n_graphs + 1) * sizeof(uint64_t));
   uint64_t* d_woff = (uint64_t*)otg_slot(ctx, SLOT_P2, (size_t)4 * (n_graphs + 1) * sizeof(uint64_t));
-  P.node_base = (uint8_t*)otg_slot(ctx, SLOT_P3, maxN);
-  P.is_end = (uint8_t*)otg_slot(ctx, SLOT_P4, maxN);
-  P.nodes = (NodeG*)otg_slot(ctx, SLOT_P6, maxN * sizeof(NodeG));
-  P.bb_cnt = (uint32_t*)otg_slot(ctx, SLOT_P9, maxN * 4);
-  P.queue = (uint32_t*)otg_slot(ctx, SLOT_P12, maxN * 4);
-  P.edges = (EdgeG*)otg_slot(ctx, SLOT_P13, maxE * sizeof(EdgeG));
-  P.start_list = (uint32_t*)otg_slot(ctx, SLOT_P16, maxS * 4);
-  P.out_arena = (uint8_t*)otg_slot(ctx, SLOT_P17, NN);
+  uint32_t* d_order = (uint32_t*)otg_slot(ctx, SLOT_P18, (size_t)(n_graphs + 1) * sizeof(uint32_t));
+  if (!d_node_off || !d_edge_off || !d_woff || !d_order) return OTG_ERR_HIP;
+  P.node_off = d_node_off; P.edge_off = d_edge_off;
+  P.wnode_off = d_woff; P.wedge_off = d_woff + (n_graphs + 1); P.wstart_off = d_woff + 2 * (size_t)(n_graphs + 1); P.wanch_off = d_woff + 3 * (size_t)(n_graphs + 1);
+  P.out_off = d_node_off;
+  P.order = d_order;
+  return OTG_OK;
+}
+
+int poa_launch_planned(otg_ctx* ctx, PoaDev& P, const PoaLayout& L, uint32_t* d_out_len)
+{
+  const uint32_t n_graphs = P.n_graphs;
+  P.node_base = (uint8_t*)otg_slot(ctx, SLOT_P3, L.maxN);
+  P.is_end = (uint8_t*)otg_slot(ctx, SLOT_P4, L.maxN);
+  P.nodes = (NodeG*)otg_slot(ctx, SLOT_P6, L.maxN * sizeof(NodeG));
+  P.bb_cnt = (uint32_t*)otg_slot(ctx, SLOT_P9, L.maxN * 4);
+  P.queue = (uint32_t*)otg_slot(ctx, SLOT_P12, L.maxN * 4);
+  P.edges = (EdgeG*)otg_slot(ctx, SLOT_P13, L.maxE * sizeof(EdgeG));
+  P.start_list = (uint32_t*)otg_slot(ctx, SLOT_P16, L.maxS * 4);
+  P.out_arena = (uint8_t*)otg_slot(ctx, SLOT_P17, L.NN);
   P.out_start = (uint32_t*)otg_slot(ctx, SLOT_P29, (size_t)n_graphs * 4);
   P.status = (int32_t*)otg_slot(ctx, SLOT_P28, (size_t)n_graphs * 4);
   P.anext = nullptr; P.ahead = nullptr; P.atail = nullptr; P.acnt = nullptr;
   if (P.v2) {
-    P.anext = (int32_t*)otg_slot(ctx, SLOT_P7, maxE * 4);
-    P.ahead = (int32_t*)otg_slot(ctx, SLOT_P8, maxA * 4);
-    P.atail = (int32_t*)otg_slot(ctx, SLOT_P10, maxA * 4);
-    P.acnt = (uint32_t*)otg_slot(ctx, SLOT_P11, maxA * 4);
+    P.anext = (int32_t*)otg_slot(ctx, SLOT_P7, L.maxE * 4);
+    P.ahead = (int32_t*)otg_slot(ctx, SLOT_P8, L.maxA * 4);
+    P.atail = (int32_t*)otg_slot(ctx, SLOT_P10, L.maxA * 4);
+    P.acnt = (uint32_t*)otg_slot(ctx, SLOT_P11, L.maxA * 4);
     if (!P.anext || !P.ahead || !P.atail || !P.acnt) return OTG_ERR_HIP;
   }
-  uint32_t* d_order = (uint32_t*)otg_slot(ctx, SLOT_P18, (size_t)(n_graphs + 1) * sizeof(uint32_t));
-  if (!d_node_off || !d_edge_off || !d_woff || !P.node_base || !P.is_end || !P.nodes || !P.bb_cnt || !P.queue ||
-      !P.edges || !P.start_list || !P.out_arena || !P.out_start || !P.status || !d_order)
+  if (!P.node_base || !P.is_end || !P.nodes || !P.bb_cnt || !P.queue || !P.edges || !P.start_list || !P.out_arena || !P.out_start || !P.status)
     return OTG_ERR_HIP;
-  P.node_off = d_node_off; P.edge_off = d_edge_off;
-  P.wnode_off = d_woff; P.wedge_off = d_woff + (n_graphs + 1); P.wstart_off = d_woff + 2 * (size_t)(n_graphs + 1); P.wanch_off = d_woff + 3 * (size_t)(n_graphs + 1);
-  P.out_off = d_node_off;
   P.out_len = d_out_len;
-  P.order = d_order;
-  if (!order.empty()) HIP_TRY(ctx, hipMemcpyAsync(d_order, order.data(), order.size() * sizeof(uint32_t), hipMemcpyHostToDevice, ctx->stream));
   HIP_TRY(ctx, hipMemsetAsync(d_out_len, 0, (size_t)n_graphs * sizeof(uint32_t), ctx->stream));
   HIP_TRY(ctx, hipMemsetAsync(P.out_start, 0, (size_t)n_graphs * sizeof(uint32_t), ctx->stream));
   HIP_TRY(ctx, hipMemsetAsync(P.status, 0, (size_t)n_graphs * sizeof(int32_t), ctx->stream));
-  HIP_TRY(ctx, hipMemcpyAsync(d_node_off, node_off.data(), (size_t)(n_graphs + 1) * sizeof(uint64_t), hipMemcpyHostToDevice, ctx->stream));
-  HIP_TRY(ctx, hipMemcpyAsync(d_edge_off, edge_off.data(), (size_t)(n_graphs + 1) * sizeof(uint64_t), hipMemcpyHostToDevice, ctx->stream));
-  HIP_TRY(ctx, hipMemcpyAsync(d_woff, wnode.data(), (size_t)(n_graphs + 1) * sizeof(uint64_t), hipMemcpyHostToDevice, ctx->stream));
-  HIP_TRY(ctx, hipMemcpyAsync(d_woff + (n_graphs + 1), wedge.data(), (size_t)(n_graphs + 1) * sizeof(uint64_t), hipMemcpyHostToDevice, ctx->stream));
-  HIP_TRY(ctx, hipMemcpyAsync(d_woff + 2 * (size_t)(n_graphs + 1), wstart.data(), (size_t)(n_graphs + 1) * sizeof(uint64_t), hipMemcpyHostToDevice, ctx->stream));
-  HIP_TRY(ctx, hipMemcpyAsync(d_woff + 3 * (size_t)(n_graphs + 1), wanch.data(), (size_t)(n_graphs + 1) * sizeof(uint64_t), hipMemcpyHostToDevice, ctx->stream));
-  HIP_TRY(ctx, hipStreamSynchronize(ctx->stream));
   static const bool profile = getenv("OTG_POA_PROFILE") != nullptr;
   P.prof = nullptr; P.prof_graph = nullptr;
   if (profile) {
@@ -1071,7 +1141,8 @@
   P.fb_list = (uint32_t*)otg_slot(ctx, SLOT_P22, (size_t)(n_graphs + 1) * sizeof(uint32_t));
   if (!P.fb_list) return OTG_ERR_HIP;
   P.fb_count = P.fb_list + n_graphs;
-  for (const Piece& pc : pieces) {
+  const uint32_t lds_bytes = L.lds_bytes, n_lds = L.n_lds, n_glob = L.n_glob;
+  for (const PoaPiece& pc : L.pieces) {
     const uint32_t n = pc.k1 - pc.k0;
     if (!pc.lds) hipLaunchKernelGGL(poa_graph_wave_kernel, dim3(n), dim3(64), 0, ctx->stream, P, P.order + pc.k0, (const uint32_t*)nullptr, n);
     else {
@@ -1112,3 +1183,202 @@
   }
   return OTG_OK;
 }
+
+int poa_plan_on_device(otg_ctx* ctx, PoaDev& P, uint32_t* d_out_len, bool no_lds, bool* planned)
+{
+  *planned = false;
+  const uint32_t n = P.n_graphs;
+  hipStream_t st = ctx->stream;
+  size_t piece_budget = 0;
+  if (int rc = poa_piece_budget(ctx, &piece_budget)) return rc;
+  if (int rc = poa_offset_slots(ctx, P, n)) return rc;
+  const size_t stride = (size_t)n + 1;
+  const uint32_t W = (n + POA_SORT_CHUNK - 1) / POA_SORT_CHUNK;
+  const size_t table_n = (size_t)POA_SORT_RADIX * W;
+  uint64_t* d_cap = (uint64_t*)otg_slot(ctx, SLOT_P20, CAP_KINDS * stride * sizeof(uint64_t));
+  uint32_t* d_est = (uint32_t*)otg_slot(ctx, SLOT_P21, 2 * stride * sizeof(uint32_t));
+  uint64_t* d_keys = (uint64_t*)otg_slot(ctx, SLOT_P14, 2 * stride * sizeof(uint64_t) + 2 * stride * sizeof(uint32_t));
+  uint64_t* d_offs = (uint64_t*)otg_slot(ctx, SLOT_P15, table_n * (sizeof(uint64_t) + sizeof(uint32_t)));
+  PoaPlanRec* d_rec = (PoaPlanRec*)otg_slot(ctx, SLOT_P5, sizeof(PoaPlanRec));
+  if (!d_cap || !d_est || !d_keys || !d_offs || !d_rec) return OTG_ERR_HIP;
+  uint32_t* d_weight = d_est + stride;
+  uint64_t* keys[2] = {d_keys, d_keys + stride};
+  uint32_t* vals[2] = {(uint32_t*)(d_keys + 2 * stride), (uint32_t*)(d_keys + 2 * stride) + stride};
+  uint32_t* d_table = (uint32_t*)(d_offs + table_n);
+  HIP_TRY(ctx, hipMemsetAsync(d_rec, 0, sizeof(PoaPlanRec), st));
+  hipLaunchKernelGGL(poa_plan_count_kernel, dim3((n + 3) / 4), dim3(256), 0, st, P.cig_arena, P.members, P.graphs, n, d_cap, d_est, d_weight, d_rec);
+  {
+    OtgScanJobs sj;
+    sj.j[0].in = d_cap + CAP_NODE * stride; sj.j[0].in_u64 = 1; sj.j[0].out = (uint64_t*)P.node_off; sj.j[0].n = n; sj.j[0].write_end = 1; sj.j[0].total = &d_rec->nn;
+    sj.j[1].in = d_cap + CAP_EDGE * stride; sj.j[1].in_u64 = 1; sj.j[1].out = (uint64_t*)P.edge_off; sj.j[1].n = n; sj.j[1].write_end = 1;
+    hipLaunchKernelGGL(otg_scan_jobs_kernel<8>, dim3(2), dim3(1024), 0, st, sj);
+  }
+  hipLaunchKernelGGL(poa_plan_keys_kernel, dim3((n + 255) / 256), dim3(256), 0, st, (const uint32_t*)d_est, (const uint32_t*)d_weight, n, no_lds ? 1 : 0, keys[0], vals[0], d_rec);
+  hipLaunchKernelGGL(poa_plan_first_kernel, dim3(1), dim3(1), 0, st, d_rec);
+  for (uint32_t pass = 0; pass < POA_SORT_PASSES; ++pass) {
+    const uint32_t src = pass & 1u, dst = src ^ 1u, shift = pass * POA_SORT_BITS;
+    hipLaunchKernelGGL(poa_plan_sort_hist_kernel, dim3(W), dim3(64), 0, st, (const uint64_t*)keys[src], n, shift, W, d_table);
+    OtgScanJobs sj;
+    sj.j[0].in = d_table; sj.j[0].out = d_offs; sj.j[0].n = (uint32_t)table_n;
+    hipLaunchKernelGGL(otg_scan_jobs_kernel<8>, dim3(1), dim3(1024), 0, st, sj);
+    hipLaunchKernelGGL(poa_plan_sort_scatter_kernel, dim3(W), dim3(64), 0, st, (const uint64_t*)keys[src], (const uint32_t*)vals[src], n, shift, W, (const uint64_t*)d_offs,
+                       keys[dst], pass + 1 == POA_SORT_PASSES ? (uint32_t*)P.order : vals[dst]);
+  }
+  {
+    OtgScanJobs sj;
+    uint64_t* w[CAP_KINDS] = {(uint64_t*)P.wnode_off, (uint64_t*)P.wedge_off, (uint64_t*)P.wstart_off, (uint64_t*)P.wanch_off};
+    for (int l = 0; l < 2; ++l)
+      for (int k = 0; k < CAP_KINDS; ++k) {
+        OtgScanJob& j = sj.j[l * CAP_KINDS + k];
+        j.in = d_cap + k * stride; j.in_u64 = 1; j.idx = P.order; j.first_ptr = &d_rec->first[l]; j.n_ptr = &d_rec->n_list[l]; j.out = w[k]; j.total = &d_rec->tot[l][k];
+      }
+    static_assert(2 * CAP_KINDS <= OTG_SCAN_MAX_JOBS, "one block per list and capacity kind");
+    hipLaunchKernelGGL(otg_scan_jobs_kernel<8>, dim3(2 * CAP_KINDS), dim3(1024), 0, st, sj);
+  }
+  PoaPlanRec rec;
+  HIP_TRY(ctx, hipMemcpyAsync(&rec, d_rec, POA_PLAN_REC_HOST_BYTES, hipMemcpyDeviceToHost, st));
+  HIP_TRY(ctx, hipStreamSynchronize(st));
+  HIP_TRY(ctx, hipGetLastError());
+  if (rec.unsortable) return OTG_OK;
+  for (int l = 0; l < 2; ++l)
+    if (rec.n_list[l] > 1 && poa_image_bytes(rec.tot[l][CAP_NODE], rec.tot[l][CAP_EDGE], rec.tot[l][CAP_START], rec.tot[l][CAP_ANCHOR]) > piece_budget) return OTG_OK;
+  if (rec.wide) P.v2 = 0;
+  PoaLayout L;
+  L.NN = rec.nn;
+  L.maxN = std::max(rec.tot[0][CAP_NODE], rec.tot[1][CAP_NODE]); L.maxE = std::max(rec.tot[0][CAP_EDGE], rec.tot[1][CAP_EDGE]);
+  L.maxS = std::max(rec.tot[0][CAP_START], rec.tot[1][CAP_START]); L.maxA = std::max(rec.tot[0][CAP_ANCHOR], rec.tot[1][CAP_ANCHOR]);
+  L.lds_bytes = rec.lds_bytes; L.n_lds = rec.n_list[0]; L.n_glob = rec.n_list[1];
+  if (L.n_glob) L.pieces.push_back({L.n_lds, L.n_lds + L.n_glob, false});
+  if (L.n_lds) L.pieces.push_back({0u, L.n_lds, true});
+  *planned = true;
+  return poa_launch_planned(ctx, P, L, d_out_len);
+}
+
+}
+
+int otg_launch_poa(otg_ctx* ctx, const uint8_t* d_seq_arena, const uint8_t* d_cig_arena,
+                   const otg_poa_member* d_members, uint32_t n_members, const otg_poa_graph* d_graphs,
+                   const otg_poa_graph* h_graphs, uint32_t n_graphs, uint32_t* d_out_len,
+                   std::vector<uint64_t>& node_off)
+{
+  if (n_graphs == 0) return OTG_OK;
+  uint32_t* d_alt = (uint32_t*)otg_slot(ctx, SLOT_P20, (size_t)(n_members + 1) * sizeof(uint32_t));
+  uint32_t* d_nonm = (uint32_t*)otg_slot(ctx, SLOT_P21, (size_t)(n_members + 1) * sizeof(uint32_t));
+  if (!d_alt || !d_nonm) return OTG_ERR_HIP;
+  std::vector<uint32_t> h_alt(n_members), h_nonm(n_members);
+  if (n_members) {
+    hipLaunchKernelGGL(poa_count_kernel, dim3((n_members + 255) / 256), dim3(256), 0, ctx->stream, d_cig_arena, d_members, n_members, d_alt, d_nonm);
+    HIP_TRY(ctx, hipMemcpyAsync(h_alt.data(), d_alt, (size_t)n_members * sizeof(uint32_t), hipMemcpyDeviceToHost, ctx->stream));
+    HIP_TRY(ctx, hipMemcpyAsync(h_nonm.data(), d_nonm, (size_t)n_members * sizeof(uint32_t), hipMemcpyDeviceToHost, ctx->stream));
+    HIP_TRY(ctx, hipStreamSynchronize(ctx->stream));
+  }
+  std::vector<uint64_t> edge_off(n_graphs + 1), start_off(n_graphs + 1);
+  node_off.assign(n_graphs + 1, 0);
+  node_off[0] = edge_off[0] = start_off[0] = 0;
+  for (uint32_t g = 0; g < n_graphs; ++g) {
+    uint64_t alt = 0, mrun = 0;
+    for (uint32_t m = 0; m < h_graphs[g].n_members; ++m) { alt += h_alt[h_graphs[g].first_member + m]; mrun += h_nonm[h_graphs[g].first_member + m]; }
+    node_off[g + 1] = node_off[g] + (((uint64_t)h_graphs[g].backbone_len + alt + 2 + 3) & ~3ull);
+    edge_off[g + 1] = edge_off[g] + ((alt + mrun + 2 + 1) & ~1ull);
+    start_off[g + 1] = start_off[g] + h_graphs[g].n_members + 2;
+  }
+  const uint64_t NN = node_off[n_graphs];
+  PoaDev P;
+  P.seq_arena = d_seq_arena; P.cig_arena = d_cig_arena; P.members = d_members; P.graphs = d_graphs; P.n_graphs = n_graphs;
+  static const bool poa_v1 = getenv("OTG_POA_V1") != nullptr;
+  P.v2 = poa_v1 ? 0 : 1;
+  for (uint32_t g = 0; g < n_graphs && P.v2; ++g)
+    if (node_off[g + 1] - node_off[g] >= (1ull << 24) - 2) P.v2 = 0;
+  static const bool no_lds = getenv("OTG_POA_NO_LDS") != nullptr;
+  uint32_t lds_bytes = 0, n_lds = 0, n_glob = 0;
+  std::vector<uint32_t> order;
+  {
+    std::vector<uint32_t> est(n_graphs, 0u), live;
+    live.reserve(n_graphs);
+    for (uint32_t g = 0; g < n_graphs; ++g) {
+      if (h_graphs[g].backbone_len == 0 && h_graphs[g].n_members == 0) continue;
+      const double B = (double)h_graphs[g].backbone_len, ncap = (double)(node_off[g + 1] - node_off[g]), ecap = (double)(edge_off[g + 1] - edge_off[g]);
+      const double need = (double)POA_LDS_NODE_B * (B + 0.5 * (ncap - B) + 4.0) + (double)POA_LDS_EDGE_B * (0.5 * ecap + 4.0) + (double)((2u * (h_graphs[g].n_members + 2u) + 7u) & ~7u) + 32.0 + 64.0;
+      est[g] = need > 4.0e9 ? 0xffffffffu : (uint32_t)need;
+      live.push_back(g);
+    }
+    if (!live.empty() && !no_lds) {
+      std::vector<uint32_t> e2(live.size());
+      for (size_t i = 0; i < live.size(); ++i) e2[i] = est[live[i]];
+      const size_t k = (size_t)((double)(live.size() - 1) * 0.97);
+      std::nth_element(e2.begin(), e2.begin() + k, e2.end());
+      if (e2[k] <= 16u * 1024u) lds_bytes = std::max<uint32_t>((e2[k] + 511u) & ~511u, 4096u);
+    }
+    auto heavier = [&](uint32_t a, uint32_t b) {
+      const uint64_t wa = (edge_off[a + 1] - edge_off[a]) + (node_off[a + 1] - node_off[a]), wb = (edge_off[b + 1] - edge_off[b]) + (node_off[b + 1] - node_off[b]);
+      return wa != wb ? wa > wb : a < b;
+    };
+    order.reserve(live.size());
+    for (uint32_t g : live) if (lds_bytes && est[g] <= lds_bytes) order.push_back(g);
+    n_lds = (uint32_t)order.size();
+    for (uint32_t g : live) if (!(lds_bytes && est[g] <= lds_bytes)) order.push_back(g);
+    n_glob = (uint32_t)order.size() - n_lds;
+    std::sort(order.begin(), order.begin() + n_lds, heavier);
+    std::sort(order.begin() + n_lds, order.end(), heavier);
+  }
+  size_t piece_budget = 0;
+  if (int rc = poa_piece_budget(ctx, &piece_budget)) return rc;
+  std::vector<PoaPiece> pieces;
+  std::vector<uint64_t> wnode(n_graphs + 1, 0), wedge(n_graphs + 1, 0), wstart(n_graphs + 1, 0), wanch(n_graphs + 1, 0);
+  uint64_t maxN = 0, maxE = 0, maxS = 0, maxA = 0;
+  {
+    auto cut = [&](uint32_t k0, uint32_t k1, bool lds) {
+      uint32_t p0 = k0;
+      uint64_t cn = 0, ce = 0, cs = 0, ca = 0;
+      for (uint32_t k = k0; k < k1; ++k) {
+        const uint32_t g = order[k];
+        const uint64_t nc = node_off[g + 1] - node_off[g], ec = edge_off[g + 1] - edge_off[g], sc = start_off[g + 1] - start_off[g];
+        const uint64_t ac = ((uint64_t)h_graphs[g].backbone_len + 2 + 3) & ~3ull;
+        const uint64_t bytes = (cn + nc) * (sizeof(NodeG) + 10) + (ce + ec) * (sizeof(EdgeG) + 4) + (cs + sc) * 4 + (ca + ac) * 12;
+        if (k > p0 && bytes > piece_budget) { pieces.push_back({p0, k, lds}); p0 = k; cn = ce = cs = ca = 0; }
+        wnode[g] = cn; wedge[g] = ce; wstart[g] = cs; wanch[g] = ca;
+        cn += nc; ce += ec; cs += sc; ca += ac;
+        maxN = std::max(maxN, cn); maxE = std::max(maxE, ce); maxS = std::max(maxS, cs); maxA = std::max(maxA, ca);
+      }
+      if (k1 > p0) pieces.push_back({p0, k1, lds});
+    };
+    cut(n_lds, n_lds + n_glob, false);
+    cut(0, n_lds, true);
+  }
+  if (int rc = poa_offset_slots(ctx, P, n_graphs)) return rc;
+  uint64_t* d_woff = (uint64_t*)P.wnode_off;
+  if (!order.empty()) HIP_TRY(ctx, hipMemcpyAsync((uint32_t*)P.order, order.data(), order.size() * sizeof(uint32_t), hipMemcpyHostToDevice, ctx->stream));
+  HIP_TRY(ctx, hipMemcpyAsync((uint64_t*)P.node_off, node_off.data(), (size_t)(n_graphs + 1) * sizeof(uint64_t), hipMemcpyHostToDevice, ctx->stream));
+  HIP_TRY(ctx, hipMemcpyAsync((uint64_t*)P.edge_off, edge_off.data(), (size_t)(n_graphs + 1) * sizeof(uint64_t), hipMemcpyHostToDevice, ctx->stream));
+  HIP_TRY(ctx, hipMemcpyAsync(d_woff, wnode.data(), (size_t)(n_graphs + 1) * sizeof(uint64_t), hipMemcpyHostToDevice, ctx->stream));
+  HIP_TRY(ctx, hipMemcpyAsync(d_woff + (n_graphs + 1), wedge.data(), (size_t)(n_graphs + 1) * sizeof(uint64_t), hipMemcpyHostToDevice, ctx->stream));
+  HIP_TRY(ctx, hipMemcpyAsync(d_woff + 2 * (size_t)(n_graphs + 1), wstart.data(), (size_t)(n_graphs + 1) * sizeof(uint64_t), hipMemcpyHostToDevice, ctx->stream));
+  HIP_TRY(ctx, hipMemcpyAsync(d_woff + 3 * (size_t)(n_graphs + 1), wanch.data(), (size_t)(n_graphs + 1) * sizeof(uint64_t), hipMemcpyHostToDevice, ctx->stream));
+  HIP_TRY(ctx, hipStreamSynchronize(ctx->stream));
+  PoaLayout L;
+  L.NN = NN; L.maxN = maxN; L.maxE = maxE; L.maxS = maxS; L.maxA = maxA;
+  L.lds_bytes = lds_bytes; L.n_lds = n_lds; L.n_glob = n_glob;
+  L.pieces = std::move(pieces);
+  return poa_launch_planned(ctx, P, L, d_out_len);
+}
+
+int otg_launch_poa_resident(otg_ctx* ctx, const uint8_t* d_seq_arena, const uint8_t* d_cig_arena,
+                            const otg_poa_member* d_members, uint32_t n_members, const otg_poa_graph* d_graphs, uint32_t n_graphs, uint32_t* d_out_len)
+{
+  if (n_graphs == 0) return OTG_OK;
+  static const bool host_plan = getenv("OTG_POA_HOST_PLAN") != nullptr || getenv("OTG_POA_V1") != nullptr;
+  static const bool no_lds = getenv("OTG_POA_NO_LDS") != nullptr;
+  if (!host_plan) {
+    PoaDev P;
+    P.seq_arena = d_seq_arena; P.cig_arena = d_cig_arena; P.members = d_members; P.graphs = d_graphs; P.n_graphs = n_graphs;
+    P.v2 = 1;
+    bool planned = false;
+    const int rc = poa_plan_on_device(ctx, P, d_out_len, no_lds, &planned);
+    if (rc || planned) return rc;
+  }
+  std::vector<otg_poa_graph> h_graphs(n_graphs);
+  HIP_TRY(ctx, hipMemcpyAsync(h_graphs.data(), d_graphs, (size_t)n_graphs * sizeof(otg_poa_graph), hipMemcpyDeviceToHost, ctx->stream));
+  HIP_TRY(ctx, hipStreamSynchronize(ctx->stream));
+  std::vector<uint64_t> node_off;
+  return otg_launch_poa(ctx, d_seq_arena, d_cig_arena, d_members, n_members, d_graphs, h_graphs.data(), n_graphs, d_out_len, node_off);
+}
```

Measured after the change: 17800, median of 6. 1.6% higher.
